# vdBerg93/cl-rrt

Hardware: AMD Instinct MI355X
Metric: nodes expanded/sec (200-obstacle scene) (higher is better)
Workload: dtype f64

## Files before the change

cl-rrt_amd/csrc/clrrt_capi.hip:

```cpp
#include <hip/hip_runtime.h>
#include <math.h>

#include <algorithm>
#include <climits>
#include <array>
#include <chrono>
#include <cmath>
#include <cstdio>
#include <cstdlib>
#include <cstring>
#include <deque>
#include <functional>
#include <optional>
#include <string>
#include <vector>

#include "../../include/clrrt.h"
#include "clrrt_dev.hpp"
#include "clrrt_internal.hpp"

static const int kWalkMaxOver = 2048, kWalkMaxChunks = 64;

using namespace clrrt;

#define CAND_K 10
#define NN_K 11

struct DevBuf {
  void* p = nullptr;
  size_t bytes = 0;
};

struct clrrt_ctx {
  int device = 0;
  int rank = 0;
  hipStream_t stream = nullptr;
  bool own_stream = false;
  clrrt_params params;
  DevParams dp;
  clrrt_capacity cap;
  std::string err;
  clrrt_node* tree = nullptr;
  NnRec* nn = nullptr;
  double* arena = nullptr;
  int64_t n_nodes = 0, n_rows = 0;
  BakedObs* obs = nullptr;
  int n_obs = 0;
  ObsGrid grid{};
  void* grid_buf = nullptr;
  size_t grid_bytes = 0;
  clrrt_sample* d_samples = nullptr;
  float* pk = nullptr;
  int* pi = nullptr;
  int64_t partial_cap = 0;
  int* cand = nullptr;
  float* ckey = nullptr;
  int* ncand = nullptr;
  int* ctie = nullptr;
  KeyId* sort_scratch = nullptr;
  int64_t sort_cap = 0;
  RollRes* res_spec = nullptr;
  clrrt_node* regnodes = nullptr;
  RollRes* res_gb = nullptr;
  double* slots = nullptr;
  int slot_rows = 0;
  int rows_deferred = 1;
  void* rep_buf = nullptr;
  int rep_n = 0;
  bool eval_deferred = false;
  clrrt_node* gbnodes = nullptr;
  SampleOut* so = nullptr;
  int* first_conflict = nullptr;
  clrrt_node* out_nodes = nullptr;
  Job* jobs = nullptr;
  int64_t* totals = nullptr;
  bool totals_zeroed = false;
  unsigned long long* work_ctr = nullptr;
  float* nn_seed = nullptr;
  double bbox[4] = {HUGE_VAL, HUGE_VAL, -HUGE_VAL, -HUGE_VAL};
  double* d_bbox = nullptr;
  double* h_bbox = nullptr;
  int64_t nnw_min_nodes = 8192;
  bool nnw_stateless = false;
  int nnw_bud_tiles = 3072, nnw_bud_ex = 4096, nnw_chunks = 16, nnw_max_over = 1024;
  bool nnw_max_over_set = false;
  bool nnw_bud_tiles_set = false;
  int nnw_half_max = 4096;
  int nnw_hscale = 50;
  int nnw_lpt = 0;
  int nnw_index = 5;
  int nnw_lds_floor = 0;
  int nnw_waves = -1;
  int nnw_double = 1;
  WalkBufs nnw{};
  WalkBufs nnw_alt{};
  struct { int64_t n = -1; double ox, oy, x0, y0, x1, y1; float delta; } nnw_built;
  CompactBufs cmp{};
  int roll_persistent = 1;
  int nn_debug = 0;
  int roll_blocks = 0;
  int n_cu = 256;
  int* roll_q = nullptr;
  int* roll_best = nullptr;
  int roll_priority = 1;
  int roll_coop = 1;
  int roll_spread = 1;
  int roll_lanes = 0;
  int nn_exact_fused = 1;
  int exact_min_width = 8;
  int exact_fixup = 1;
  int exact_fix_cap = 0;
  int* fix_n = nullptr;
  int* fix_ids = nullptr;
  int* fix_adj = nullptr;
  NnRec* fix_xrec = nullptr;
  int* fix_xi = nullptr;
  int* fix_xcand = nullptr;
  float* fix_xkey = nullptr;
  int* fix_xn = nullptr;
  std::vector<int> h_fix_cand;
  std::vector<RollRes> h_fix_spec;
  Job* fix_jobs = nullptr;
  RollRes* fix_res = nullptr;
  std::vector<int> h_fix;
  std::vector<clrrt_sample> h_fix_smp;
  std::vector<Job> h_fix_jobs;
  std::vector<int> h_fix_owner;
  std::vector<RollRes> h_fix_res;
  std::vector<SampleOut> h_fix_so;
  int64_t ex_stats[10] = {0, 0, 0, 0, 0, 0, 0, 0, 0, 0};
  int* roll_perm = nullptr;
  int* roll_pflag = nullptr;
  GoalRec* goal_recs = nullptr;
  int* bp_path = nullptr;
  clrrt_node* path_nodes = nullptr;
  double* path_rows = nullptr;
  int path_cap = 0;
  int64_t path_rows_cap = 0;
  int path_n = 0;
  int64_t path_nrows = 0;
  int* ri_int = nullptr;
  int64_t* ri_off = nullptr;
  float* ri_cost = nullptr;
  double* ri_terms = nullptr;
  double reg_x0 = 0, reg_y0 = 0, reg_x1 = 0, reg_y1 = 0;
  int nn_pipeline = 1;
  hipStream_t side = nullptr;
  int cu_split = 0;
  hipStream_t roll_st = nullptr;
  hipEvent_t ev_rs0 = nullptr, ev_rs1 = nullptr;
  hipEvent_t ev_tree = nullptr, ev_walk = nullptr, ev_commit = nullptr;
  clrrt_sample* d_samples2 = nullptr;
  clrrt_sample* h_samples2 = nullptr;
  int* cand2 = nullptr;
  float* ckey2 = nullptr;
  int* ncand2 = nullptr;
  int* ctie2 = nullptr;
  int nn_lag = 0;
  clrrt_sample* d_samples3 = nullptr;
  clrrt_sample* h_samples3 = nullptr;
  int* cand3 = nullptr;
  float* ckey3 = nullptr;
  int* ncand3 = nullptr;
  int* ctie3 = nullptr;
  WalkBufs nnw3{};
  hipStream_t side2 = nullptr;
  hipStream_t mst = nullptr;
  int nn_split_delta = 0;
  int nn_delta_early = 1;
  int nn_lane_order = 1;
  int* nn_order = nullptr;
  float* wseed[3] = {nullptr, nullptr, nullptr};
  hipEvent_t ev_wm[3] = {nullptr, nullptr, nullptr};
  float* nn_seed2 = nullptr;
  float* d1pk[3] = {nullptr, nullptr, nullptr};
  int* d1pi[3] = {nullptr, nullptr, nullptr};
  hipEvent_t ev_d1[3] = {nullptr, nullptr, nullptr};
  hipEvent_t ev_s[3] = {nullptr, nullptr, nullptr};
  hipEvent_t ev_lagw[3] = {nullptr, nullptr, nullptr};
  int stream_prio = 1;
  int walk_cu_reserve = 0;
  hipEvent_t ev_lag[3] = {nullptr, nullptr, nullptr};
  int stream_prio_applied = 0;
  bool side_prio_set = false;
  std::vector<clrrt_sample> pf_next, pf_samples;
  int pf_state = 0;
  struct {
    int T = 0;
    bool active = false;
    int R = 0;
    int T_alloc = 0, n_steps_alloc = 0;
    int64_t vcap = 0;
    RollRes* res = nullptr;
    RollRes* res_gb = nullptr;
    int* cand = nullptr;
    int* ncand = nullptr;
    clrrt_sample* samp = nullptr;
    int* best = nullptr;
    int* dlist[2] = {nullptr, nullptr};
    int cur_dl = 0, nd = 0;
    int nd_eval = -1;
    int* gv = nullptr;
    uint8_t* pend = nullptr;
    void* sel_tmp = nullptr;
    size_t sel_bytes = 0;
    int* d_cnt = nullptr;
    void* carry[2] = {nullptr, nullptr};
    int cur_c = 0, ncarry = 0, carry_cap = 0;
    int64_t round = 0;
    int slot = 0;
    int64_t deferred_total = 0;
  } def;
  struct {
    int rank = 0, world = 1;
    void* dev_local = nullptr;
    int cap_local = 0;
    clrrt_exchange_fn fn = nullptr;
    void* user = nullptr;
    double max_ms = 0;
    int64_t nd_global = 0;
    int64_t rows_stop = 0;
    int last_nb = 0;
    clrrt_node* xbuf = nullptr;
    uint32_t* xkey = nullptr;
    void* xtmp = nullptr;
    size_t xtmp_bytes = 0;
    int64_t xcap = 0;
    unsigned long long* d_goal = nullptr;
    bool poison_seen = false;
    bool fn_failed = false;
  } sh;
  int fail_at_round = 0;
  int fail_after_exchange = 0;
  bool debug_sync = false;
  unsigned long long* dbg_host = nullptr;
  bool iter_log = false;
  std::vector<int64_t> round_sizes;
  std::vector<clrrt_iteration> iters;
  std::vector<SampleOut> iter_tmp;
  clrrt_sample* h_samples = nullptr;
  int64_t* h_totals = nullptr;
  int* h_int = nullptr;
  int64_t last_eval_rows = 0;
  int64_t last_goal_nodes = 0;
  clrrt_counters counters{};
  int64_t nn_bf_keys = 0, nn_samples = 0;
  int64_t nn_super_bounds = 0;
  bool timing = false;
  static constexpr int kKtClasses = 6;
  double kt_ms[kKtClasses] = {};
  int64_t kt_n[kKtClasses] = {};
  std::vector<hipEvent_t> ev_pool;
  std::vector<std::pair<int, std::pair<hipEvent_t, hipEvent_t>>> ev_pending;
};
// ... 130 lines not shown
extern "C" {

int clrrt_abi_version(void) { return CLRRT_ABI_VERSION; }
static_assert(sizeof(clrrt_exchange_io) == 128, "clrrt_exchange_io layout (clrrt/abi.py ExchangeIO)");

int clrrt_params_default(clrrt_params* p, double v0, const double goal[4], double vmax) {
  if (!p) return CLRRT_EINVAL;
  memset(p, 0, sizeof(*p));
  p->veh.dmax = 0.52; p->veh.ddmax = 0.3294; p->veh.Td = 0.3; p->veh.Ta = 0.3;
  p->veh.amin = -6; p->veh.amax = 2; p->veh.L = 2.7;
  double lf = 1.0868, lr = 1.6132, Cf = 22201, Cr = 22201, m = 950 + 640;
  p->veh.Kus = (m / p->veh.L) * (lr / Cf - lf / Cr);
  p->veh.Vch = 20;
  p->ctrl_tla = 1.4; p->ctrl_mindla = 3.2; p->ctrl_dlavmin = 3; p->ref_int = 0.02; p->ref_mindist = 0.2;
  p->sim_dt = 0.04; p->ctrl_Kp = 8; p->ctrl_Ki = 0.05;
  p->Wcost[0] = 10; p->Wcost[1] = 5; p->Wcost[2] = 0; p->Wcost[3] = 4; p->Wcost[4] = 1;
  p->ref_res = std::max(std::abs(v0) * p->ref_int, p->ref_mindist);
  p->vmax = vmax;
  p->ay_road_max = 0;
  for (int i = 0; i < 4; i++) p->goal[i] = goal ? goal[i] : 0.0;
  p->bend = 0;
  p->obs_use_pred = 1;
  p->sort_limit = 10;
  p->collision_mode = CLRRT_COLLISION_STUB;
  return CLRRT_OK;
}

void clrrt_rng_seed(clrrt_rng* g, uint32_t seed) {
  int32_t* s = g->r;
  int32_t word = (int32_t)(seed == 0 ? 1 : seed);
  s[0] = word;
  for (int i = 1; i < 31; i++) {
    int32_t hi = word / 127773, lo = word % 127773;
    word = 16807 * lo - 2836 * hi;
    if (word < 0) word += 2147483647;
    s[i] = word;
  }
  s[31] = 3;
  s[32] = 0;
  s[33] = 0;
  g->pos = 0;
  for (int i = 0; i < 310; i++) clrrt_rng_next(g);
}

int32_t clrrt_rng_next(clrrt_rng* g) {
  int32_t* s = g->r;
  int f = s[31], r = s[32];
  uint32_t v = (uint32_t)s[f] + (uint32_t)s[r];
  s[f] = (int32_t)v;
  int32_t out = (int32_t)(v >> 1);
  f = f + 1 == 31 ? 0 : f + 1;
  r = r + 1 == 31 ? 0 : r + 1;
  s[31] = f;
  s[32] = r;
  return out;
}

int clrrt_draw_samples(const clrrt_params* p, clrrt_rng* rng, int32_t n, clrrt_sample* out) {
  if (!p || !rng || (n > 0 && !out)) return CLRRT_EINVAL;
  const double* g = p->goal;
  const double RM = 2147483647.0;
  double dGoal = sqrt(g[0] * g[0] + g[1] * g[1]);
  double hd = atan2(g[1], g[0]);
  double latMin = -7, latMax = 7;
  float fl = (float)(RM / (dGoal + 10));
  float fw = (float)(RM / (latMax - latMin));
  double ch, sh, cq, sq;
  ::sincos(hd, &sh, &ch);
  ::sincos(hd + M_PI / 2, &sq, &cq);
  for (int j = 0; j < n; j++) {
    double rLong = (float)clrrt_rng_next(rng) / fl;
    double rLat = latMin + (float)clrrt_rng_next(rng) / fw;
    out[j].x = rLong * ch + rLat * cq;
    out[j].y = rLong * sh + rLat * sq;
    double r = (double)clrrt_rng_next(rng) / (double)(2147483647 / 1);
    out[j].explore = r <= ((0 * 0.3) + (1 * 0.7));
    out[j].pad = 0;
  }
  return CLRRT_OK;
}

const char* clrrt_last_error(const clrrt_ctx* c) { return c ? c->err.c_str() : "null context"; }

static void free_all(clrrt_ctx* c) {
  if (c->side) hipStreamSynchronize(c->side);
  void* ptrs[] = {c->tree, c->nn, c->arena, c->obs, c->d_samples, c->pk, c->pi, c->cand, c->ckey, c->ncand,
                  c->ctie, c->sort_scratch, c->res_spec, c->regnodes, c->res_gb, c->gbnodes, c->so, c->first_conflict,
                  c->out_nodes, c->jobs, c->slots, c->rep_buf, c->totals, c->work_ctr, c->grid_buf,
                  c->nn_seed, c->d_bbox, c->roll_q, c->roll_best, c->roll_perm, c->roll_pflag,
                  c->goal_recs, c->bp_path, c->path_nodes, c->path_rows, c->ri_int, c->ri_off, c->ri_cost,
                  c->ri_terms, c->nnw.keys, c->nnw.keys2, c->nnw.vals, c->nnw.vals2, c->nnw.tmp, c->nnw.P, c->nnw.Q,
                  c->nnw.CE, c->nnw.ID, c->nnw.tiles, c->nnw.supers, c->nnw.sorder, c->nnw.HEAD, c->nnw.ovf_n, c->nnw.ovf, c->nnw.pk, c->nnw.pi, c->nnw_alt.keys, c->nnw_alt.keys2, c->nnw_alt.vals, c->nnw_alt.vals2, c->nnw_alt.tmp, c->nnw_alt.P, c->nnw_alt.Q, c->nnw_alt.CE, c->nnw_alt.ID, c->nnw_alt.tiles, c->nnw_alt.supers, c->nnw_alt.sorder, c->nnw_alt.HEAD, c->nnw_alt.ovf_n, c->nnw_alt.ovf, c->nnw_alt.pk, c->nnw_alt.pi, c->nnw.skeys, c->nnw.sids, c->nnw_alt.skeys, c->nnw_alt.sids, c->cmp.packed, c->cmp.scanned,
                  c->cmp.tmp, c->d_samples2, c->cand2, c->ckey2, c->ncand2, c->ctie2, c->d_samples3, c->cand3, c->ckey3,
                  c->ncand3, c->ctie3, c->nnw3.keys, c->nnw3.keys2, c->nnw3.vals, c->nnw3.vals2, c->nnw3.tmp, c->nnw3.P,
                  c->nnw3.Q, c->nnw3.CE, c->nnw3.ID, c->nnw3.tiles, c->nnw3.supers, c->nnw3.sorder, c->nnw3.HEAD,
                  c->nnw3.ovf_n, c->nnw3.ovf, c->nnw3.pk, c->nnw3.pi, c->nnw3.skeys, c->nnw3.sids,
                  c->nnw.trun, c->nnw_alt.trun, c->nnw3.trun, c->nnw.wctr, c->nnw_alt.wctr, c->nnw3.wctr};
  for (void* p : ptrs)
    if (p) hipFree(p);
  void* sptrs[] = {c->sh.xbuf, c->sh.xkey, c->sh.xtmp, c->sh.d_goal, c->fix_n, c->fix_ids, c->fix_jobs, c->fix_res, c->fix_adj,
                   c->fix_xrec, c->fix_xi, c->fix_xcand, c->fix_xkey, c->fix_xn};
  for (void* p : sptrs)
    if (p) hipFree(p);
  void* dptrs[] = {c->def.res, c->def.res_gb, c->def.cand, c->def.ncand, c->def.samp, c->def.best, c->def.dlist[0],
                   c->def.dlist[1], c->def.gv, c->def.pend, c->def.sel_tmp, c->def.d_cnt, c->def.carry[0],
                   c->def.carry[1]};
  for (void* p : dptrs)
    if (p) hipFree(p);
  if (c->h_samples) hipHostFree(c->h_samples);
  if (c->h_samples2) hipHostFree(c->h_samples2);
  if (c->h_samples3) hipHostFree(c->h_samples3);
  if (c->side2) hipStreamSynchronize(c->side2);
  if (c->side2) hipStreamDestroy(c->side2);
  for (auto e : c->ev_lag)
    if (e) hipEventDestroy(e);
  for (auto e : c->ev_lagw)
    if (e) hipEventDestroy(e);
  if (c->mst) hipStreamSynchronize(c->mst);
  if (c->mst) hipStreamDestroy(c->mst);
  for (int q = 0; q < 3; q++) {
    if (c->ev_d1[q]) hipEventDestroy(c->ev_d1[q]);
    if (c->ev_s[q]) hipEventDestroy(c->ev_s[q]);
    if (c->d1pk[q]) hipFree(c->d1pk[q]);
    if (c->wseed[q]) hipFree(c->wseed[q]);
    if (q == 0 && c->nn_order) hipFree(c->nn_order);
    if (c->ev_wm[q]) hipEventDestroy(c->ev_wm[q]);
    if (c->d1pi[q]) hipFree(c->d1pi[q]);
  }
  if (c->nn_seed2) hipFree(c->nn_seed2);
  if (c->side) hipStreamSynchronize(c->side);
  if (c->ev_tree) hipEventDestroy(c->ev_tree);
  if (c->ev_walk) hipEventDestroy(c->ev_walk);
  if (c->ev_commit) hipEventDestroy(c->ev_commit);
  if (c->side) hipStreamDestroy(c->side);
  if (c->roll_st) hipStreamDestroy(c->roll_st);
  if (c->ev_rs0) hipEventDestroy(c->ev_rs0);
  if (c->ev_rs1) hipEventDestroy(c->ev_rs1);
  if (c->h_totals) hipHostFree(c->h_totals);
  if (c->h_int) hipHostFree(c->h_int);
  if (c->h_bbox) hipHostFree(c->h_bbox);
  if (c->dbg_host) hipHostFree(c->dbg_host);
  for (auto& pe : c->ev_pending) { hipEventDestroy(pe.second.first); hipEventDestroy(pe.second.second); }
  for (auto e : c->ev_pool) hipEventDestroy(e);
  if (c->own_stream && c->stream) hipStreamDestroy(c->stream);
}

int clrrt_create(const clrrt_params* p, const clrrt_capacity* cap, int device, clrrt_ctx** out) {
  if (!p || !out) return CLRRT_EINVAL;
  *out = nullptr;
  int ndev = 0;
  if (hipGetDeviceCount(&ndev) != hipSuccess || ndev <= 0) return CLRRT_EHIP;
  if (device < 0 || device >= ndev) return CLRRT_EINVAL;
  clrrt_ctx* c = new clrrt_ctx();
  c->device = device;
  c->params = *p;
  c->debug_sync = getenv("CLRRT_DEBUG_SYNC") != nullptr;
  clrrt_capacity dc;
  dc.max_nodes = 1 << 20;
  dc.max_rows = 1 << 24;
  dc.max_batch = 4096;
  dc.max_obstacles = 4096;
  c->cap = cap ? *cap : dc;
  if (c->cap.max_nodes < 2 || c->cap.max_rows < 2 || c->cap.max_batch < 1 || c->cap.max_obstacles < 0) {
    delete c;
    return CLRRT_EINVAL;
  }
  derive(c->params, c->dp, 0);
  int rc = CLRRT_OK;
  auto chk = [&](hipError_t e) {
    if (e != hipSuccess && rc == CLRRT_OK) { rc = CLRRT_EHIP; c->err = hipGetErrorString(e); }
  };
  chk(hipSetDevice(device));
  chk(hipStreamCreateWithFlags(&c->stream, hipStreamNonBlocking));
  c->own_stream = true;
  const int64_t B = c->cap.max_batch;
  chk(dalloc(&c->tree, c->cap.max_nodes));
  chk(dalloc(&c->nn, c->cap.max_nodes));
  chk(dalloc(&c->arena, (size_t)c->cap.max_rows * 10));
  chk(dalloc(&c->obs, std::max<int64_t>(1, c->cap.max_obstacles)));
  chk(dalloc(&c->d_samples, B));
  c->partial_cap = std::max<int64_t>(B * 16, 4096) * NN_K;
  chk(dalloc(&c->pk, c->partial_cap));
  chk(dalloc(&c->pi, c->partial_cap));
  chk(dalloc(&c->cand, B * CAND_K));
  chk(dalloc(&c->ckey, B * CAND_K));
  chk(dalloc(&c->ncand, B));
  chk(dalloc(&c->ctie, B));
  chk(dalloc(&c->d_samples2, B));
  chk(dalloc(&c->cand2, B * CAND_K));
  chk(dalloc(&c->ckey2, B * CAND_K));
  chk(dalloc(&c->ncand2, B));
  chk(dalloc(&c->ctie2, B));
  chk(hipStreamCreateWithFlags(&c->side, hipStreamNonBlocking));
  chk(hipEventCreateWithFlags(&c->ev_tree, hipEventDisableTiming));
  chk(hipEventCreateWithFlags(&c->ev_walk, hipEventDisableTiming));
  chk(hipEventCreateWithFlags(&c->ev_commit, hipEventDisableTiming));
  chk(dalloc(&c->res_spec, B * CAND_K));
  chk(dalloc(&c->regnodes, B));
  chk(dalloc(&c->res_gb, B * CAND_K));
  c->slot_rows = 0;
  chk(hipMalloc(&c->rep_buf, replay_bytes() * (size_t)2 * B));
  chk(dalloc(&c->gbnodes, B));
  chk(dalloc(&c->so, B));
  chk(dalloc(&c->first_conflict, 1));
  chk(dalloc(&c->out_nodes, 2 * B));
  chk(dalloc(&c->jobs, 2 * B));
  chk(dalloc(&c->totals, 8));
  chk(dalloc(&c->cmp.packed, B));
  chk(dalloc(&c->cmp.scanned, B));
  c->cmp.tmp_bytes = compact_scan_bytes((int)B);
  chk(hipMalloc(&c->cmp.tmp, std::max<size_t>(c->cmp.tmp_bytes, 256)));
  chk(dalloc(&c->nn_seed, B));
  chk(dalloc(&c->roll_q, 1));
  chk(dalloc(&c->roll_best, B));
  chk(dalloc(&c->roll_perm, (int64_t)B * CAND_K));
  chk(dalloc(&c->roll_pflag, 2 * (int64_t)B * CAND_K + (int64_t)(roll_order_scratch_bytes(B * CAND_K) / 4 + 64)));
  {
    int ncu = 0;
    if (hipDeviceGetAttribute(&ncu, hipDeviceAttributeMultiprocessorCount, device) == hipSuccess && ncu > 0)
      c->n_cu = ncu;
  }
  chk(dalloc(&c->d_bbox, 4));
  chk(hipHostMalloc((void**)&c->h_bbox, sizeof(double) * 4, hipHostMallocDefault));
  chk(dalloc(&c->work_ctr, 64));
  if (rc == CLRRT_OK) chk(hipMemset(c->work_ctr, 0, 64 * sizeof(unsigned long long)));
  chk(hipHostMalloc((void**)&c->h_samples, sizeof(clrrt_sample) * B, hipHostMallocDefault));
  chk(hipHostMalloc((void**)&c->h_samples2, sizeof(clrrt_sample) * B, hipHostMallocDefault));
  chk(hipHostMalloc((void**)&c->h_totals, sizeof(int64_t) * 8, hipHostMallocDefault));
  chk(hipHostMalloc((void**)&c->h_int, sizeof(int) * 4, hipHostMallocDefault));
  if (rc != CLRRT_OK) {
    fprintf(stderr, "clrrt_create: %s\n", c->err.c_str());
    free_all(c);
    delete c;
    return rc;
  }
  *out = c;
  return CLRRT_OK;
}

void clrrt_destroy(clrrt_ctx* c) {
  if (!c) return;
  hipSetDevice(c->device);
  if (c->stream) hipStreamSynchronize(c->stream);
  free_all(c);
  delete c;
}

int clrrt_set_stream(clrrt_ctx* c, void* s) {
  if (!c) return CLRRT_EINVAL;
  HIPC(c, hipStreamSynchronize(c->stream));
  if (c->own_stream) hipStreamDestroy(c->stream);
  if (s) {
    c->stream = (hipStream_t)s;
    c->own_stream = false;
  } else {
    HIPC(c, hipStreamCreateWithFlags(&c->stream, hipStreamNonBlocking));
    c->own_stream = true;
  }
  return CLRRT_OK;
}

int clrrt_set_rank(clrrt_ctx* c, int32_t rank) {
  if (!c || rank < 0) return CLRRT_EINVAL;
  c->rank = rank;
  return CLRRT_OK;
}

int clrrt_set_params(clrrt_ctx* c, const clrrt_params* p) {
  if (!c || !p) return CLRRT_EINVAL;
  pf_reset(c);
  DevParams d;
  derive(*p, d, c->n_obs);
  int rc = flush_replays(c);
  if (rc != CLRRT_OK) return rc;
  if (c->slots && d.n_steps_max + 1 > c->slot_rows) {
    HIPC(c, hipSetDevice(c->device));
    HIPC(c, hipStreamSynchronize(c->stream));
    HIPC(c, hipFree(c->slots));
    c->slots = nullptr;
    c->slot_rows = 0;
    HIPC(c, dalloc(&c->slots, (size_t)2 * (d.n_steps_max + 1) * 10 * c->cap.max_batch * CAND_K));
    c->slot_rows = d.n_steps_max + 1;
  }
  c->params = *p;
  c->dp = d;
  return CLRRT_OK;
}

}

static const float kVehRad = 2.6220219f, kCullMargin = 0.05f;
static int build_grid(clrrt_ctx* c, const std::vector<BakedObs>& b) {
  std::vector<int> stat, mov;
  for (int i = 0; i < (int)b.size(); i++) (b[i].moving ? mov : stat).push_back(i);
// ... 1029 lines not shown
    const RollRes* sres = c->h_fix_spec.data() + (size_t)j * K;
    const int acc = o.k >= 0 ? spec[o.k] : -1;
    for (int q = 0; q < K; q++) {
      if (spec[q] < 0 || (o.k >= 0 && q >= o.k)) break;
      add_res(d, sres[q], -1);
    }
    bool found = false;
    for (int t = 0; t < ln; t++) {
      const int e = lst[t];
      if (e == acc) { found = true; break; }
      int q = -1;
      if (e < N)
        for (int r = 0; r < K && spec[r] >= 0; r++)
          if (spec[r] == e) { q = r; break; }
      if (q >= 0 && (o.k < 0 || q < o.k) && is_fail(sres[q].outcome)) {
        add_res(d, sres[q], +1);
      } else if (e < N) {
        job(j, 0, e);
      } else {
        const int pw = xpos[e - N];
        job(j, 1 + (pw & 1), pw >> 1);
      }
    }
    if (o.k >= 0 && !found) {
      stop = j;
      c->ex_stats[8]++;
      while (!c->h_fix_owner.empty() && c->h_fix_owner.back() == j) {
        c->h_fix_owner.pop_back();
        c->h_fix_jobs.pop_back();
      }
      break;
    }
  }
  const int nj = (int)c->h_fix_jobs.size();
  c->h_fix_res.resize(nj);
  if (nj > 0) {
    HIPC(c, hipMemcpyAsync(c->fix_jobs, c->h_fix_jobs.data(), sizeof(Job) * nj, hipMemcpyHostToDevice, st));
    RollArgs a = roll_args(c, nj);
    a.jobs = c->fix_jobs;
    a.res = c->fix_res;
    a.res_gb = c->fix_res;
    a.xreg = c->regnodes;
    a.xgb = c->gbnodes;
    a.job_stride = 64;
    if (c->exact_fix_cap > 0 && c->exact_fix_cap < a.p.n_steps_max) a.p.n_steps_max = c->exact_fix_cap;
    {
      KTimer kt(c, 1);
      HIPC(c, launch_rollout(st, SRC_LIST, a));
    }
    HIPC(c, hipMemcpyAsync(c->h_fix_res.data(), c->fix_res, sizeof(RollRes) * nj, hipMemcpyDeviceToHost, st));
    HIPC(c, hipStreamSynchronize(st));
  }
  int Lr = stop, resolved = 0;
  bool patched = false;
  const int cap = c->exact_fix_cap > 0 && c->exact_fix_cap < c->dp.n_steps_max ? c->exact_fix_cap : 0;
  for (int j = 0, q = 0; j < stop; j++) {
    SampleOut add = delta[j];
    bool ok = true, any = fn[j] != 0;
    for (; q < nj && c->h_fix_owner[q] == j; q++) {
      const RollRes& r = c->h_fix_res[q];
      if (!is_fail(r.outcome) || (cap && r.outcome == CLRRT_ROLL_ITERLIMIT)) ok = false;
      add_res(add, r, +1);
    }
    if (!ok) {
      Lr = j;
      c->ex_stats[4]++;
      break;
    }
    if (!any) continue;
    SampleOut& o = c->h_fix_so[j];
    o.rollouts += add.rollouts; o.steps += add.steps; o.f_col += add.f_col; o.f_acc += add.f_acc; o.f_it += add.f_it;
    patched = true;
    resolved++;
  }
  if (patched) HIPC(c, hipMemcpyAsync(c->so, c->h_fix_so.data(), sizeof(SampleOut) * Lr, hipMemcpyHostToDevice, st));
  c->ex_stats[0]++;
  c->ex_stats[1] += resolved;
  c->ex_stats[2] += nj;
  c->ex_stats[3] += Lr < n;
  *L = std::max(1, Lr);
  return CLRRT_OK;
}

static int eval_samples(clrrt_ctx* c, int n, bool exact, int* L_out, bool have_lists = false,
                        const std::function<int()>& during_roll = nullptr,
                        const std::function<int()>& pre_roll = nullptr) {
  hipStream_t st = c->stream;
  KeyId* scratch = nullptr;
  if (exact) {
    int rc = ensure_sort_scratch(c, (int64_t)n * c->n_nodes);
    if (rc != CLRRT_OK) return rc;
    scratch = c->sort_scratch;
  }
  if (!have_lists) {
    int rc = run_nn(c, n, scratch);
    if (rc != CLRRT_OK) return rc;
  }
  if (pre_roll) {
    int rc = pre_roll();
    if (rc != CLRRT_OK) return rc;
  }
  if (during_roll) HIPC(c, hipEventRecord(c->ev_tree, st));
  hipStream_t rst = st;
  if (c->roll_st) {
    rst = c->roll_st;
    HIPC(c, hipEventRecord(c->ev_rs0, st));
    HIPC(c, hipStreamWaitEvent(rst, c->ev_rs0, 0));
  }
  const bool persistent = c->roll_persistent && c->dp.n_steps_max > 0;
  const bool deferred = persistent && c->rows_deferred;
  if (!deferred) {
    int rc = flush_replays(c);
    if (rc == CLRRT_OK) rc = ensure_slots(c);
    if (rc != CLRRT_OK) return rc;
  }
  const bool defer = c->def.active && !exact && persistent && deferred;
  if (defer) {
    auto& d = c->def;
    d.slot = (int)(d.round % d.R);
    const int64_t B = c->cap.max_batch;
    HIPC(c, hipMemcpyAsync(d.cand + (int64_t)d.slot * B * CAND_K, c->cand, sizeof(int) * n * CAND_K,
                           hipMemcpyDeviceToDevice, st));
    HIPC(c, hipMemcpyAsync(d.ncand + (int64_t)d.slot * B, c->ncand, sizeof(int) * n, hipMemcpyDeviceToDevice, st));
    HIPC(c, hipMemcpyAsync(d.samp + (int64_t)d.slot * B, c->d_samples, sizeof(clrrt_sample) * n,
                           hipMemcpyDeviceToDevice, st));
    if (d.nd + (int64_t)n > d.vcap) return fail(c, CLRRT_ECAPACITY, "deferred samples exceed the commit buffers");
    if (rst != st) {
      HIPC(c, hipEventRecord(c->ev_rs0, st));
      HIPC(c, hipStreamWaitEvent(rst, c->ev_rs0, 0));
    }
  }
  {
    KTimer kt(c, 1, rst);
    RollArgs a = roll_args(c, n * CAND_K);
    a.res = c->res_spec;
    a.res_gb = c->res_gb;
    if (defer) defer_roll_args(c, a, true);
    a.slots = deferred ? nullptr : c->slots;
    a.slot_rows = c->slot_rows;
    a.slot_jobs = (int)(c->cap.max_batch * CAND_K);
    if (deferred) {
      a.rep = c->rep_buf;
      a.nrep = c->rep_n;
    }
    const int64_t nt = c->n_nodes;
    const int eighths = nt < 300000 ? 7 : nt < 700000 ? 5 : nt < 1100000 ? 4 : 3;
    const int blocks = c->roll_blocks > 0 ? std::min(c->roll_blocks, 4 * c->n_cu)
                       : c->cu_split > 0  ? std::max(1, (c->cu_split * c->n_cu) / 8)
                                          : std::max(1, (eighths * c->n_cu) / 8);
    a.coop_enable = c->roll_coop;
    a.lanes_per_wave = c->roll_lanes > 0 ? c->roll_lanes : c->roll_spread ? 0 : 64;
    if (c->roll_priority) {
      a.perm = c->roll_perm;
      a.pflag = c->roll_pflag;
    }
    unsigned long long*& dbg_host = c->dbg_host;
    if (c->debug_sync) {
      if (!dbg_host) HIPC(c, hipHostMalloc((void**)&dbg_host, sizeof(unsigned long long) * 8 * 4096, hipHostMallocMapped));
      memset(dbg_host, 0, sizeof(unsigned long long) * 8 * 4096);
      HIPC(c, hipHostGetDevicePointer((void**)&a.dbg, dbg_host, 0));
      HIPC(c, hipStreamSynchronize(rst));
      fprintf(stderr, "[dbg] pre-rollout work done (n %d, nrep %d, ncarry %d)\n", n, a.nrep, a.ncarry);
    }
    if (persistent && defer) {
      FillInts f;
      f.add(a.ncarry_out, 1, 0);
      f.add(c->roll_q, 1, 0);
      f.add(c->def.best + a.sbase, n, 0x7f7f7f7f);
      f.add(c->def.d_cnt + 2, 1, 0);
      f.add((int*)c->totals, 16, 0);
      HIPC(c, launch_fill_ints(rst, f));
      c->totals_zeroed = true;
      HIPC(c, launch_rollout_persistent(rst, a, n, c->roll_q, c->def.best, blocks, true));
    } else if (persistent)
      HIPC(c, launch_rollout_persistent(rst, a, n, c->roll_q, defer ? c->def.best : c->roll_best, blocks));
    else
      HIPC(c, launch_rollout(rst, SRC_SPEC, a));
    if (c->debug_sync) {
      const auto t0 = std::chrono::steady_clock::now();
      while (hipStreamQuery(rst) == hipErrorNotReady) {
        if (std::chrono::duration<double>(std::chrono::steady_clock::now() - t0).count() > 10.0) {
          fprintf(stderr, "[dbg] rollout kernel not done after 10 s; waves (iterations, busy, parked, qdone|first "
                          "busy lane, j|pass, steps|chain, wp|N, t):\n");
          unsigned long long tmax = 0;
          for (int w = 0; w < 4096; w++) tmax = std::max(tmax, dbg_host[w * 8 + 7]);
          int shown = 0;
          for (int w = 0; w < 4096 && shown < 40; w++) {
            const unsigned long long* d = dbg_host + w * 8;
            if (d[7] == 0 || tmax - d[7] < 100000000ull) continue;
            if (d[1] == 0 && d[2] == 0 && (d[3] >> 32)) continue;
            fprintf(stderr, "  wave %d: it %llu busy %016llx parked %016llx qdone %llu lane %d j %d pass %d steps %d "
                            "chain %d wp %d N %d age %.3f s\n", w, d[0], d[1], d[2], d[3] >> 32, (int)(uint32_t)d[3],
                    (int)(d[4] >> 32), (int)(uint32_t)d[4], (int)(d[5] >> 32), (int)(uint32_t)d[5], (int)(d[6] >> 32),
                    (int)(uint32_t)d[6], (double)(tmax - d[7]) * 1e-8);
            shown++;
          }
          int alive = 0;
          for (int w = 0; w < 4096; w++) alive += dbg_host[w * 8 + 7] != 0 && tmax - dbg_host[w * 8 + 7] < 100000000ull;
          fprintf(stderr, "  waves still beating: %d\n", alive);
          abort();
        }
      }
      fprintf(stderr, "[dbg] rollout kernel done: %s\n", hipGetErrorString(hipStreamQuery(rst)));
    }
    if (deferred) c->rep_n = 0;
    c->eval_deferred = deferred;
  }
  if (c->roll_st) {
    HIPC(c, hipEventRecord(c->ev_rs1, rst));
    HIPC(c, hipStreamWaitEvent(st, c->ev_rs1, 0));
  }
  if (during_roll) {
    int rc = during_roll();
    if (rc != CLRRT_OK) return rc;
  }
  SelArgs s;
  memset(&s, 0, sizeof(s));
  s.p = c->dp; s.tree = c->tree; s.cand = c->cand; s.ckey = c->ckey; s.ncand = c->ncand; s.res = c->res_spec;
  s.res_gb = c->res_gb; s.regnodes = c->regnodes; s.gbnodes = c->gbnodes; s.so = c->so; s.B = n;
  if (defer) {
    auto& d = c->def;
    s.cand = d.cand; s.ncand = d.ncand; s.res = d.res; s.res_gb = d.res_gb;
    s.ckey = nullptr;
    s.view = d.dlist[d.cur_dl];
    s.nd = d.nd;
    s.sbase = d.slot * (int)c->cap.max_batch;
    s.gv = d.gv;
    s.pend = d.pend;
    s.new_pend = d.d_cnt + 2;
    s.B = d.nd + n;
  }
  c->def.nd_eval = defer ? c->def.nd : -1;
  {
    KTimer kt(c, 2);
    HIPC(c, launch_select(st, s));
  }
  int L = n;
  if (exact && n > 1 && c->exact_fixup) {
    int rc = exact_fixups(c, n, &L);
    if (rc != CLRRT_OK) return rc;
  } else if (exact && n > 1) {
    c->h_int[0] = n;
    HIPC(c, hipMemcpyAsync(c->first_conflict, c->h_int, sizeof(int), hipMemcpyHostToDevice, st));
    {
      KTimer kt(c, 2);
      HIPC(c, launch_conflict(st, c->dp, n, c->d_samples, c->regnodes, c->gbnodes, c->so, c->ctie,
                              c->first_conflict));
    }
    HIPC(c, hipMemcpyAsync(c->h_int + 1, c->first_conflict, sizeof(int), hipMemcpyDeviceToHost, st));
    HIPC(c, hipStreamSynchronize(st));
    L = std::max(1, std::min(n, c->h_int[1]));
  }
  *L_out = L;
  return CLRRT_OK;
}

static int compact_and_copy(clrrt_ctx* c, int L, int* n_out, bool merge_bbox) {
  hipStream_t st = c->stream;
  auto& d = c->def;
  const bool defer = d.nd_eval >= 0;
  const int V = defer ? d.nd_eval + L : L;
  {
    KTimer kt(c, 2);
    const bool tag = defer && c->sh.world > 1;
    HIPC(c, launch_compact(st, V, c->d_samples, c->cand, c->regnodes, c->gbnodes, c->so, c->n_rows, c->rank,
                           c->out_nodes, c->jobs, c->totals, c->cmp, tag ? d.slot : 0, tag ? d.R : 0,
                           (int)c->cap.max_batch, c->totals_zeroed));
    c->totals_zeroed = false;
    if (merge_bbox) HIPC(c, launch_bbox(st, c->out_nodes, c->totals, 0, c->d_bbox));
    if (defer) HIPC(c, launch_defer_select(st, d.gv, d.pend, V, d.dlist[1 - d.cur_dl], d.d_cnt, d.sel_tmp, d.sel_bytes));
  }
  HIPC(c, hipMemcpyAsync(c->h_totals, c->totals, sizeof(int64_t) * 8, hipMemcpyDeviceToHost, st));
  if (merge_bbox) HIPC(c, hipMemcpyAsync(c->h_bbox, c->d_bbox, sizeof(double) * 4, hipMemcpyDeviceToHost, st));
  if (defer) {
    HIPC(c, hipMemcpyAsync(c->h_int, d.d_cnt, sizeof(int) * 2, hipMemcpyDeviceToHost, st));
    HIPC(c, hipMemcpyAsync(c->h_int + 3, d.d_cnt + 2, sizeof(int), hipMemcpyDeviceToHost, st));
    HIPC(c, hipMemcpyAsync(c->h_int + 2, (const char*)(c->work_ctr + 62), sizeof(int), hipMemcpyDeviceToHost, st));
  }
  HIPC(c, hipStreamSynchronize(st));
  {
    const int rw = watchdog_check(c);
    if (rw != CLRRT_OK) return rw;
  }
  if (c->iter_log && !defer && L > 0) {
    c->iter_tmp.resize(L);
    HIPC(c, hipMemcpy(c->iter_tmp.data(), c->so, sizeof(SampleOut) * L, hipMemcpyDeviceToHost));
    for (int j = 0; j < L; j++) {
      const SampleOut& o = c->iter_tmp[j];
      clrrt_iteration r;
      r.nodes = (o.k >= 0) + (o.k >= 0 && o.gb_ok);
      r.sim_count = o.steps; r.fail_collision = o.f_col; r.fail_acclimit = o.f_acc; r.fail_iterlimit = o.f_it;
      r.rollouts = o.rollouts;
      c->iters.push_back(r);
    }
  }
  if (merge_bbox) bbox_add(c, c->h_bbox[0], c->h_bbox[1], c->h_bbox[2], c->h_bbox[3]);
  if (defer) {
    if (c->h_int[2] != 0 || c->h_int[1] > d.carry_cap)
      return fail(c, CLRRT_ECAPACITY, "suspended rollouts exceed the carry buffer (raise defer_steps)");
    if (L > 0) d.deferred_total += c->h_int[3];
    d.cur_dl ^= 1;
    d.nd = c->h_int[0];
    d.cur_c ^= 1;
    d.ncarry = c->h_int[1];
    d.round++;
    d.nd_eval = -1;
  }
  int64_t nn = c->h_totals[0], nr = c->h_totals[1];
  if (c->n_rows + nr > c->cap.max_rows) return fail(c, CLRRT_ECAPACITY, "trajectory arena full");
  if (c->fail_at_round > 0 && --c->fail_at_round == 0)
    return fail(c, CLRRT_ECAPACITY, "injected failure (option fail_at_round)");
  c->counters.sim_count += c->h_totals[2];
  c->counters.fail_collision += c->h_totals[3];
  c->counters.fail_acclimit += c->h_totals[4];
  c->counters.fail_iterlimit += c->h_totals[5];
  c->counters.rollouts += c->h_totals[6];
  c->last_goal_nodes = c->h_totals[7];
  if (c->eval_deferred) {
    if (c->rep_n > 0) {
      int rc = flush_replays(c);
      if (rc != CLRRT_OK) return rc;
    }
    KTimer kt(c, 2);
    if (defer)
      HIPC(c, launch_replay_gather(st, c->jobs, c->out_nodes, (int)nn, c->tree, d.cand, d.samp, d.res, c->rep_buf));
    else
      HIPC(c, launch_replay_gather(st, c->jobs, c->out_nodes, (int)nn, c->tree, c->cand, c->d_samples, c->res_spec,
                                   c->rep_buf));
    c->rep_n = (int)nn;
  } else {
    KTimer kt(c, 2);
    HIPC(c, launch_copy_rows(st, c->jobs, c->out_nodes, (int)nn, c->slots, c->slot_rows,
                             (int)(c->cap.max_batch * CAND_K), c->arena));
  }
  c->n_rows += nr;
  c->last_eval_rows = nr;
  *n_out = (int)nn;
  return CLRRT_OK;
}

static int ensure_defer(clrrt_ctx* c) {
  auto& d = c->def;
  const int64_t B = c->cap.max_batch;
  const int n = std::max(1, c->dp.n_steps_max);
  const int R = (int)((2LL * n + d.T - 1) / d.T) + 2;
  if (c->sh.world > 1 && R > 256)
    return fail(c, CLRRT_EINVAL, "defer_steps too small for sharded rounds (more than 256 rounds in flight)");
  if (!d.res || d.R < R) {
    HIPC(c, hipStreamSynchronize(c->stream));
    for (void* p : {(void*)d.res, (void*)d.res_gb, (void*)d.cand, (void*)d.ncand, (void*)d.samp, (void*)d.best})
      if (p) HIPC(c, hipFree(p));
    d.res = nullptr; d.res_gb = nullptr; d.cand = nullptr; d.ncand = nullptr; d.samp = nullptr; d.best = nullptr;
    d.R = 0;
    HIPC(c, dalloc(&d.res, (size_t)R * B * CAND_K));
    HIPC(c, dalloc(&d.res_gb, (size_t)R * B * CAND_K));
    HIPC(c, dalloc(&d.cand, (size_t)R * B * CAND_K));
    HIPC(c, dalloc(&d.ncand, (size_t)R * B));
    HIPC(c, dalloc(&d.samp, (size_t)R * B));
    HIPC(c, dalloc(&d.best, (size_t)R * B));
    d.R = R;
  }
  if (!d.gv || d.vcap < (int64_t)d.R * B) {
    const int64_t V = (int64_t)d.R * B;
    int rc = flush_replays(c);
    if (rc != CLRRT_OK) return rc;
    HIPC(c, hipStreamSynchronize(c->stream));
    for (void* p : {(void*)c->regnodes, (void*)c->gbnodes, (void*)c->so, (void*)c->out_nodes, (void*)c->jobs,
                    c->rep_buf, (void*)c->cmp.packed, (void*)c->cmp.scanned, c->cmp.tmp})
      if (p) HIPC(c, hipFree(p));
    c->regnodes = nullptr; c->gbnodes = nullptr; c->so = nullptr; c->out_nodes = nullptr; c->jobs = nullptr;
    c->rep_buf = nullptr; c->cmp.packed = nullptr; c->cmp.scanned = nullptr; c->cmp.tmp = nullptr;
    for (void* p : {(void*)d.dlist[0], (void*)d.dlist[1], (void*)d.gv, (void*)d.pend, d.sel_tmp, (void*)d.d_cnt,
                    d.carry[0], d.carry[1]})
      if (p) HIPC(c, hipFree(p));
    d.dlist[0] = d.dlist[1] = nullptr; d.gv = nullptr; d.pend = nullptr; d.sel_tmp = nullptr; d.d_cnt = nullptr;
    d.carry[0] = d.carry[1] = nullptr;
    HIPC(c, dalloc(&c->regnodes, V));
    HIPC(c, dalloc(&c->gbnodes, V));
    HIPC(c, dalloc(&c->so, V));
    HIPC(c, dalloc(&c->out_nodes, 2 * V));
    HIPC(c, dalloc(&c->jobs, 2 * V));
    HIPC(c, hipMalloc(&c->rep_buf, replay_bytes() * (size_t)2 * V));
    HIPC(c, dalloc(&c->cmp.packed, V));
    HIPC(c, dalloc(&c->cmp.scanned, V));
    c->cmp.tmp_bytes = compact_scan_bytes((int)V);
    HIPC(c, hipMalloc(&c->cmp.tmp, std::max<size_t>(c->cmp.tmp_bytes, 256)));
    HIPC(c, dalloc(&d.dlist[0], V));
    HIPC(c, dalloc(&d.dlist[1], V));
    HIPC(c, dalloc(&d.gv, V));
    HIPC(c, dalloc(&d.pend, V));
    d.sel_bytes = defer_select_bytes((int)V);
    HIPC(c, hipMalloc(&d.sel_tmp, std::max<size_t>(d.sel_bytes, 256)));
    HIPC(c, dalloc(&d.d_cnt, 3));
    d.carry_cap = (int)std::min<int64_t>(V * CAND_K, 1 << 21);
    HIPC(c, hipMalloc(&d.carry[0], carry_bytes() * (size_t)d.carry_cap));
    HIPC(c, hipMalloc(&d.carry[1], carry_bytes() * (size_t)d.carry_cap));
    d.vcap = V;
  }
  return CLRRT_OK;
}

static int defer_begin(clrrt_ctx* c, bool batch) {
  auto& d = c->def;
  d.active = batch && d.T > 0 && c->roll_persistent && c->rows_deferred && c->dp.n_steps_max > 0;
  d.nd = 0; d.ncarry = 0; d.round = 0; d.slot = 0; d.nd_eval = -1; d.deferred_total = 0;
  return d.active ? ensure_defer(c) : CLRRT_OK;
}

static void defer_roll_args(clrrt_ctx* c, RollArgs& a, bool capped) {
  auto& d = c->def;
  a.res = d.res;
  a.res_gb = d.res_gb;
  a.jbase = d.slot * (int)c->cap.max_batch * CAND_K;
  a.sbase = d.slot * (int)c->cap.max_batch;
  a.cap = capped ? d.T : 0;
  a.carry_in = d.carry[d.cur_c];
  a.ncarry = d.ncarry;
  a.carry_out = d.carry[1 - d.cur_c];
  a.ncarry_out = d.d_cnt + 1;
  a.carry_cap = d.carry_cap;
}

static int ensure_slots(clrrt_ctx* c) {
  const int need = c->dp.n_steps_max + 1;
  if (c->slots && c->slot_rows >= need) return CLRRT_OK;
  HIPC(c, hipSetDevice(c->device));
  HIPC(c, hipStreamSynchronize(c->stream));
  if (c->slots) HIPC(c, hipFree(c->slots));
  c->slots = nullptr;
  c->slot_rows = 0;
  HIPC(c, dalloc(&c->slots, (size_t)2 * need * 10 * c->cap.max_batch * CAND_K));
  c->slot_rows = need;
  return CLRRT_OK;
}

static int watchdog_check(clrrt_ctx* c) {
  unsigned long long h[4];
  HIPC(c, hipMemcpy(h, c->work_ctr + 56, sizeof(h), hipMemcpyDeviceToHost));
  if (h[0] == 0) return CLRRT_OK;
  char msg[256];
  snprintf(msg, sizeof(msg), "rollout kernel watchdog: %llu waves; j %d fin %d steps %d chain %d qdone %d busy %d",
           h[0], (int)(h[1] >> 32), (int)(uint32_t)h[1], (int)(h[2] >> 32), (int)(uint32_t)h[2], (int)(h[3] >> 32),
           (int)(uint32_t)h[3]);
  return fail(c, CLRRT_EHIP, msg);
}

static int replay_check(clrrt_ctx* c) {
  HIPC(c, hipMemcpyAsync(c->h_int + 2, (const char*)(c->work_ctr + 61), sizeof(int), hipMemcpyDeviceToHost,
                         c->stream));
  HIPC(c, hipStreamSynchronize(c->stream));
  if (c->h_int[2] != 0) return fail(c, CLRRT_EHIP, "a deferred-row replay diverged from its committed rollout");
  return watchdog_check(c);
}

static int flush_replays(clrrt_ctx* c) {
  auto& d = c->def;
  if (c->rep_n <= 0 && d.ncarry <= 0) return CLRRT_OK;
  HIPC(c, hipSetDevice(c->device));
  KTimer kt(c, 1);
  RollArgs a = roll_args(c, 0);
  a.res = c->res_spec;
  a.res_gb = c->res_gb;
  a.rep = c->rep_buf;
  a.nrep = c->rep_n;
  a.coop_enable = c->roll_coop;
  a.lanes_per_wave = c->roll_spread ? 0 : 64;
  int* best = c->roll_best;
  if (d.ncarry > 0) {
    defer_roll_args(c, a, false);
    best = d.best;
    d.ncarry = 0;
  }
  HIPC(c, launch_rollout_persistent(c->stream, a, 0, c->roll_q, best, c->n_cu));
  c->rep_n = 0;
  return replay_check(c);
}

static int defer_drain(clrrt_ctx* c, int64_t* goal_nodes) {
  auto& d = c->def;
  if (!d.active) return CLRRT_OK;
  const bool sharded = c->sh.world > 1;
  if (d.nd > 0 || d.ncarry > 0 || sharded) {
    hipStream_t st = c->stream;
    {
      KTimer kt(c, 1);
      RollArgs a = roll_args(c, 0);
      a.rep = c->rep_buf;
      a.nrep = c->rep_n;
      a.coop_enable = c->roll_coop;
      a.lanes_per_wave = c->roll_spread ? 0 : 64;
      defer_roll_args(c, a, false);
      HIPC(c, launch_rollout_persistent(st, a, 0, c->roll_q, d.best, c->n_cu));
      c->rep_n = 0;
      d.ncarry = 0;
    }
    if (d.nd > 0 || sharded) {
      SelArgs s;
      memset(&s, 0, sizeof(s));
      s.p = c->dp; s.tree = c->tree; s.cand = d.cand; s.ckey = nullptr; s.ncand = d.ncand; s.res = d.res;
      s.res_gb = d.res_gb; s.regnodes = c->regnodes; s.gbnodes = c->gbnodes; s.so = c->so;
      s.view = d.dlist[d.cur_dl]; s.nd = d.nd; s.sbase = 0; s.gv = d.gv; s.pend = d.pend; s.B = d.nd;
      if (d.nd > 0) {
        KTimer kt(c, 2);
        HIPC(c, launch_select(st, s));
      }
      d.nd_eval = d.nd;
      int nn = 0, n_app = 0;
      int rc = compact_and_copy(c, 0, &nn, true);
      if (rc == CLRRT_OK) rc = commit_round(c, nn, c->sh.max_ms, &n_app);
      if (rc != CLRRT_OK) return rc;
      if (goal_nodes) *goal_nodes += c->last_goal_nodes;
      if (d.nd != 0 || d.ncarry != 0) return fail(c, CLRRT_EHIP, "deferred samples left after the drain");
    }
  }
  d.active = false;
  return flush_replays(c);
}

static int append_nodes(clrrt_ctx* c, const clrrt_node* dev_nodes, int n) {
  if (c->n_nodes + n > c->cap.max_nodes) return fail(c, CLRRT_ECAPACITY, "tree full");
  {
    KTimer kt(c, 2);
    HIPC(c, launch_append(c->stream, dev_nodes, n, c->n_nodes, c->tree, c->nn));
  }
  c->n_nodes += n;
  return CLRRT_OK;
}

extern "C" {

int clrrt_round_eval(clrrt_ctx* c, const clrrt_sample* samples, int32_t n, void* dev_out, int32_t* n_out) {
  if (!c || n < 0 || (n > 0 && !samples) || !n_out) return CLRRT_EINVAL;
  if (n > c->cap.max_batch) return fail(c, CLRRT_ECAPACITY, "batch larger than max_batch");
  if (c->n_nodes <= 0) return fail(c, CLRRT_ESTATE, "tree not initialised");
  HIPC(c, hipSetDevice(c->device));
  *n_out = 0;
  if (n == 0) return CLRRT_OK;
  const bool have = c->pf_state == 2 && (int)c->pf_samples.size() == n &&
                    memcmp(c->pf_samples.data(), samples, sizeof(clrrt_sample) * n) == 0;
  if (!have) {
    if (c->pf_state != 0 && c->side) HIPC(c, hipStreamSynchronize(c->side));
    memcpy(c->h_samples, samples, sizeof(clrrt_sample) * n);
    HIPC(c, hipMemcpyAsync(c->d_samples, c->h_samples, sizeof(clrrt_sample) * n, hipMemcpyHostToDevice, c->stream));
  }
  c->pf_state = 0;
  const int n2 = (int)std::min<size_t>(c->pf_next.size(), (size_t)c->cap.max_batch);
  NnSetup su{};
  bool side = false;
  if (n2 > 0 && c->nn_pipeline) {
    su = nn_setup(c);
    side = walk_serves(c, su);
  }
  auto during = [&]() -> int {
    memcpy(c->h_samples2, c->pf_next.data(), sizeof(clrrt_sample) * n2);
    c->pf_samples.assign(c->pf_next.begin(), c->pf_next.begin() + n2);
    c->pf_state = 1;
    return launch_side_walk(c, n2, su);
  };
  c->pf_next.clear();
  int L = n, rc;
  auto build = [&]() -> int { return pre_roll_build(c, su); };
  if ((rc = eval_samples(c, n, false, &L, have, side ? std::function<int()>(during) : nullptr,
                         side ? std::function<int()>(build) : nullptr)) != CLRRT_OK)
    return rc;
  int nn = 0;
  if ((rc = compact_and_copy(c, L, &nn, false)) != CLRRT_OK) return rc;
  if (dev_out && nn > 0)
    HIPC(c, hipMemcpyAsync(dev_out, c->out_nodes, sizeof(clrrt_node) * nn, hipMemcpyDeviceToDevice, c->stream));
  HIPC(c, hipStreamSynchronize(c->stream));
  *n_out = nn;
  return CLRRT_OK;
}

int clrrt_round_commit(clrrt_ctx* c, const void* dev_nodes, int32_t n, int32_t local_first, int32_t local_count) {
  (void)local_first;
  (void)local_count;
  if (!c || n < 0 || (n > 0 && !dev_nodes)) return CLRRT_EINVAL;
  HIPC(c, hipSetDevice(c->device));
  const int64_t first_new = c->n_nodes;
  int rc = append_nodes(c, (const clrrt_node*)dev_nodes, n);
  if (rc != CLRRT_OK) return rc;
  if (n > 0) {
    HIPC(c, launch_bbox(c->stream, (const clrrt_node*)dev_nodes, nullptr, n, c->d_bbox));
    HIPC(c, hipMemcpyAsync(c->h_bbox, c->d_bbox, sizeof(double) * 4, hipMemcpyDeviceToHost, c->stream));
  }
  HIPC(c, hipStreamSynchronize(c->stream));
  if (n > 0) bbox_add(c, c->h_bbox[0], c->h_bbox[1], c->h_bbox[2], c->h_bbox[3]);
  if (c->pf_state == 1) {
    if ((rc = side_delta_launch(c, (int)c->pf_samples.size(), first_new, n)) != CLRRT_OK) return rc;
    if (c->nnw_double && (rc = next_round_build(c)) != CLRRT_OK) return rc;
    if ((rc = side_lists_join(c)) != CLRRT_OK) return rc;
    c->pf_state = 2;
  }
  return CLRRT_OK;
}

int clrrt_rows_flush(clrrt_ctx* c) {
  if (!c) return CLRRT_EINVAL;
  HIPC(c, hipSetDevice(c->device));
  return flush_replays(c);
}

int clrrt_round_prefetch(clrrt_ctx* c, const clrrt_sample* next, int32_t n) {
  if (!c || n < 0 || (n > 0 && !next)) return CLRRT_EINVAL;
  if (n > c->cap.max_batch) return fail(c, CLRRT_ECAPACITY, "batch larger than max_batch");
  c->pf_next.assign(next, next + n);
  return CLRRT_OK;
}

static int shard_goal_reset(clrrt_ctx* c) {
  HIPC(c, hipMemsetAsync(c->sh.d_goal, 0, sizeof(unsigned long long), c->stream));
  return CLRRT_OK;
}
static int shard_goal_count(clrrt_ctx* c, int64_t* out) {
  unsigned long long v = 0;
  HIPC(c, hipMemcpyAsync(c->h_totals, c->sh.d_goal, sizeof(v), hipMemcpyDeviceToHost, c->stream));
  HIPC(c, hipStreamSynchronize(c->stream));
  memcpy(&v, c->h_totals, sizeof(v));
  *out = (int64_t)v;
  return CLRRT_OK;
}

static inline void shard_slice(const clrrt_ctx* c, int64_t g, int64_t* f, int* n) {
  const int64_t W = c->sh.world, r = c->sh.rank;
  *f = g * r / W;
  *n = (int)(g * (r + 1) / W - *f);
}

static int shard_expansion_end(clrrt_ctx* c, int rc) {
  auto& h = c->sh;
  if (h.world > 1 && !h.poison_seen && !h.fn_failed) {
    clrrt_exchange_io io;
    memset(&io, 0, sizeof(io));
    io.flags = 1;
    io.elapsed_ms = h.max_ms;
    io.aux_local = rc != CLRRT_OK ? (1ll << 48) : 0;
    io.bbox_local[0] = io.bbox_local[1] = HUGE_VAL;
    io.bbox_local[2] = io.bbox_local[3] = -HUGE_VAL;
    io.stream = (void*)c->stream;
    io.aux_sum = io.aux_local;
    const int r = h.fn(h.user, &io);
    if (rc == CLRRT_OK) {
      if (r != 0) rc = fail(c, CLRRT_EHIP, "the closing exchange of the sharded expansion failed");
      else if (io.aux_sum >> 48)
        rc = fail(c, CLRRT_EHIP, "sharded expansion: " + std::to_string(io.aux_sum >> 48) + " rank(s) failed");
    }
  }
  if (rc != CLRRT_OK) {
    c->def.ncarry = 0;
    c->def.nd = 0;
  }
  return rc;
}
static void shard_expansion_begin(clrrt_ctx* c) {
  c->sh.poison_seen = c->sh.fn_failed = false;
}

static int commit_round(clrrt_ctx* c, int nn, double elapsed_ms, int* n_app) {
  auto& h = c->sh;
  *n_app = 0;
  if (h.world <= 1) {
    *n_app = nn;
    const int rc = append_nodes(c, c->out_nodes, nn);
    if (rc == CLRRT_OK) c->round_sizes.push_back(c->n_nodes);
    return rc;
  }
  if (nn > h.cap_local) return fail(c, CLRRT_ECAPACITY, "the round's records exceed the exchange buffer");
  std::optional<KTimer> kt;
  kt.emplace(c, 5);
  if (nn > 0)
    HIPC(c, hipMemcpyAsync(h.dev_local, c->out_nodes, sizeof(clrrt_node) * nn, hipMemcpyDeviceToDevice, c->stream));
  clrrt_exchange_io io;
  memset(&io, 0, sizeof(io));
  io.n_local = nn;
  io.elapsed_ms = elapsed_ms;
  const int64_t nd_loc = c->def.active ? c->def.nd : 0;
  const bool rows_full =
      c->n_rows + nn + 2 * ((int64_t)h.last_nb + nd_loc) * (c->dp.n_steps_max + 1) > c->cap.max_rows;
  io.aux_local = nd_loc + (rows_full ? (1ll << 32) : 0);
  for (int q = 0; q < 4; q++) io.bbox_local[q] = nn > 0 ? c->h_bbox[q] : (q < 2 ? HUGE_VAL : -HUGE_VAL);
  io.stream = (void*)c->stream;
  io.max_elapsed_ms = elapsed_ms;
  io.aux_sum = io.aux_local;
  if (h.fn(h.user, &io) != 0 || io.n_all < 0 || (io.n_all > 0 && !io.dev_all)) {
    h.fn_failed = true;
    return fail(c, CLRRT_EHIP, "the exchange of the round's records failed");
  }
  kt.reset();
  const int64_t aux_sum = io.aux_sum;
  if (aux_sum >> 48) {
    h.poison_seen = true;
    return fail(c, CLRRT_EHIP, "sharded expansion: " + std::to_string(aux_sum >> 48) + " rank(s) failed this round");
  }
  if (c->fail_after_exchange > 0 && --c->fail_after_exchange == 0)
    return fail(c, CLRRT_ECAPACITY, "injected failure (option fail_after_exchange)");
  h.max_ms = io.max_elapsed_ms;
  h.nd_global = aux_sum & 0xffffffffll;
  h.rows_stop = (aux_sum >> 32) & 0xffff;
  const int32_t n_all = io.n_all;
  void* all = io.dev_all;
  if (n_all > 0) {
    if (n_all > h.xcap) {
      HIPC(c, hipStreamSynchronize(c->stream));
      for (void* p : {(void*)h.xbuf, (void*)h.xkey, h.xtmp})
        if (p) HIPC(c, hipFree(p));
      h.xbuf = nullptr; h.xkey = nullptr; h.xtmp = nullptr;
      const int64_t cap = std::max<int64_t>(2 * (int64_t)n_all, 4096);
      HIPC(c, dalloc(&h.xbuf, cap));
      HIPC(c, dalloc(&h.xkey, 4 * cap));
      h.xtmp_bytes = xorder_sort_bytes((int)cap);
      HIPC(c, hipMalloc(&h.xtmp, std::max<size_t>(h.xtmp_bytes, 256)));
      h.xcap = cap;
    }
    HIPC(c, launch_xorder(c->stream, (const clrrt_node*)all, n_all, c->def.active, h.xkey, h.xtmp, h.xtmp_bytes,
                          h.xbuf, h.d_goal));
    int rc = append_nodes(c, h.xbuf, n_all);
    if (rc != CLRRT_OK) return rc;
    bbox_add(c, io.bbox_all[0], io.bbox_all[1], io.bbox_all[2], io.bbox_all[3]);
  }
  *n_app = n_all;
  c->round_sizes.push_back(c->n_nodes);
  return CLRRT_OK;
}

struct LagSlot {
  clrrt_sample* d = nullptr;
  clrrt_sample* h = nullptr;
  int* cand = nullptr;
  float* ckey = nullptr;
  int* ncand = nullptr;
  int* ctie = nullptr;
  hipEvent_t ev = nullptr;
  hipEvent_t evw = nullptr;
  int n = 0;
  int64_t g = 0;
  int64_t tree_n = 0;
  int stream = 0;
  float* d1pk = nullptr;
  int* d1pi = nullptr;
  int d1_chunks = 0;
  int64_t d1_count = 0;
  hipEvent_t evd1 = nullptr;
  hipEvent_t evs = nullptr;
  float* wseed = nullptr;
  hipEvent_t evm = nullptr;
};

static int lag_alloc(clrrt_ctx* c) {
  if (c->side2) return CLRRT_OK;
  const int64_t B = c->cap.max_batch;
  HIPC(c, dalloc(&c->d_samples3, B));
  HIPC(c, dalloc(&c->cand3, B * CAND_K));
  HIPC(c, dalloc(&c->ckey3, B * CAND_K));
  HIPC(c, dalloc(&c->ncand3, B));
  HIPC(c, dalloc(&c->ctie3, B));
  HIPC(c, hipHostMalloc((void**)&c->h_samples3, sizeof(clrrt_sample) * B, hipHostMallocDefault));
  for (auto& e : c->ev_lag) HIPC(c, hipEventCreateWithFlags(&e, hipEventDisableTiming));
  for (auto& e : c->ev_lagw) HIPC(c, hipEventCreateWithFlags(&e, hipEventDisableTiming));
  if (c->cu_split > 0) {
    const int nw = (c->n_cu + 31) / 32;
    std::vector<uint32_t> ms(nw, 0u);
    for (int i = 0; i < c->n_cu; i++)
      if ((i % 8) >= c->cu_split) ms[i / 32] |= 1u << (i % 32);
    HIPC(c, hipExtStreamCreateWithCUMask(&c->side2, (uint32_t)nw, ms.data()));
  } else {
    HIPC(c, hipStreamCreateWithFlags(&c->side2, hipStreamNonBlocking));
  }
  HIPC(c, hipStreamCreateWithFlags(&c->mst, hipStreamNonBlocking));
  HIPC(c, dalloc(&c->nn_seed2, B));
  for (int q = 0; q < 3; q++) {
    HIPC(c, dalloc(&c->d1pk[q], c->partial_cap));
    HIPC(c, dalloc(&c->wseed[q], B));
    if (q == 0) HIPC(c, dalloc(&c->nn_order, B));
    HIPC(c, hipEventCreateWithFlags(&c->ev_wm[q], hipEventDisableTiming));
    HIPC(c, dalloc(&c->d1pi[q], c->partial_cap));
    HIPC(c, hipEventCreateWithFlags(&c->ev_d1[q], hipEventDisableTiming));
    HIPC(c, hipEventCreateWithFlags(&c->ev_s[q], hipEventDisableTiming));
  }
  return CLRRT_OK;
}

static int apply_stream_prio(clrrt_ctx* c) {
  const int want = (c->stream_prio ? 1 : 2) + 4 * c->walk_cu_reserve;
  if (c->stream_prio_applied == want || c->cu_split > 0) return CLRRT_OK;
  int lo = 0, hi = 0;
  HIPC(c, hipDeviceGetStreamPriorityRange(&lo, &hi));
  const int p_hi = c->stream_prio ? hi : 0, p_lo = c->stream_prio ? lo : 0;
  HIPC(c, hipDeviceSynchronize());
  auto remake = [&](hipStream_t& st, int pr) -> int {
    if (st) HIPC(c, hipStreamDestroy(st));
    HIPC(c, hipStreamCreateWithPriority(&st, hipStreamNonBlocking, pr));
    return CLRRT_OK;
  };
  int rc;
  if (c->walk_cu_reserve > 0) {
    const int nw = (c->n_cu + 31) / 32;
    std::vector<uint32_t> ms(nw, 0u);
    for (int i = 0; i < c->n_cu; i++)
      if ((i % 8) >= c->walk_cu_reserve) ms[i / 32] |= 1u << (i % 32);
    for (hipStream_t* st : {&c->side, &c->side2}) {
      if (*st) HIPC(c, hipStreamDestroy(*st));
      HIPC(c, hipExtStreamCreateWithCUMask(st, (uint32_t)nw, ms.data()));
    }
    if ((rc = remake(c->mst, p_hi)) != CLRRT_OK) return rc;
  } else if ((!c->side_prio_set && (rc = remake(c->side, p_lo)) != CLRRT_OK) ||
             (rc = remake(c->side2, p_lo)) != CLRRT_OK || (rc = remake(c->mst, p_hi)) != CLRRT_OK) {
    return rc;
  }
  if (c->own_stream && (rc = remake(c->stream, p_hi)) != CLRRT_OK) return rc;
  c->stream_prio_applied = want;
  return CLRRT_OK;
}

static int expand_lag2(clrrt_ctx* c, clrrt_rng* rng, int64_t n_iters, double budget_ms, int32_t batch,
                       clrrt_stats* out) {
  int rc = lag_alloc(c);
  if (rc == CLRRT_OK) rc = apply_stream_prio(c);
  if (rc == CLRRT_OK) rc = defer_begin(c, true);
  if (rc != CLRRT_OK) return rc;
  clrrt_stats st{};
  const auto t0 = std::chrono::steady_clock::now();
  clrrt_rng work = *rng, committed = *rng;
  std::deque<clrrt_sample> pending;
  const int cur = batch;
  const bool sharded = c->sh.world > 1;
  c->sh.max_ms = 0;
  c->sh.nd_global = 0;
  c->sh.rows_stop = 0;
  shard_expansion_begin(c);
  if (sharded && (rc = shard_goal_reset(c)) != CLRRT_OK) return rc;
  const int64_t nodes_before = c->n_nodes;
  hipStream_t sides[2] = {c->side, c->side2};
  WalkBufs* W[3] = {&c->nnw, &c->nnw_alt, &c->nnw3};
  int64_t built_n[3] = {-1, -1, -1};
  double built_f[3][7] = {};
  LagSlot A, B;
  A.d = c->d_samples2; A.h = c->h_samples2; A.cand = c->cand2; A.ckey = c->ckey2; A.ncand = c->ncand2;
  A.ctie = c->ctie2; A.ev = c->ev_lag[0]; A.evw = c->ev_lagw[0];
  B.d = c->d_samples3; B.h = c->h_samples3; B.cand = c->cand3; B.ckey = c->ckey3; B.ncand = c->ncand3;
  B.ctie = c->ctie3; B.ev = c->ev_lag[1]; B.evw = c->ev_lagw[1];
  A.d1pk = c->d1pk[0]; A.d1pi = c->d1pi[0]; A.evd1 = c->ev_d1[0]; A.evs = c->ev_s[0];
  B.d1pk = c->d1pk[1]; B.d1pi = c->d1pi[1]; B.evd1 = c->ev_d1[1]; B.evs = c->ev_s[1];
  A.wseed = c->wseed[0]; A.evm = c->ev_wm[0];
  B.wseed = c->wseed[1]; B.evm = c->ev_wm[1];
  float* cur_wseed = c->wseed[2];
  hipEvent_t cur_evm = c->ev_wm[2];
  const bool early = c->nn_delta_early != 0;
  hipEvent_t cur_ev = c->ev_lag[2];
  hipEvent_t cur_evw = c->ev_lagw[2];
  float* cur_d1pk = c->d1pk[2];
  int* cur_d1pi = c->d1pi[2];
  hipEvent_t cur_evd1 = c->ev_d1[2], cur_evs = c->ev_s[2];
  const bool split_delta = c->nn_split_delta != 0;
  struct RoleGuard {
    std::function<void()> f;
    ~RoleGuard() { f(); }
  } role_guard{[&]() {
    c->d_samples2 = A.d; c->h_samples2 = A.h; c->cand2 = A.cand; c->ckey2 = A.ckey; c->ncand2 = A.ncand; c->ctie2 = A.ctie;
    c->d_samples3 = B.d; c->h_samples3 = B.h; c->cand3 = B.cand; c->ckey3 = B.ckey; c->ncand3 = B.ncand; c->ctie3 = B.ctie;
    c->ev_lag[0] = A.ev; c->ev_lag[1] = B.ev; c->ev_lag[2] = cur_ev;
    c->ev_lagw[0] = A.evw; c->ev_lagw[1] = B.evw; c->ev_lagw[2] = cur_evw;
    c->nnw_built.n = -1;
    c->nnw.sorted_n = -1;
    c->nnw_alt.sorted_n = -1;
    c->nnw3.sorted_n = -1;
  }};
  bool have_cur = false;
  int cur_stream = 0;
  double last_round_ms = 0;
  auto frame_of = [](const NnSetup& su, double* f) {
    f[0] = su.fr.ox; f[1] = su.fr.oy; f[2] = su.fr.delta; f[3] = su.x0; f[4] = su.y0; f[5] = su.x1; f[6] = su.y1;
  };
  auto build = [&](int k, const NnSetup& su) -> int {
    double f[7];
    frame_of(su, f);
    if (built_n[k] == c->n_nodes && std::equal(f, f + 7, built_f[k])) return CLRRT_OK;
    int r2 = ensure_walk_set(c, *W[k]);
    if (r2 != CLRRT_OK) return r2;
    const WalkBufs* prev = nullptr;
    for (int q = 1; q <= 2 && !prev; q++) {
      const WalkBufs* w = W[(k + 3 - q) % 3];
      if (w->P && w->sorted_n > 0) prev = w;
    }
    KTimer kt(c, 0, c->stream);
    HIPC(c, launch_nn_walk_build(c->stream, c->nn, (int)c->n_nodes, su.fr, su.x0, su.y0, su.x1, su.y1, *W[k], prev));
    built_n[k] = c->n_nodes;
    std::copy(f, f + 7, built_f[k]);
    return CLRRT_OK;
  };
  auto walk = [&](LagSlot& sl, int n, int k, const NnSetup& su, int si) -> int {
    hipStream_t s = sides[si];
    int r2 = ensure_walk_set(c, *W[k]);
    if (r2 != CLRRT_OK) return r2;
    c->nn_bf_keys += (int64_t)n * c->n_nodes;
    c->nn_samples += n;
    HIPC(c, hipStreamWaitEvent(s, c->ev_tree, 0));
    HIPC(c, hipMemcpyAsync(sl.d, sl.h, sizeof(clrrt_sample) * n, hipMemcpyHostToDevice, s));
    HIPC(c, hipEventRecord(sl.evs, s));
    sl.d1_count = 0;
    sl.d1_chunks = 0;
    c->nn_super_bounds += (int64_t)n * walk_super_count(c->n_nodes);
    {
      KTimer kt(c, 0, s), kt3(c, 3, s);
      W[k]->seed_out = early ? sl.wseed : nullptr;
      W[k]->ev_main = early ? sl.evm : nullptr;
      const hipError_t ew = launch_nn_walk_search(s, sl.d, n, c->nn, (int)c->n_nodes, c->dp, su.fr, su.x0, su.y0, su.x1,
                                                  su.y1, *W[k], sl.cand, sl.ckey, sl.ncand, sl.ctie, c->work_ctr + 18,
                                                  c->nnw_stateless);
      W[k]->seed_out = nullptr;
      W[k]->ev_main = nullptr;
      HIPC(c, ew);
    }
    HIPC(c, hipEventRecord(sl.evw, s));
    sl.n = n;
    sl.tree_n = c->n_nodes;
    sl.stream = si;
    return CLRRT_OK;
  };
  auto draw_to = [&](int64_t want) {
    while ((int64_t)pending.size() < want) {
      clrrt_sample smp;
      clrrt_draw_samples(&c->params, &work, 1, &smp);
      pending.push_back(smp);
    }
  };
  for (int64_t k = 0; rc == CLRRT_OK; k++) {
    const auto tr0 = std::chrono::steady_clock::now();
    if (n_iters > 0 && st.iterations >= n_iters) break;
    const double ms0 = std::chrono::duration<double, std::milli>(tr0 - t0).count();
    if (n_iters == 0 && !((sharded ? c->sh.max_ms : ms0) < budget_ms)) break;
    const int64_t left = n_iters > 0 ? n_iters - st.iterations : INT64_MAX;
    const int64_t gb = std::min<int64_t>(cur, left);
    int64_t f0 = 0;
    int nb = (int)gb;
    if (sharded) shard_slice(c, gb, &f0, &nb);
    c->sh.last_nb = nb;
    const int64_t nc = gb + (sharded ? c->sh.nd_global : (int64_t)c->def.nd);
    if (c->n_nodes + 2 * nc > c->cap.max_nodes ||
        (sharded ? c->sh.rows_stop > 0 : c->n_rows + 2 * nc * (c->dp.n_steps_max + 1) > c->cap.max_rows)) {
      if (n_iters > 0) { rc = fail(c, CLRRT_ECAPACITY, "tree capacity exhausted"); break; }
      st.capacity_stop = 1;
      break;
    }
    const int wk = (int)(k % 3);
    const NnSetup su = nn_setup(c);
    const bool serve = c->n_nodes >= c->nnw_min_nodes && su.region_ok;
    int64_t gA = 0, gB = 0, fA = 0, fB = 0;
    int nA = 0, nB = 0;
    if (serve) {
      const bool more = n_iters > 0 || ms0 + 2.0 * last_round_ms < budget_ms;
      if (A.n == 0 && (n_iters > 0 || ms0 + last_round_ms < budget_ms)) gA = std::max<int64_t>(0, std::min<int64_t>(cur, left - gb));
      const int64_t gA_eff = A.n > 0 ? A.g : gA;
      if (more && gA_eff > 0) gB = std::max<int64_t>(0, std::min<int64_t>(cur, left - gb - gA_eff));
      nA = (int)gA;
      nB = (int)gB;
      if (sharded) {
        shard_slice(c, gA, &fA, &nA);
        shard_slice(c, gB, &fB, &nB);
      }
    }
    const int64_t gA_all = A.n > 0 ? A.g : gA;
    draw_to(gb + gA_all + gB);
    if (have_cur) {
      KTimer kt(c, 4);
      HIPC(c, hipStreamWaitEvent(c->stream, cur_ev, 0));
    } else {
      for (int j = 0; j < nb; j++) c->h_samples[j] = pending[f0 + j];
      HIPC(c, hipMemcpyAsync(c->d_samples, c->h_samples, sizeof(clrrt_sample) * nb, hipMemcpyHostToDevice, c->stream));
      if (serve) {
        HIPC(c, hipStreamSynchronize(c->side));
        HIPC(c, hipStreamSynchronize(c->side2));
        HIPC(c, hipStreamSynchronize(c->mst));
        if ((rc = build(wk, su)) != CLRRT_OK) break;
        c->nn_bf_keys += (int64_t)nb * c->n_nodes;
        c->nn_samples += nb;
        c->nn_super_bounds += (int64_t)nb * walk_super_count(c->n_nodes);
        KTimer kt(c, 0), kt3(c, 3);
        HIPC(c, launch_nn_walk_search(c->stream, c->d_samples, nb, c->nn, (int)c->n_nodes, c->dp, su.fr, su.x0, su.y0,
                                      su.x1, su.y1, *W[wk], c->cand, c->ckey, c->ncand, c->ctie, c->work_ctr + 18,
                                      c->nnw_stateless));
      } else if ((rc = run_nn(c, nb, nullptr)) != CLRRT_OK) {
        break;
      }
    }
    if (serve && (nA > 0 || nB > 0) && (rc = build(wk, su)) != CLRRT_OK) break;
    auto ahead = [&]() -> int {
      if (nA > 0) {
        for (int j = 0; j < nA; j++) A.h[j] = pending[gb + fA + j];
        const int r2 = walk(A, nA, wk, su, cur_stream);
        if (r2 != CLRRT_OK) return r2;
        A.g = gA;
      }
      if (nB > 0) {
        for (int j = 0; j < nB; j++) B.h[j] = pending[gb + gA_all + fB + j];
        const int r2 = walk(B, nB, wk, su, nA > 0 ? A.stream : 1 - A.stream);
        if (r2 != CLRRT_OK) return r2;
        B.g = gB;
      }
      return CLRRT_OK;
    };
    int L = nb, nn = 0, n_app = 0;
    if ((rc = eval_samples(c, nb, false, &L, true, (nA > 0 || nB > 0) ? std::function<int()>(ahead) : nullptr,
                           nullptr)) != CLRRT_OK)
      break;
    if ((rc = compact_and_copy(c, L, &nn, true)) != CLRRT_OK) break;
    const double ms_commit = std::chrono::duration<double, std::milli>(std::chrono::steady_clock::now() - t0).count();
    if ((rc = commit_round(c, nn, ms_commit, &n_app)) != CLRRT_OK) break;
    if ((A.n > 0 || (split_delta && B.n > 0)))
      HIPC(c, hipEventRecord(c->ev_commit, c->stream));
    if (A.n > 0 && split_delta) {
      hipStream_t s = c->mst;
      HIPC(c, hipStreamWaitEvent(s, c->ev_commit, 0));
      HIPC(c, hipStreamWaitEvent(s, early ? A.evm : A.evw, 0));
      const int64_t first2 = A.tree_n + A.d1_count, cnt2 = c->n_nodes - first2;
      int nch2 = 0;
      if (cnt2 > 0) {
        KTimer kt(c, 0, s);
        c->nn_bf_keys += (int64_t)A.n * cnt2;
        const NnSetup su2 = nn_setup(c);
        const int max_chunks = (int)std::max<int64_t>(1, c->partial_cap / ((int64_t)A.n * NN_K));
        HIPC(c, launch_nn_delta_partial(s, A.d, A.n, c->nn, (int)first2, (int)cnt2, c->dp, su2.fr, c->pk, c->pi,
                                        max_chunks, A.ckey, A.ncand, early ? A.wseed : c->nn_seed, early,
                                        c->nn_lane_order ? c->nn_order : nullptr, &nch2));
      }
      if (early) HIPC(c, hipStreamWaitEvent(s, A.evw, 0));
      if (A.d1_count > 0) HIPC(c, hipStreamWaitEvent(s, A.evd1, 0));
      {
        KTimer kt(c, 0, s);
        if (A.d1_count > 0)
          HIPC(c, launch_nn_delta_merge(s, A.n, A.d1_chunks, c->dp, A.d1pk, A.d1pi, (int)A.tree_n, A.cand, A.ckey,
                                        A.ncand, A.ctie));
        HIPC(c, launch_nn_delta_merge(s, A.n, nch2, c->dp, c->pk, c->pi, (int)first2, A.cand, A.ckey, A.ncand, A.ctie));
      }
      HIPC(c, hipEventRecord(A.ev, s));
    } else if (A.n > 0 && early) {
      hipStream_t s = c->mst;
      HIPC(c, hipStreamWaitEvent(s, c->ev_commit, 0));
      HIPC(c, hipStreamWaitEvent(s, A.evm, 0));
      const int64_t first = A.tree_n, cnt = c->n_nodes - A.tree_n;
      int nch = 0;
      if (cnt > 0) {
        KTimer kt(c, 0, s);
        c->nn_bf_keys += (int64_t)A.n * cnt;
        const NnSetup su2 = nn_setup(c);
        const int max_chunks = (int)std::max<int64_t>(1, c->partial_cap / ((int64_t)A.n * NN_K));
        HIPC(c, launch_nn_delta_partial(s, A.d, A.n, c->nn, (int)first, (int)cnt, c->dp, su2.fr, c->pk, c->pi,
                                        max_chunks, nullptr, nullptr, A.wseed, true,
                                        c->nn_lane_order ? c->nn_order : nullptr, &nch));
      }
      HIPC(c, hipStreamWaitEvent(s, A.evw, 0));
      {
        KTimer kt(c, 0, s);
        HIPC(c, launch_nn_delta_merge(s, A.n, nch, c->dp, c->pk, c->pi, (int)first, A.cand, A.ckey, A.ncand, A.ctie));
      }
      HIPC(c, hipEventRecord(A.ev, s));
    } else if (A.n > 0) {
      hipStream_t s = c->mst;
      HIPC(c, hipStreamWaitEvent(s, c->ev_commit, 0));
      HIPC(c, hipStreamWaitEvent(s, A.evw, 0));
      const int64_t first = A.tree_n, cnt = c->n_nodes - A.tree_n;
      if (cnt > 0) {
        KTimer kt(c, 0, s);
        c->nn_bf_keys += (int64_t)A.n * cnt;
        const NnSetup su2 = nn_setup(c);
        const int max_chunks = (int)std::max<int64_t>(1, c->partial_cap / ((int64_t)A.n * NN_K));
        HIPC(c, launch_nn_delta(s, A.d, A.n, c->nn, (int)first, (int)cnt, c->dp, su2.fr, c->pk, c->pi, max_chunks,
                                A.cand, A.ckey, A.ncand, A.ctie, c->nn_seed));
      }
      HIPC(c, hipEventRecord(A.ev, s));
    }
    if (split_delta && B.n > 0) {
      hipStream_t s2 = c->mst;
      HIPC(c, hipStreamWaitEvent(s2, c->ev_commit, 0));
      HIPC(c, hipStreamWaitEvent(s2, B.evs, 0));
      HIPC(c, hipStreamWaitEvent(s2, early ? B.evm : B.evw, 0));
      const int64_t cnt1 = c->n_nodes - B.tree_n;
      B.d1_count = cnt1;
      B.d1_chunks = 0;
      if (cnt1 > 0) {
        KTimer kt(c, 0, s2);
        c->nn_bf_keys += (int64_t)B.n * cnt1;
        const NnSetup su1 = nn_setup(c);
        const int max_chunks = (int)std::max<int64_t>(1, c->partial_cap / ((int64_t)B.n * NN_K));
        HIPC(c, launch_nn_delta_partial(s2, B.d, B.n, c->nn, (int)B.tree_n, (int)cnt1, c->dp, su1.fr, B.d1pk, B.d1pi,
                                        max_chunks, B.ckey, B.ncand, early ? B.wseed : c->nn_seed2, early,
                                        c->nn_lane_order ? c->nn_order : nullptr, &B.d1_chunks));
      }
      HIPC(c, hipEventRecord(B.evd1, s2));
    }
    {
      const NnSetup sn = nn_setup(c);
      if (B.n > 0 && c->n_nodes >= c->nnw_min_nodes && sn.region_ok && (rc = build((int)((k + 1) % 3), sn)) != CLRRT_OK)
        break;
    }
    for (int64_t j = 0; j < gb; j++) {
      pending.pop_front();
      for (int q = 0; q < 3; q++) clrrt_rng_next(&committed);
    }
    st.iterations += gb;
    st.goal_nodes_added += c->last_goal_nodes;
    st.speculated += gb;
    st.rounds++;
    {
      LagSlot old;
      old.d = c->d_samples; old.h = c->h_samples; old.cand = c->cand; old.ckey = c->ckey; old.ncand = c->ncand;
      old.ctie = c->ctie; old.ev = cur_ev; old.evw = cur_evw; old.stream = cur_stream;
      old.d1pk = cur_d1pk; old.d1pi = cur_d1pi; old.evd1 = cur_evd1; old.evs = cur_evs;
      old.wseed = cur_wseed; old.evm = cur_evm;
      have_cur = A.n > 0;
      c->d_samples = A.d; c->h_samples = A.h; c->cand = A.cand; c->ckey = A.ckey; c->ncand = A.ncand; c->ctie = A.ctie;
      cur_ev = A.ev;
      cur_evw = A.evw;
      cur_stream = A.stream;
      cur_d1pk = A.d1pk; cur_d1pi = A.d1pi; cur_evd1 = A.evd1; cur_evs = A.evs;
      cur_wseed = A.wseed; cur_evm = A.evm;
      A = B;
      B = old;
      B.n = 0;
      B.stream = 1 - A.stream;
    }
    last_round_ms = std::chrono::duration<double, std::milli>(std::chrono::steady_clock::now() - tr0).count();
  }
  if (rc == CLRRT_OK) rc = defer_drain(c, &st.goal_nodes_added);
  st.deferred = c->def.deferred_total;
  if (rc == CLRRT_OK) rc = flush_replays(c);
  if (rc == CLRRT_OK && sharded) rc = shard_goal_count(c, &st.goal_nodes_added);
  rc = shard_expansion_end(c, rc);
  c->def.active = false;
  for (hipStream_t s : {c->side, c->side2, c->mst, c->stream}) {
    const hipError_t e = hipStreamSynchronize(s);
    if (e != hipSuccess && rc == CLRRT_OK) rc = fail(c, CLRRT_EHIP, std::string("hipStreamSynchronize: ") + hipGetErrorString(e));
  }
  st.nodes_added = c->n_nodes - nodes_before;
  st.elapsed_ms = std::chrono::duration<double, std::milli>(std::chrono::steady_clock::now() - t0).count();
  *rng = committed;
  if (out) *out = st;
  return rc;
}

int clrrt_expand(clrrt_ctx* c, clrrt_rng* rng, int64_t n_iters, double budget_ms, int32_t mode, int32_t batch,
                 clrrt_stats* out) {
  if (!c || !rng || n_iters < 0 || (mode != CLRRT_MODE_EXACT && mode != CLRRT_MODE_BATCH)) return CLRRT_EINVAL;
  pf_reset(c);
  if (n_iters == 0 && !(budget_ms > 0)) return CLRRT_EINVAL;
  if (c->n_nodes <= 0) return fail(c, CLRRT_ESTATE, "tree not initialised");
  c->round_sizes.clear();
  const bool sharded = c->sh.world > 1;
  if (sharded && mode != CLRRT_MODE_BATCH) return fail(c, CLRRT_EINVAL, "sharded expansion runs BATCH rounds only");
  HIPC(c, hipSetDevice(c->device));
  const int64_t bmax = (int64_t)c->cap.max_batch * c->sh.world;
  batch = (int32_t)std::max<int64_t>(1, std::min<int64_t>(batch > 0 ? batch : bmax, bmax));
  if (sharded && batch < c->sh.world) return fail(c, CLRRT_EINVAL, "fewer samples per round than ranks");
  const int lag = c->nn_lag ? c->nn_lag
                  : (n_iters == 0 ? budget_ms >= 1000.0 : n_iters >= 64 * (int64_t)batch) ? 2 : 1;
  if (mode == CLRRT_MODE_BATCH && c->nn_pipeline && lag == 2) return expand_lag2(c, rng, n_iters, budget_ms, batch, out);
  clrrt_stats st{};
  auto t0 = std::chrono::steady_clock::now();
  clrrt_rng work = *rng;
  clrrt_rng committed = *rng;
  std::deque<clrrt_sample> pending;
  const bool exact = mode == CLRRT_MODE_EXACT;
  int cur = exact ? std::min(batch, std::max(16, c->exact_min_width)) : batch;
  int64_t nodes_before = c->n_nodes;
  int rc = defer_begin(c, !exact);
  c->sh.max_ms = 0;
  c->sh.nd_global = 0;
  c->sh.rows_stop = 0;
  shard_expansion_begin(c);
  if (rc == CLRRT_OK && sharded) rc = shard_goal_reset(c);
  bool have_next = false;
  double last_round_ms = 0;
  auto draw_to = [&](int64_t want) {
    while ((int64_t)pending.size() < want) {
      clrrt_sample smp;
      clrrt_draw_samples(&c->params, &work, 1, &smp);
      pending.push_back(smp);
    }
  };
  for (; rc == CLRRT_OK;) {
    const auto tr0 = std::chrono::steady_clock::now();
    if (n_iters > 0 && st.iterations >= n_iters) break;
    if (n_iters == 0) {
      double ms = std::chrono::duration<double, std::milli>(std::chrono::steady_clock::now() - t0).count();
      if (!((sharded ? c->sh.max_ms : ms) < budget_ms)) break;
    }
    int64_t gb = cur;
    if (n_iters > 0) gb = std::min<int64_t>(gb, n_iters - st.iterations);
    int64_t f0 = 0;
    int nb = (int)gb;
    if (sharded) shard_slice(c, gb, &f0, &nb);
    c->sh.last_nb = nb;
    const int64_t nc = gb + (sharded ? c->sh.nd_global : (int64_t)c->def.nd);
    if (c->n_nodes + 2 * nc > c->cap.max_nodes ||
        (sharded ? c->sh.rows_stop > 0 : c->n_rows + 2 * nc * (c->dp.n_steps_max + 1) > c->cap.max_rows)) {
      if (n_iters > 0) { rc = fail(c, CLRRT_ECAPACITY, "tree capacity exhausted"); break; }
      st.capacity_stop = 1;
      break;
    }
    draw_to(gb);
    if (!have_next) {
      for (int j = 0; j < nb; j++) c->h_samples[j] = pending[f0 + j];
      HIPC(c, hipMemcpyAsync(c->d_samples, c->h_samples, sizeof(clrrt_sample) * nb, hipMemcpyHostToDevice, c->stream));
    }
    int64_t gb2 = 0, f2 = 0;
    int nb2 = 0;
    NnSetup su{};
    if (!exact && c->nn_pipeline) {
      gb2 = cur;
      if (n_iters > 0) gb2 = std::max<int64_t>(0, std::min<int64_t>(gb2, n_iters - st.iterations - gb));
      if (n_iters == 0) {
        double ms = std::chrono::duration<double, std::milli>(std::chrono::steady_clock::now() - t0).count();
        if (!(ms + last_round_ms < budget_ms)) gb2 = 0;
      }
      nb2 = (int)gb2;
      if (sharded) shard_slice(c, gb2, &f2, &nb2);
      if (nb2 > 0) {
        su = nn_setup(c);
        if (!walk_serves(c, su)) nb2 = 0;
      }
    }
    auto prefetch = [&]() -> int {
      draw_to(gb + gb2);
      for (int j = 0; j < nb2; j++) c->h_samples2[j] = pending[gb + f2 + j];
      return launch_side_walk(c, nb2, su);
    };
    int L = nb, nn = 0, n_app = 0;
    auto build = [&]() -> int { return pre_roll_build(c, su); };
    if ((rc = eval_samples(c, nb, exact, &L, have_next, nb2 > 0 ? std::function<int()>(prefetch) : nullptr,
                           nb2 > 0 ? std::function<int()>(build) : nullptr)) != CLRRT_OK)
      break;
    if (!exact) {
      int64_t want = gb + (int64_t)cur;
      if (n_iters > 0) want = std::min<int64_t>(want, n_iters - st.iterations);
      draw_to(want);
    }
    if ((rc = compact_and_copy(c, L, &nn, true)) != CLRRT_OK) break;
    const int64_t first_new = c->n_nodes;
    const double ms_commit = std::chrono::duration<double, std::milli>(std::chrono::steady_clock::now() - t0).count();
    if ((rc = commit_round(c, nn, ms_commit, &n_app)) != CLRRT_OK) break;
    have_next = false;
    if (nb2 > 0) {
      if ((rc = side_delta_launch(c, nb2, first_new, n_app)) != CLRRT_OK) break;
      if (c->nnw_double && (rc = next_round_build(c)) != CLRRT_OK) break;
      if ((rc = side_lists_join(c)) != CLRRT_OK) break;
      have_next = true;
    }
    const int64_t used = exact ? L : gb;
    for (int64_t j = 0; j < used; j++) {
      pending.pop_front();
      for (int k = 0; k < 3; k++) clrrt_rng_next(&committed);
    }
    st.iterations += used;
    st.goal_nodes_added += c->last_goal_nodes;
    st.speculated += exact ? nb : gb;
    st.rounds++;
    if (exact) cur = std::max(c->exact_min_width, std::min(batch, L == nb ? 2 * nb : 2 * L));
    last_round_ms = std::chrono::duration<double, std::milli>(std::chrono::steady_clock::now() - tr0).count();
  }
  if (rc == CLRRT_OK) rc = defer_drain(c, &st.goal_nodes_added);
  st.deferred = c->def.deferred_total;
  if (rc == CLRRT_OK) rc = flush_replays(c);
  if (rc == CLRRT_OK && sharded) rc = shard_goal_count(c, &st.goal_nodes_added);
  rc = shard_expansion_end(c, rc);
  c->def.active = false;
  HIPC(c, hipStreamSynchronize(c->side));
  HIPC(c, hipStreamSynchronize(c->stream));
  st.nodes_added = c->n_nodes - nodes_before;
  st.elapsed_ms = std::chrono::duration<double, std::milli>(std::chrono::steady_clock::now() - t0).count();
  *rng = committed;
  if (out) *out = st;
  return rc;
}

int clrrt_set_shards(clrrt_ctx* c, int32_t rank, int32_t world, void* dev_local, int32_t cap_local,
                     clrrt_exchange_fn exchange, void* user) {
  if (!c || world < 1 || rank < 0 || rank >= world) return CLRRT_EINVAL;
  if (world > 1 && (!dev_local || cap_local <= 0 || !exchange)) return CLRRT_EINVAL;
  HIPC(c, hipSetDevice(c->device));
  auto& h = c->sh;
  h.rank = rank;
  h.world = world;
  h.dev_local = world > 1 ? dev_local : nullptr;
  h.cap_local = world > 1 ? cap_local : 0;
  h.fn = world > 1 ? exchange : nullptr;
  h.user = world > 1 ? user : nullptr;
  c->rank = rank;
  if (world > 1 && !h.d_goal) HIPC(c, dalloc(&h.d_goal, 1));
  return CLRRT_OK;
}

int clrrt_rollout_batch(clrrt_ctx* c, const clrrt_rollout_job* jobs, int32_t n, clrrt_rollout_result* out,
                        double* rows_out, int32_t rows_cap) {
  if (!c || n < 0 || (n > 0 && (!jobs || !out))) return CLRRT_EINVAL;
  pf_reset(c);
  if (rows_out && rows_cap < c->dp.n_steps_max + 1) return fail(c, CLRRT_EINVAL, "rows_cap < max steps + 1");
  HIPC(c, hipSetDevice(c->device));
  if (n == 0) return CLRRT_OK;
  for (int j = 0; j < n; j++)
    if (jobs[j].parent < 0 || jobs[j].parent >= c->n_nodes) return fail(c, CLRRT_EINVAL, "job parent out of range");
  std::vector<Job> hj(n);
  for (int j = 0; j < n; j++) {
    hj[j].parent = jobs[j].parent; hj[j].from_reg = 0; hj[j].gb = jobs[j].gb; hj[j].pad = 0;
    hj[j].sx = jobs[j].sample[0]; hj[j].sy = jobs[j].sample[1];
    hj[j].row_off = rows_out ? (int64_t)j * rows_cap : -1;
  }
  Job* dj = nullptr;
  RollRes* dr = nullptr;
  double* drows = nullptr;
  hipError_t e = hipMalloc((void**)&dj, sizeof(Job) * n);
  if (e == hipSuccess) e = hipMalloc((void**)&dr, sizeof(RollRes) * n);
  if (e == hipSuccess && rows_out) e = hipMalloc((void**)&drows, sizeof(double) * 10 * (size_t)rows_cap * n);
  if (e == hipSuccess) e = hipMemcpyAsync(dj, hj.data(), sizeof(Job) * n, hipMemcpyHostToDevice, c->stream);
  if (e == hipSuccess) {
    RollArgs a = roll_args(c, n);
    a.jobs = dj;
    a.arena = drows;
    a.res = dr;
    KTimer kt(c, 1);
    e = launch_rollout(c->stream, SRC_LIST, a);
// ... 235 lines not shown
```

cl-rrt_amd/csrc/clrrt_internal.hpp:

```cpp
#pragma once
#include <hip/hip_runtime.h>
#include <stdint.h>

#include "../../include/clrrt.h"
#include "clrrt_dev.hpp"
#include "clrrt_stdsort.hpp"

namespace clrrt {

#define CLRRT_ROLL_PENDING (-2)

struct RollRes {
  double st[10];
  double costE, costS;
  double bx, by;
  double fx, fy;
  double vback;
  int32_t outcome;
  int32_t nrows;
  int32_t refN;
  int32_t pad;
};

struct WorkCtr {
  uint32_t steps, scan, box;
};

struct St10 {
  double v[10];
};

struct Job {
  int32_t parent;
  int32_t from_reg;
  int32_t gb;
  int32_t pad;
  double sx, sy;
  int64_t row_off;
};

struct SampleOut {
  float thr;
  int32_t k;
  int32_t gb_ok;
  int32_t nrows_reg, nrows_gb;
  int32_t rollouts, steps, f_col, f_acc, f_it;
  int32_t g;
  int32_t pend;
};

enum { SRC_SPEC = 0, SRC_LIST = 2, SRC_EXPL = 3 };

struct SimJob {
  double st[10];
  double ax, ay, hx, hy, vstart;
  int32_t n, gb;
  int64_t row_off;
  int64_t ref_off;
};

struct ObsGrid {
  const uint32_t* start;
  const uint16_t* items;
  const uint16_t* mov;
  int gw, gh, nitems, nmov;
  float x0, y0, inv;
};

struct RollArgs {
  DevParams p;
  ObsGrid grid;
  const clrrt_node* __restrict__ tree;
  const clrrt_sample* __restrict__ samples;
  const int* __restrict__ cand;
  const Job* __restrict__ jobs;
  const SimJob* __restrict__ sims;
  double* __restrict__ refv;
  int ref_cap;
  const BakedObs* __restrict__ obs;
  double* __restrict__ arena;
  double* __restrict__ slots;
  int slot_rows, slot_jobs;
  RollRes* __restrict__ res;
  RollRes* __restrict__ res_gb;
  unsigned long long* ctr;
  int njobs;
  int* perm;
  int* pflag;
  int B;
  int coop_off;
  int coop_enable;
  const void* rep;
  int nrep;
  int lanes_per_wave;
  int cap;
  const void* carry_in;
  int ncarry;
  void* carry_out;
  int* ncarry_out;
  int carry_cap;
  int jbase, sbase;
  unsigned long long* dbg;
  const clrrt_node* __restrict__ xreg;
  const clrrt_node* __restrict__ xgb;
  int job_stride;
};

struct SelArgs {
  DevParams p;
  const clrrt_node* __restrict__ tree;
  const int* __restrict__ cand;
  const float* __restrict__ ckey;
  const int* __restrict__ ncand;
  const RollRes* __restrict__ res;
  const RollRes* __restrict__ res_gb;
  clrrt_node* regnodes;
  clrrt_node* gbnodes;
  SampleOut* so;
  int B;
  const int* view;
  int nd, sbase;
  int* gv;
  uint8_t* pend;
  int* new_pend;
};

struct NnFrame {
  double ox, oy;
  float delta;
  int debug;
};
struct WalkTile {
  float pcx, pcy, pr;
  float rcx, rcy, rr;
  float thx, thy, thh;
  float apx, apy, aph;
  float cemin;
  float aopt;
  int32_t nonfinite;
  float eroot;
};
static_assert(sizeof(WalkTile) == 64, "WalkTile layout");
struct WalkBufs {
  uint32_t *keys, *keys2;
  int *vals, *vals2;
  int* sorder;
  void* tmp;
  size_t tmp_bytes;
  float4 *P, *Q;
  float* CE;
  int* ID;
  int* HEAD;
  int2* trun;
  WalkTile *tiles, *supers;
  int bud_tiles, bud_ex, max_over, nch;
  int half_max = 4096;
  int lds_floor = 0;
  int waves = 0;
  int waves_min_batch = 0;
  int index_kind = 0;
  int hscale_pct = 100;
  int* wctr = nullptr;
  int lpt = 0;
  float* seed_out = nullptr;
  hipEvent_t ev_main = nullptr;
  int* ovf_n;
  int4* ovf;
  float* pk;
  int* pi;
  uint64_t* skeys;
  int* sids;
  int64_t sorted_n;
  double sorted_x0, sorted_y0, sorted_scale;
  int sorted_kind;
  int64_t cap_nodes;
  int cap_batch;
};
size_t walk_sort_bytes(int n);
int64_t walk_tile_count(int64_t n);
int64_t walk_super_count(int64_t n);
hipError_t launch_nn_walk(hipStream_t st, const clrrt_sample* S, int B, const NnRec* nodes, int N, const DevParams& p,
                          const NnFrame& fr, double x0, double y0, double x1, double y1, WalkBufs& w, int* cand,
                          float* ckey, int* ncand, int* ctie, unsigned long long* stats, bool stateless);
hipError_t launch_nn_walk_build(hipStream_t st, const NnRec* nodes, int N, const NnFrame& fr, double x0, double y0,
                                double x1, double y1, WalkBufs& w, const WalkBufs* prev = nullptr);
hipError_t launch_nn_walk_search(hipStream_t st, const clrrt_sample* S, int B, const NnRec* nodes, int N,
                                 const DevParams& p, const NnFrame& fr, double x0, double y0, double x1, double y1,
                                 WalkBufs& w, int* cand, float* ckey, int* ncand, int* ctie, unsigned long long* stats,
                                 bool stateless);
hipError_t launch_walk_audit(hipStream_t st, const clrrt_sample* S, int B, const NnRec* nodes, int N, const DevParams& p,
                             const NnFrame& fr, const WalkBufs& w, int* out);
hipError_t launch_nn_delta(hipStream_t st, const clrrt_sample* S, int B, const NnRec* nodes, int first, int count,
                           const DevParams& p, const NnFrame& fr, float* pk, int* pi, int max_chunks, int* cand,
                           float* ckey, int* ncand, int* ctie, float* seed);
hipError_t launch_nn_delta_partial(hipStream_t st, const clrrt_sample* S, int B, const NnRec* nodes, int first,
                                   int count, const DevParams& p, const NnFrame& fr, float* pk, int* pi, int max_chunks,
                                   const float* ckey, const int* ncand, float* gcap, bool seeded, int* order,
                                   int* nchunks_out);
hipError_t launch_nn_delta_merge(hipStream_t st, int B, int nchunks, const DevParams& p, const float* pk, const int* pi,
                                 int id0, int* cand, float* ckey, int* ncand, int* ctie);
hipError_t launch_nn(hipStream_t st, const clrrt_sample* S, int B, const NnRec* nodes, int N,
                     const DevParams& p, float* pk, int* pi, int* cand, float* ckey, int* ncand, int* ctie,
                     int max_chunks, KeyId* exact_scratch, float* seed, unsigned long long* stats, const NnFrame& fr);
hipError_t launch_nn_exact_only(hipStream_t st, const clrrt_sample* S, int B, const NnRec* nodes, int N,
                                const DevParams& p, const int* ctie, KeyId* scratch, int* cand, float* ckey,
                                int* ncand);
hipError_t launch_rollout(hipStream_t st, int src, const RollArgs& a);
hipError_t launch_nn_exact_small(hipStream_t st, const clrrt_sample* S, int B, const NnRec* nodes, int N,
                                 const DevParams& p, int* cand, float* ckey, int* ncand, int* ctie);
int nn_exact_small_max();
hipError_t launch_rollout_persistent(hipStream_t st, const RollArgs& a, int B, int* qnext, int* best, int blocks,
                                     bool prefilled = false);
struct FillInts {
  int* p[8];
  int n[8];
  int v[8];
  int nj = 0;
  void add(int* ptr, int count, int value) {
    if (ptr && count > 0) { p[nj] = ptr; n[nj] = count; v[nj] = value; nj++; }
  }
};
hipError_t launch_fill_ints(hipStream_t st, const FillInts& f);
size_t roll_order_scratch_bytes(int n);
size_t replay_bytes();
size_t carry_bytes();
hipError_t launch_replay_gather(hipStream_t st, const Job* jobs, const clrrt_node* recs, int n, const clrrt_node* tree,
                                const int* cand, const clrrt_sample* S, const RollRes* res, void* out);
hipError_t launch_select(hipStream_t st, const SelArgs& a);
hipError_t launch_copy_rows(hipStream_t st, const Job* jobs, const clrrt_node* recs, int n, const double* slots,
                            int slot_rows, int slot_jobs, double* arena);
#define FIX_MAX 4
hipError_t launch_nn_exact_x(hipStream_t st, const clrrt_sample* S, const NnRec* nodes, int N, const DevParams& p,
                             const clrrt_node* reg, const clrrt_node* gbn, const SampleOut* so, int n, NnRec* xrec,
                             const int* slist, const int* xcnt, int nlist, int xmax, int* cand, float* ckey,
                             int* ncand, int* ctie);
hipError_t launch_conflict_fix(hipStream_t st, const DevParams& p, int B, const clrrt_sample* S,
                               const clrrt_node* reg, const clrrt_node* gbn, const SampleOut* so, const int* ctie,
                               const int* ncand, const float* ckey, const RollRes* res, int* fix_n, int* fix_ids,
                               int* fix_adj);
hipError_t launch_conflict(hipStream_t st, const DevParams& p, int B, const clrrt_sample* S,
                           const clrrt_node* reg, const clrrt_node* gbn, const SampleOut* so, const int* ctie,
                           int* first);
struct CompactBufs {
  uint64_t* packed;
  uint64_t* scanned;
  void* tmp;
  size_t tmp_bytes;
};
size_t compact_scan_bytes(int n);
size_t defer_select_bytes(int n);
hipError_t launch_defer_select(hipStream_t st, const int* gv, const uint8_t* pend, int n, int* out, int* n_out,
                               void* tmp, size_t tmp_bytes);
hipError_t launch_compact(hipStream_t st, int L, const clrrt_sample* S, const int* cand, const clrrt_node* reg,
                          const clrrt_node* gbn, const SampleOut* so, int64_t row_base, int rank,
                          clrrt_node* out, Job* jobs, int64_t* totals, CompactBufs& cb, int tag_slot = 0,
                          int tag_R = 0, int tag_B = 1, bool totals_zeroed = false);
size_t xorder_sort_bytes(int n);
hipError_t launch_xorder(hipStream_t st, const clrrt_node* recs, int n, bool sort, uint32_t* keys, void* tmp,
                         size_t tmp_bytes, clrrt_node* out, unsigned long long* goal);
hipError_t launch_bbox(hipStream_t st, const clrrt_node* recs, const int64_t* n_dev, int n_host, double* out4);
hipError_t launch_append(hipStream_t st, const clrrt_node* in, int n, int64_t base, clrrt_node* tree, NnRec* nn);
hipError_t launch_selftest_math(hipStream_t st, int fn, const double* a, const double* b, int n, double* out);
hipError_t launch_obs_distance(hipStream_t st, const DevParams& p, const BakedObs* obs, const double* states, int n,
                               double* out);
hipError_t launch_selftest_units(hipStream_t st, int unit, const double* in, const BakedObs* obs, int n,
                                 const DevParams& p, const DevParams* cp, double* out);
struct GoalRec { int32_t id; float cost; };
hipError_t launch_goal_gather(hipStream_t st, const clrrt_node* tree, int64_t n, GoalRec* out, int* cnt);
hipError_t launch_backtrack(hipStream_t st, const clrrt_node* tree, int64_t n, int start, int cap, int* path,
                            int* len);
struct ReinitArgs {
  DevParams p;
  const BakedObs* obs;
  const clrrt_node* pn;
  int n;
  const double* prow;
  double car[10];
  clrrt_node* tree;
  NnRec* nn;
  double* arena;
  int* kidx;
  int64_t* koff;
  double* terms;
  float* costs;
  int64_t* out;
  int rank;
  int64_t max_nodes, max_rows;
};
hipError_t launch_gather_nodes(hipStream_t st, const clrrt_node* tree, const int* ids, int n, clrrt_node* out);
hipError_t launch_path_transform(hipStream_t st, clrrt_node* nodes, int n, double* rows, int64_t nrows, int to_world,
                                 const double pose[3]);
hipError_t launch_tree_reinit(hipStream_t st, const ReinitArgs& a);
hipError_t launch_init_root(hipStream_t st, const double* state, clrrt_node* tree, NnRec* nn, double* arena);

}
```

cl-rrt_amd/csrc/clrrt_kernels.hip:

```cpp
#include <hip/hip_runtime.h>
#include <hipcub/hipcub.hpp>
#include <stddef.h>
#include <stdint.h>

#include "clrrt_dev.hpp"
#include "clrrt_internal.hpp"
#include "clrrt_stdsort.hpp"

namespace clrrt {

#define CAND_K 10
#define NN_K (CAND_K + 1)
static_assert(CAND_K == 10, "sortLimit");

__device__ __forceinline__ bool lex_less(float ka, int ia, float kb, int ib) {
  return (ka < kb) || (ka == kb && ia < ib);
}

__device__ __forceinline__ void topk_insert(float (&keys)[NN_K], int (&ids)[NN_K], float k, int i) {
#pragma unroll
  for (int j = 0; j < NN_K; j++) {
    bool sw = lex_less(k, i, keys[j], ids[j]);
    float tk = keys[j];
    int ti = ids[j];
// ... 1138 lines not shown
  PhaseClk pclk{};
  pclk.last = __builtin_amdgcn_s_memtime();
  PhaseClk* pc = &pclk;
#else
  PhaseClk* pc = nullptr;
#endif
  if (act) {
    for (int pass = 0; pass < 2; pass++) {
      RollRes out;
      const RefD R = gb ? make_goal_ref(pbx, pby, P) : make_ref(pbx, pby, sx, sy, P);
      run_rollout_ref<NEED_GAP>(ps, R, pvb, gb, P, ov, rows, es, out, w, nullptr, pc);
      if (pass == 1) {
        a.res_gb[j] = out;
        break;
      }
      a.res[j] = out;
      if (SRC != SRC_SPEC) break;
      const bool ok = (out.outcome == CLRRT_ROLL_END || out.outcome == CLRRT_ROLL_GOAL) &&
                      feasible_goal_bias(P, out.st, out.bx, out.by);
      if (!ok) {
        a.res_gb[j].outcome = -1;
        break;
      }
#pragma unroll
      for (int k = 0; k < 10; k++) ps.v[k] = out.st[k];
      pbx = out.bx; pby = out.by; pvb = out.vback;
      gb = 1;
      if (a.slots) rows = a.slots + pass_stride + j * slot;
    }
  }
  if (a.ctr) {
    __shared__ __attribute__((aligned(16))) unsigned long long s_ctr[4];
    if (threadIdx.x < 3) s_ctr[threadIdx.x] = 0;
    __syncthreads();
    if (w.steps) {
      atomicAdd(&s_ctr[0], (unsigned long long)w.steps);
      atomicAdd(&s_ctr[1], (unsigned long long)w.scan);
      atomicAdd(&s_ctr[2], (unsigned long long)w.box);
    }
    __syncthreads();
    if (threadIdx.x < 3 && s_ctr[threadIdx.x]) atomicAdd(&a.ctr[threadIdx.x], s_ctr[threadIdx.x]);
  }
#ifdef CLRRT_ROLL_PROFILE
  if (a.ctr && j < a.njobs && gt % js == 0)
    for (int q = 0; q < 8; q++) atomicAdd(&a.ctr[40 + q], (unsigned long long)pclk.t[q]);
#endif
}


struct RollSrc {
  double st[10];
  double bx, by, vb;
  double sx, sy;
  int32_t gb, pad;
};

struct Replay {
  RollSrc src;
  int64_t row_off;
  int32_t nrows;
  int32_t pad;
};

struct Carry {
  Roll r;
  double c7, c8, c9;
  int64_t row_off;
  int32_t j;
  int32_t bs;
  int32_t k, pass, steps, chain, rp, nrows_rp;
};

size_t carry_bytes() { return sizeof(Carry); }

__device__ __forceinline__ int roll_likely_long(const double* st, double sx, double sy) {
  const float dx = (float)(sx - st[0]), dy = (float)(sy - st[1]);
  const float d2 = dx * dx + dy * dy;
  if (!(d2 >= 64.f && d2 < 400.f)) return 0;
  const float c = cosf((float)st[2]), s = sinf((float)st[2]);
  const float along = dx * c + dy * s, across = fabsf(dy * c - dx * s);
  return (along > 0.f && across >= 0.57735f * along) ? 1 : 0;
}

__global__ void __launch_bounds__(256) k_roll_order(const int* __restrict__ pflag, const int* __restrict__ ppos,
                                                    int n, int* __restrict__ perm) {
  const int q = blockIdx.x * blockDim.x + threadIdx.x;
  if (q >= n) return;
  const int nf = ppos[n - 1] + pflag[n - 1];
  const int pos = pflag[q] ? ppos[q] : nf + (q - ppos[q]);
  perm[pos] = q;
}

__global__ void __launch_bounds__(256) k_roll_flag(RollArgs a) {
  const int j = blockIdx.x * blockDim.x + threadIdx.x;
  if (j >= a.njobs) return;
  const int id = a.cand[j];
  a.pflag[(j % CAND_K) * a.B + j / CAND_K] =
      id < 0 ? 0 : roll_likely_long(a.tree[id].state, a.samples[j / CAND_K].x, a.samples[j / CAND_K].y);
}

#ifndef REFILL_MIN
#define REFILL_MIN 16
#endif

#ifndef CLRRT_ABANDON_EVERY
#define CLRRT_ABANDON_EVERY 16
#endif

#ifndef CLRRT_ROLL_WAVES
#define CLRRT_ROLL_WAVES 1
#endif
constexpr int kFinSuspend = 1000;
template <bool NEED_GAP, bool COOP, bool CARRY>
__global__ void __launch_bounds__(256) __attribute__((amdgpu_waves_per_eu(CLRRT_ROLL_WAVES))) k_roll_run(RollArgs a,
                                                  int* __restrict__ qnext, int* __restrict__ best, int B) {
  extern __shared__ float4 lds[];
  glibc::stage_tables();
  const ObsView ov = stage_obstacles<NEED_GAP>(a, lds);
  CLRRT_PARAMS_DECL(P);
  const int lane = threadIdx.x & 63;
  CoopLds cl{};
  if constexpr (COOP) {
    char* base = (char*)lds + a.coop_off + (size_t)(threadIdx.x >> 6) * kCoopLdsPerWave;
    cl.veh = (Box4*)base;
    cl.t = (double*)(base + 64 * sizeof(Box4));
    cl.hit = (int*)(base + 64 * sizeof(Box4) + 64 * sizeof(double));
    cl.q = (uint32_t*)(base + 64 * sizeof(Box4) + 64 * sizeof(double) + 64 * sizeof(int));
    cl.cap = COOP_QCAP;
  }
  const int64_t slot = (int64_t)a.slot_rows * 10;
  const int64_t pass_stride = slot * a.slot_jobs;
  WorkCtr w{0, 0, 0};
  Roll r;
  double c7 = 0, c8 = 0, c9 = 0;
  int j = -1, k = 0, bs = 0, pass = 0, steps = 0, chain = 0, cap_at = 0x7fffffff;
  bool exhausted = false;
  const Replay* __restrict__ reps = (const Replay*)a.rep;
  const Carry* __restrict__ cin = (const Carry*)a.carry_in;
  Carry* __restrict__ cout = (Carry*)a.carry_out;
  const int ncarry = CARRY ? a.ncarry : 0;
  const int nq = ncarry + a.nrep + a.njobs;
  double* rows = nullptr;
  bool rp = false;
  int nrows_rp = 0;
  unsigned long long n_rep = 0, n_rep_bad = 0;
  bool iq = false;
  RollSrc src;
  PhaseClk pclk{};
#ifdef CLRRT_ROLL_PROFILE
  __shared__ uint64_t s_phase[4][9];
  PhaseClk* pc = &pclk;
  pclk.wq = s_phase[threadIdx.x >> 6];
  if ((threadIdx.x & 63) == 0) {
    pclk.wq[0] = __builtin_amdgcn_s_memtime();
    for (int q = 1; q < 9; q++) pclk.wq[q] = 0;
  }
  __builtin_amdgcn_wave_barrier();
#else
  PhaseClk* pc = nullptr;
#endif
  int fin = -1;
#ifdef CLRRT_ROLL_PROFILE
  unsigned long long chain_steps = 0, job_steps = 0, tail_steps = 0;
  uint64_t t_qdone = 0;
  const uint64_t t_start = __builtin_amdgcn_s_memtime();
#endif
  bool qdone = false;
#ifdef CLRRT_LANE_STATS
  unsigned long long ls_w[2] = {0, 0}, ls_l[2] = {0, 0}, ls_sparse[2] = {0, 0};
#endif
  const bool lane_on = lane < a.lanes_per_wave;
  const int refill_min = min(REFILL_MIN, max(1, a.lanes_per_wave / 4));

  auto finish_parked = [&]() {
    if (CARRY && fin == kFinSuspend) {
      const int slot_c = atomicAdd(a.ncarry_out, 1);
      if (slot_c < a.carry_cap) {
        Carry& co = cout[slot_c];
        co.r = r;
        co.c7 = c7; co.c8 = c8; co.c9 = c9;
        co.row_off = rows ? (int64_t)((rows - a.arena) / 10) : -1;
// ... 216 lines not shown
#endif
    w.steps++;
    if (rows && (!rp || steps < nrows_rp)) store_row(rows + (int64_t)steps * 10, 1, r, c7, c8, c9);
    if (pc) pc->mark(5);
    if (o < 0 && steps >= P.n_steps_max) o = CLRRT_ROLL_ITERLIMIT;
    if (o >= 0) {
      fin = o;
    } else if (best_s < k) {
      if (pass == 0) a.res[j].outcome = -1;
      a.res_gb[j].outcome = -1;
      j = -1;
    }
  }
  if (a.ctr) {
    unsigned long long v0 = w.steps, v1 = w.scan, v2 = w.box;
#pragma unroll
    for (int q = 32; q > 0; q >>= 1) {
      v0 += (unsigned long long)__shfl_xor((long long)v0, q, 64);
      v1 += (unsigned long long)__shfl_xor((long long)v1, q, 64);
      v2 += (unsigned long long)__shfl_xor((long long)v2, q, 64);
    }
    if (lane == 0 && v0) {
      atomicAdd(&a.ctr[0], v0);
      atomicAdd(&a.ctr[1], v1);
      atomicAdd(&a.ctr[2], v2);
    }
    if (n_rep) {
      atomicAdd(&a.ctr[60], n_rep);
      if (n_rep_bad) atomicAdd(&a.ctr[61], n_rep_bad);
    }
  }
#ifdef CLRRT_LANE_STATS
  if (a.ctr && lane == 0)
    for (int q = 0; q < 2; q++) {
      atomicAdd(&a.ctr[33 + 3 * q], ls_w[q]);
      atomicAdd(&a.ctr[34 + 3 * q], ls_l[q]);
      atomicAdd(&a.ctr[35 + 3 * q], ls_sparse[q]);
    }
#endif
#ifdef CLRRT_ROLL_PROFILE
  if (a.ctr && lane == 0)
    for (int q = 0; q < 8; q++) atomicAdd(&a.ctr[40 + q], (unsigned long long)pclk.wq[1 + q]);
  if (a.ctr) {
    unsigned long long cmax = chain_steps, tail = tail_steps;
#pragma unroll
    for (int q = 32; q > 0; q >>= 1) {
      cmax = max(cmax, (unsigned long long)__shfl_xor((long long)cmax, q, 64));
      tail = max(tail, (unsigned long long)__shfl_xor((long long)tail, q, 64));
    }
    if (lane == 0) {
      const unsigned long long life = __builtin_amdgcn_s_memtime() - t_start;
      atomicAdd(&a.ctr[48], life);
      atomicMax(&a.ctr[49], life);
      atomicMax(&a.ctr[50], cmax);
      atomicAdd(&a.ctr[51], 1ull);
      if (t_qdone) {
        atomicAdd(&a.ctr[52], t_qdone - t_start);
        atomicMax(&a.ctr[53], t_qdone - t_start);
      }
      atomicMax(&a.ctr[54], tail);
      atomicAdd(&a.ctr[55], tail);
    }
  }
#endif
}

__device__ __forceinline__ void fill_node(clrrt_node& n, const RollRes& r, int parent, float pcE,
                                          float pcS) {
  for (int k = 0; k < 10; k++) n.state[k] = r.st[k];
  n.ref_front[0] = r.fx; n.ref_front[1] = r.fy;
  n.ref_back[0] = r.bx; n.ref_back[1] = r.by;
  n.ref_vback = r.vback;
  n.ang_par = node_ang_par(r.bx, r.by, r.fx, r.fy);
  n.parent = parent;
  n.costE = (float)(r.costE + (double)pcE);
  n.costS = (float)(r.costS + (double)pcS);
  n.goal = r.outcome == CLRRT_ROLL_GOAL;
  n.nrows = r.nrows;
  n.owner = 0;
  n.row_offset = -1;
}


__global__ void k_select(SelArgs a) {
  const int v = blockIdx.x * blockDim.x + threadIdx.x;
  if (v >= a.B) return;
  const int g = v < a.nd ? a.view[v] : a.sbase + (v - a.nd);
  const int64_t g0 = (int64_t)g * CAND_K;
  const int nc = a.ncand[g];
  SampleOut o = {};
  o.k = -1;
  o.g = g;
  static_assert(offsetof(RollRes, nrows) == offsetof(RollRes, outcome) + 4 && offsetof(RollRes, outcome) % 8 == 0,
                "outcome and nrows load as one int2");
  int2 on[CAND_K];
#pragma unroll
  for (int k = 0; k < CAND_K; k++)
    on[k] = k < nc ? *(const int2*)&a.res[g0 + k].outcome : make_int2(-1, 1);
  bool pend = false;
#pragma unroll
  for (int k = 0; k < CAND_K; k++) {
    if (k >= nc || o.k >= 0 || pend) break;
    if (on[k].x == CLRRT_ROLL_PENDING) { pend = true; break; }
    o.rollouts++;
    o.steps += on[k].y - 1;
    o.f_col += on[k].x == CLRRT_ROLL_COLLISION;
    o.f_acc += on[k].x == CLRRT_ROLL_ACCLIMIT;
    o.f_it += on[k].x == CLRRT_ROLL_ITERLIMIT;
    if (on[k].x == CLRRT_ROLL_END || on[k].x == CLRRT_ROLL_GOAL) o.k = k;
  }
  if (!pend && o.k >= 0 && a.res_gb[g0 + o.k].outcome == CLRRT_ROLL_PENDING) pend = true;
  if (pend) {
    SampleOut z = {};
    z.k = -1;
    z.g = g;
    z.pend = 1;
    a.so[v] = z;
    if (a.gv) a.gv[v] = g;
    if (a.pend) a.pend[v] = 1;
    if (a.new_pend && v >= a.nd) atomicAdd(a.new_pend, 1);
    return;
  }
  if (a.gv) a.gv[v] = g;
  if (a.pend) a.pend[v] = 0;
  o.thr = !a.ckey ? __builtin_inff()
          : o.k >= 0 ? a.ckey[g0 + o.k] : (nc == a.p.sort_limit ? a.ckey[g0 + nc - 1] : __builtin_inff());
  o.gb_ok = 0;
  if (o.k >= 0) {
    const int pid = a.cand[g0 + o.k];
    const clrrt_node& par = a.tree[pid];
    clrrt_node n;
    fill_node(n, a.res[g0 + o.k], pid, par.costE, par.costS);
    a.regnodes[v] = n;
    o.nrows_reg = n.nrows;
    const RollRes& gr = a.res_gb[g0 + o.k];
    if (gr.outcome >= 0) {
      o.rollouts++;
      o.steps += gr.nrows - 1;
      o.f_col += gr.outcome == CLRRT_ROLL_COLLISION;
      o.f_acc += gr.outcome == CLRRT_ROLL_ACCLIMIT;
      o.f_it += gr.outcome == CLRRT_ROLL_ITERLIMIT;
      if (gr.outcome == CLRRT_ROLL_END || gr.outcome == CLRRT_ROLL_GOAL) {
        clrrt_node gn;
        fill_node(gn, gr, CLRRT_PARENT_PREV, n.costE, n.costS);
        a.gbnodes[v] = gn;
        o.gb_ok = 1;
        o.nrows_gb = gn.nrows;
      }
    }
  }
  a.so[v] = o;
}

__global__ void k_conflict(DevParams p, int B, const clrrt_sample* __restrict__ S,
                           const clrrt_node* __restrict__ regnodes, const clrrt_node* __restrict__ gbnodes,
                           const SampleOut* __restrict__ so, const int* __restrict__ ctie, int* first_conflict) {
  const int j = blockIdx.x * blockDim.x + threadIdx.x;
  if (j >= B) return;
  const double sx = S[j].x, sy = S[j].y;
  const int ex = S[j].explore;
  const float thr = so[j].thr;
  const bool tie = ctie[j] != 0;
  bool conflict = false;
  for (int k = 0; k < j && !conflict; k++) {
    if (so[k].k < 0) continue;
    if (tie) { conflict = true; break; }
    for (int w = 0; w < 2; w++) {
      if (w == 1 && !so[k].gb_ok) break;
      const clrrt_node& n = w == 0 ? regnodes[k] : gbnodes[k];
      float c, s;
      glibc::sincosf((float)(-n.state[2] - 0.0), s, c);
      float key = dubins_key(sx, sy, n.state[0], n.state[1], c, s);
      if (!ex) key = n.costE + key;
      if (!(key > thr) && feasible_node(n.ref_back[0], n.ref_back[1], n.ang_par, sx, sy, p.feas_len)) {
        conflict = true;
        break;
      }
    }
  }
  if (conflict) atomicMin(first_conflict, j);
}

__global__ void k_conflict_fix(DevParams p, int B, const clrrt_sample* __restrict__ S,
                               const clrrt_node* __restrict__ regnodes, const clrrt_node* __restrict__ gbnodes,
                               const SampleOut* __restrict__ so, const int* __restrict__ ctie,
                               const int* __restrict__ ncand, const float* __restrict__ ckey,
                               const RollRes* __restrict__ res, int* __restrict__ fix_n, int* __restrict__ fix_ids,
                               int* __restrict__ fix_adj) {
  const int j = blockIdx.x * blockDim.x + threadIdx.x;
  if (j >= B) return;
  const double sx = S[j].x, sy = S[j].y;
  const int ex = S[j].explore;
  const float thr = so[j].thr;
  const int kk = so[j].k, nc = ncand[j], lim = p.sort_limit;
  const int g0 = so[j].g * CAND_K;
  const bool tie = ctie[j] != 0 &&
                   !(kk >= 0 && kk < lim - 1 && (kk == 0 || ckey[g0 + kk - 1] != ckey[g0 + kk]) &&
                     (kk + 1 >= nc || ckey[g0 + kk + 1] != ckey[g0 + kk]));
  int m = 0;
  int ids[FIX_MAX];
  float nk[FIX_MAX];
  int bad = 0;
  for (int k = 0; k < j && !bad; k++) {
    if (so[k].k < 0) continue;
    if (tie) { bad = 1; break; }
    for (int w = 0; w < 2; w++) {
      if (w == 1 && !so[k].gb_ok) break;
      const clrrt_node& n = w == 0 ? regnodes[k] : gbnodes[k];
      float c, s;
      glibc::sincosf((float)(-n.state[2] - 0.0), s, c);
      float key = dubins_key(sx, sy, n.state[0], n.state[1], c, s);
      if (!ex) key = n.costE + key;
      if (!(key > thr) && feasible_node(n.ref_back[0], n.ref_back[1], n.ang_par, sx, sy, p.feas_len)) {
        if (key == thr || m == FIX_MAX) { bad = key == thr ? 2 : 3; break; }
        ids[m] = 2 * k + w;
        nk[m] = key;
        m++;
      }
    }
  }
  int adj[5] = {0, 0, 0, 0, 0};
  int mw = m;
  if (!bad && m > 0) {
    if (kk >= 0) {
      if (kk + m > lim - 1) bad = 4;
    } else {
      for (int a = 0; a < m && !bad; a++) {
        for (int b = a + 1; b < m; b++)
          if (nk[a] == nk[b]) bad = 1;
        for (int o = 0; o < nc; o++)
          if (nk[a] == ckey[g0 + o]) bad = 1;
      }
      if (!bad) {
        mw = 0;
// ... 20 lines not shown
    }
  }
  for (int a = 0; a < (bad ? 0 : mw); a++) fix_ids[j * FIX_MAX + a] = ids[a];
#pragma unroll
  for (int q = 0; q < 5; q++) fix_adj[j * 5 + q] = adj[q];
  fix_n[j] = bad ? -bad : mw;
}

__global__ void __launch_bounds__(256) k_compact_count(int L, const SampleOut* __restrict__ so,
                                                       const clrrt_node* __restrict__ regnodes,
                                                       const clrrt_node* __restrict__ gbnodes,
                                                       uint64_t* __restrict__ packed, int64_t* __restrict__ totals) {
  const int s = blockIdx.x * blockDim.x + threadIdx.x;
  unsigned long long cnt[6] = {0, 0, 0, 0, 0, 0};
  if (s < L) {
    const SampleOut& o = so[s];
    uint64_t nn = 0, nr = 0;
    if (o.k >= 0) { nn++; nr += (uint64_t)o.nrows_reg; cnt[5] += regnodes[s].goal; }
    if (o.gb_ok) { nn++; nr += (uint64_t)o.nrows_gb; cnt[5] += gbnodes[s].goal; }
    cnt[0] = o.steps; cnt[1] = o.f_col; cnt[2] = o.f_acc; cnt[3] = o.f_it; cnt[4] = o.rollouts;
    packed[s] = (nr << 24) | nn;
  }
  __shared__ unsigned long long s_cnt[6];
  if (threadIdx.x < 6) s_cnt[threadIdx.x] = 0;
  __syncthreads();
#pragma unroll
  for (int c = 0; c < 6; c++) {
    unsigned long long v = cnt[c];
#pragma unroll
    for (int o = 32; o > 0; o >>= 1) v += __shfl_xor(v, o, 64);
    if ((threadIdx.x & 63) == 0 && v) atomicAdd(&s_cnt[c], v);
  }
  __syncthreads();
  if (threadIdx.x < 6 && s_cnt[threadIdx.x]) atomicAdd((unsigned long long*)&totals[2 + threadIdx.x], s_cnt[threadIdx.x]);
}

__global__ void __launch_bounds__(256) k_compact_scatter(int L, const SampleOut* __restrict__ so,
                                                         const clrrt_node* __restrict__ regnodes,
                                                         const clrrt_node* __restrict__ gbnodes,
                                                         const uint64_t* __restrict__ packed,
                                                         const uint64_t* __restrict__ scanned, int64_t row_base,
                                                         int rank, clrrt_node* __restrict__ out, Job* __restrict__ jobs,
                                                         int64_t* __restrict__ totals, int tag_slot, int tag_R,
                                                         int tag_B) {
  const int s = blockIdx.x * blockDim.x + threadIdx.x;
  if (s >= L) return;
  const uint64_t off = scanned[s];
  int64_t node_off = (int64_t)(off & 0xffffffu), row_off = (int64_t)(off >> 24);
  if (s == L - 1) {
    const uint64_t tot = off + packed[s];
    totals[0] = (int64_t)(tot & 0xffffffu);
    totals[1] = (int64_t)(tot >> 24);
  }
  const SampleOut& o = so[s];
  const int tag = tag_R > 0 ? ((tag_slot - o.g / tag_B + tag_R) % tag_R) << 8 : 0;
  if (o.k >= 0) {
    clrrt_node n = regnodes[s];
    n.goal |= tag;
    n.owner = rank;
    n.row_offset = row_base + row_off;
    out[node_off] = n;
    Job jb;
    jb.parent = o.g * CAND_K + o.k; jb.from_reg = 0; jb.gb = 0; jb.pad = 0;
    jb.sx = 0; jb.sy = 0;
    jb.row_off = row_base + row_off;
    jobs[node_off] = jb;
    node_off++;
    row_off += o.nrows_reg;
  }
  if (o.gb_ok) {
    clrrt_node n = gbnodes[s];
    n.goal |= tag;
    n.owner = rank;
    n.row_offset = row_base + row_off;
    out[node_off] = n;
    Job jb;
    jb.parent = o.g * CAND_K + o.k; jb.from_reg = 0; jb.gb = 1; jb.pad = 0;
    jb.sx = 0; jb.sy = 0;
    jb.row_off = row_base + row_off;
    jobs[node_off] = jb;
  }
}

__global__ void __launch_bounds__(256) k_copy_rows(const Job* __restrict__ jobs, const clrrt_node* __restrict__ recs,
                                                   const double* __restrict__ slots, int slot_rows, int slot_jobs,
                                                   double* __restrict__ arena) {
  const int i = blockIdx.x;
  const Job jb = jobs[i];
  const int n = recs[i].nrows * 10;
  const double* src = slots + ((int64_t)jb.gb * slot_jobs + jb.parent) * slot_rows * 10;
  double* dst = arena + jb.row_off * 10;
  for (int t = threadIdx.x; t < n; t += blockDim.x) dst[t] = src[t];
}

__global__ void __launch_bounds__(256) k_replay_gather(const Job* __restrict__ jobs, const clrrt_node* __restrict__ recs,
                                                       int n, const clrrt_node* __restrict__ tree,
                                                       const int* __restrict__ cand, const clrrt_sample* __restrict__ S,
                                                       const RollRes* __restrict__ res, Replay* __restrict__ out) {
  const int i = blockIdx.x * blockDim.x + threadIdx.x;
  if (i >= n) return;
  const Job jb = jobs[i];
  Replay o;
  o.row_off = jb.row_off;
  o.nrows = recs[i].nrows;
  o.pad = 0;
  o.src.gb = jb.gb;
  o.src.pad = 0;
  if (jb.gb) {
    const RollRes& g = res[jb.parent];
#pragma unroll
    for (int q = 0; q < 10; q++) o.src.st[q] = g.st[q];
    o.src.bx = g.bx; o.src.by = g.by; o.src.vb = g.vback;
    o.src.sx = o.src.sy = 0.0;
  } else {
    const clrrt_node& p = tree[cand[jb.parent]];
#pragma unroll
    for (int q = 0; q < 10; q++) o.src.st[q] = p.state[q];
    o.src.bx = p.ref_back[0]; o.src.by = p.ref_back[1]; o.src.vb = p.ref_vback;
    o.src.sx = S[jb.parent / CAND_K].x; o.src.sy = S[jb.parent / CAND_K].y;
  }
  out[i] = o;
}

size_t replay_bytes() { return sizeof(Replay); }

hipError_t launch_replay_gather(hipStream_t st, const Job* jobs, const clrrt_node* recs, int n, const clrrt_node* tree,
                                const int* cand, const clrrt_sample* S, const RollRes* res, void* out) {
  if (n <= 0) return hipSuccess;
  hipLaunchKernelGGL(k_replay_gather, dim3((n + 255) / 256), dim3(256), 0, st, jobs, recs, n, tree, cand, S, res,
                     (Replay*)out);
  return hipGetLastError();
}

__global__ void __launch_bounds__(256) k_bbox(const clrrt_node* __restrict__ recs, const int64_t* n_dev, int n_host,
                                              double* __restrict__ out4) {
  __shared__ double s[4][256];
  const int n = n_dev ? (int)*n_dev : n_host;
  double v[4] = {HUGE_VAL, HUGE_VAL, -HUGE_VAL, -HUGE_VAL};
  for (int i = threadIdx.x; i < n; i += blockDim.x) {
    const double x = recs[i].state[0], y = recs[i].state[1];
    if (isfinite(x) && isfinite(y)) {
      v[0] = fmin(v[0], x); v[1] = fmin(v[1], y); v[2] = fmax(v[2], x); v[3] = fmax(v[3], y);
    }
  }
  for (int k = 0; k < 4; k++) s[k][threadIdx.x] = v[k];
  __syncthreads();
  for (int off = blockDim.x / 2; off > 0; off >>= 1) {
    if ((int)threadIdx.x < off) {
      s[0][threadIdx.x] = fmin(s[0][threadIdx.x], s[0][threadIdx.x + off]);
      s[1][threadIdx.x] = fmin(s[1][threadIdx.x], s[1][threadIdx.x + off]);
      s[2][threadIdx.x] = fmax(s[2][threadIdx.x], s[2][threadIdx.x + off]);
      s[3][threadIdx.x] = fmax(s[3][threadIdx.x], s[3][threadIdx.x + off]);
    }
    __syncthreads();
  }
  if (threadIdx.x < 4) out4[threadIdx.x] = s[threadIdx.x][0];
}

__global__ void k_append(const clrrt_node* __restrict__ in, int n, int64_t base, clrrt_node* __restrict__ tree,
                         NnRec* __restrict__ nn) {
  const int i = blockIdx.x * blockDim.x + threadIdx.x;
  if (i >= n) return;
  clrrt_node d = in[i];
  if (d.parent == CLRRT_PARENT_PREV) d.parent = (int32_t)(base + i - 1);
  tree[base + i] = d;
  NnRec r;
  r.x = d.state[0]; r.y = d.state[1];
  r.bx = d.ref_back[0]; r.by = d.ref_back[1];
  r.ang_par = d.ang_par;
  float ang = (float)(-d.state[2] - 0.0);
  glibc::sincosf(ang, r.s, r.c);
  r.costE = d.costE;
  r.id = (int32_t)(base + i);
  r.ca = cosf((float)d.ang_par); r.sa = sinf((float)d.ang_par);
  nn[base + i] = r;
}

__device__ __forceinline__ NnRec nn_record(const clrrt_node& d, int64_t id) {
  NnRec r;
  r.x = d.state[0]; r.y = d.state[1];
  r.bx = d.ref_back[0]; r.by = d.ref_back[1];
  r.ang_par = d.ang_par;
  float ang = (float)(-d.state[2] - 0.0);
  glibc::sincosf(ang, r.s, r.c);
  r.costE = d.costE;
  r.id = (int32_t)id;
  r.ca = cosf((float)d.ang_par); r.sa = sinf((float)d.ang_par);
  return r;
}

__device__ void init_root(const double* st, clrrt_node* tree, NnRec* nn, double* arena, int owner) {
  const int N = (int)floor(sqrt(1.0 * 1.0 + 0.0 * 0.0) / 0.1);
  double h = (1.0 - 0.0) / (double)(uint64_t)(N - 1);
  double x = 0.0;
  for (int i = 1; i < N; i++) x += h;
  clrrt_node n;
  for (int k = 0; k < 10; k++) { n.state[k] = st[k]; arena[k] = st[k]; }
  n.ref_front[0] = 0.0; n.ref_front[1] = 0.0;
  n.ref_back[0] = x; n.ref_back[1] = 0.0;
  n.ref_vback = st[4];
  n.ang_par = node_ang_par(x, 0.0, 0.0, 0.0);
  n.parent = -1;
  n.costE = 0.f; n.costS = 0.f;
  n.goal = 0;
  n.nrows = 1;
  n.owner = owner;
  n.row_offset = 0;
  tree[0] = n;
  nn[0] = nn_record(n, 0);
}

__global__ void k_init_root(const double* __restrict__ st, clrrt_node* tree, NnRec* nn, double* arena) {
  if (threadIdx.x != 0 || blockIdx.x != 0) return;
  init_root(st, tree, nn, arena, 0);
}

__global__ void __launch_bounds__(256) k_goal_gather(const clrrt_node* __restrict__ tree, int64_t n,
                                                     GoalRec* __restrict__ out, int* __restrict__ cnt) {
  for (int64_t i = (int64_t)blockIdx.x * blockDim.x + threadIdx.x; i - threadIdx.x < n;
       i += (int64_t)gridDim.x * blockDim.x) {
    const bool g = i < n && tree[i].goal != 0;
    const unsigned long long m = __ballot(g);
    if (m == 0) continue;
    const int lane = threadIdx.x & 63;
    int base = 0;
    if (lane == __ffsll((long long)m) - 1) base = atomicAdd(cnt, __popcll(m));
    base = __shfl(base, __ffsll((long long)m) - 1);
    if (g) {
      const int off = __popcll(m & ((1ull << lane) - 1ull));
      out[base + off] = GoalRec{(int32_t)i, tree[i].costS};
    }
  }
}

__global__ void k_backtrack(const clrrt_node* __restrict__ tree, int64_t n, int start, int cap,
                            int* __restrict__ path, int* __restrict__ len) {
  if (threadIdx.x != 0 || blockIdx.x != 0) return;
  int k = 0;
  int64_t p = start;
  while (p >= 0 && p < n && k <= n) {
    if (k < cap) path[k] = (int)p;
    k++;
    p = tree[p].parent;
  }
  *len = (p == -1) ? k : -1;
}

__global__ void k_gather_nodes(const clrrt_node* __restrict__ tree, const int* __restrict__ ids, int n,
                               clrrt_node* __restrict__ out) {
  const int i = blockIdx.x * blockDim.x + threadIdx.x;
  if (i < n) out[i] = tree[ids[i]];
}

__device__ __forceinline__ void point_world_to_car(double& Xw, double& Yw, double P0, double P1, double s,
                                                   double c) {
  double Xc = Xw * c - P0 * c - P1 * s + Yw * s;
  double Yc = Yw * c - P1 * c + P0 * s - Xw * s;
  Xw = Xc; Yw = Yc;
}
__device__ __forceinline__ void point_car_to_world(double& Xc, double& Yc, double P0, double P1, double s,
                                                   double c) {
  double Xw = c * Xc - s * Yc + P0;
  double Yw = s * Xc + c * Yc + P1;
  Xc = Xw; Yc = Yw;
}

__global__ void __launch_bounds__(256) k_path_transform(clrrt_node* __restrict__ nodes, int n,
                                                        double* __restrict__ rows, int64_t nrows, int to_world,
                                                        double P0, double P1, double P2) {
  glibc::stage_tables();
  double s, c;
// ... 370 lines not shown
    if (e != hipSuccess) return e;
    e = launch_nn_brute(st, S, B, nodes, N, p, fr, pk, pi, cand, ckey, ncand, ctie, max_chunks, seed,
                        stats ? stats + 5 : nullptr);
    if (e != hipSuccess) return e;
  }
  if (exact_scratch) return launch_nn_exact_any(st, S, B, nodes, N, p, ctie, exact_scratch, cand, ckey, ncand);
  return hipSuccess;
}

hipError_t launch_nn_exact_small(hipStream_t st, const clrrt_sample* S, int B, const NnRec* nodes, int N,
                                 const DevParams& p, int* cand, float* ckey, int* ncand, int* ctie) {
  if (N > NN_EXACT_LDS_MAX || B <= 0) return hipErrorInvalidValue;
  const size_t lds = sizeof(KeyId) * (size_t)N + sizeof(int2) * (size_t)(N / 2 + 64);
  if (lds > 64 * 1024) {
    const hipError_t e = hipFuncSetAttribute((const void*)&k_nn_exact_fused, hipFuncAttributeMaxDynamicSharedMemorySize,
                                             (int)lds);
    if (e != hipSuccess) return e;
  }
  hipLaunchKernelGGL(k_nn_exact_fused, dim3(B), dim3(64), lds, st, S, B, nodes, N, p, cand, ckey, ncand, ctie);
  return hipGetLastError();
}

int nn_exact_small_max() { return NN_EXACT_LDS_MAX; }

__global__ void k_build_xrec(const clrrt_node* __restrict__ reg, const clrrt_node* __restrict__ gbn,
                             const SampleOut* __restrict__ so, int n, int64_t base, NnRec* __restrict__ xrec) {
  if (blockIdx.x != 0 || threadIdx.x != 0) return;
  int64_t pos = 0;
  for (int k = 0; k < n; k++) {
    if (so[k].k < 0) continue;
    xrec[pos] = nn_record(reg[k], base + pos);
    pos++;
    if (so[k].gb_ok) {
      xrec[pos] = nn_record(gbn[k], base + pos);
      pos++;
    }
  }
}

hipError_t launch_nn_exact_x(hipStream_t st, const clrrt_sample* S, const NnRec* nodes, int N, const DevParams& p,
                             const clrrt_node* reg, const clrrt_node* gbn, const SampleOut* so, int n, NnRec* xrec,
                             const int* slist, const int* xcnt, int nlist, int xmax, int* cand, float* ckey,
                             int* ncand, int* ctie) {
  if (nlist <= 0) return hipSuccess;
  const int Nl = N + xmax;
  if (Nl > NN_EXACT_LDS_MAX) return hipErrorInvalidValue;
  hipLaunchKernelGGL(k_build_xrec, dim3(1), dim3(64), 0, st, reg, gbn, so, n, (int64_t)N, xrec);
  LAUNCH_CHECK();
  const size_t lds = sizeof(KeyId) * (size_t)Nl + sizeof(int2) * (size_t)(Nl / 2 + 64);
  if (lds > 64 * 1024) {
    const hipError_t e = hipFuncSetAttribute((const void*)&k_nn_exact_fused, hipFuncAttributeMaxDynamicSharedMemorySize,
                                             (int)lds);
    if (e != hipSuccess) return e;
  }
  hipLaunchKernelGGL(k_nn_exact_fused, dim3(nlist), dim3(64), lds, st, S, nlist, nodes, N, p, cand, ckey, ncand, ctie,
                     (const NnRec*)xrec, xcnt, slist, Nl);
  return hipGetLastError();
}

hipError_t launch_nn_delta(hipStream_t st, const clrrt_sample* S, int B, const NnRec* nodes, int first, int count,
                           const DevParams& p, const NnFrame& fr, float* pk, int* pi, int max_chunks, int* cand,
                           float* ckey, int* ncand, int* ctie, float* seed) {
  if (count <= 0 || B <= 0) return hipSuccess;
  const int groups = (B + CLRRT_PATH_BLK - 1) / CLRRT_PATH_BLK;
  int nchunks = (count + 255) / 256;
  const int want = max(1, 2048 / max(1, groups));
  nchunks = max(1, min(nchunks, min(want, max_chunks)));
  int chunk = (count + nchunks - 1) / nchunks;
  chunk = (chunk + 255) & ~255;
  nchunks = (count + chunk - 1) / chunk;
  hipLaunchKernelGGL(k_nn_delta_seed, dim3((B + 63) / 64), dim3(64), 0, st, B, p.sort_limit, ckey, ncand, seed);
  LAUNCH_CHECK();
  hipLaunchKernelGGL(k_nn_partial, dim3(groups, nchunks), dim3(CLRRT_PATH_BLK), 0, st, S, B, nodes + first, count, chunk,
                     nchunks, p, fr, pk, pi, seed, nullptr, nullptr);
  LAUNCH_CHECK();
  hipLaunchKernelGGL(k_nn_merge_delta, dim3((B + 63) / 64), dim3(64), 0, st, B, nchunks, p.sort_limit, pk, pi,
                     first, cand, ckey, ncand, ctie);
  LAUNCH_CHECK();
  return hipSuccess;
}

hipError_t launch_nn_delta_partial(hipStream_t st, const clrrt_sample* S, int B, const NnRec* nodes, int first,
                                   int count, const DevParams& p, const NnFrame& fr, float* pk, int* pi, int max_chunks,
                                   const float* ckey, const int* ncand, float* gcap, bool seeded, int* order,
                                   int* nchunks_out) {
  *nchunks_out = 0;
  if (count <= 0 || B <= 0) return hipSuccess;
  const int* sord = nullptr;
  if (order) {
    hipLaunchKernelGGL(k_nn_order, dim3(1), dim3(1024), 0, st, S, B, order);
    LAUNCH_CHECK();
    sord = order;
  }
  const int groups = (B + CLRRT_PATH_BLK - 1) / CLRRT_PATH_BLK;
  int nchunks = (count + 255) / 256;
  const int want = max(1, 2048 / max(1, groups));
  nchunks = max(1, min(nchunks, min(want, max_chunks)));
  int chunk = (count + nchunks - 1) / nchunks;
  chunk = (chunk + 255) & ~255;
  nchunks = (count + chunk - 1) / chunk;
  if (!seeded) {
    hipLaunchKernelGGL(k_nn_delta_seed, dim3((B + 63) / 64), dim3(64), 0, st, B, ckey ? p.sort_limit : 0, ckey, ncand,
                       gcap);
    LAUNCH_CHECK();
  }
  hipLaunchKernelGGL(k_nn_partial, dim3(groups, nchunks), dim3(CLRRT_PATH_BLK), 0, st, S, B, nodes + first, count, chunk,
                     nchunks, p, fr, pk, pi, gcap, nullptr, sord);
  LAUNCH_CHECK();
  *nchunks_out = nchunks;
  return hipSuccess;
}
hipError_t launch_nn_delta_merge(hipStream_t st, int B, int nchunks, const DevParams& p, const float* pk, const int* pi,
                                 int id0, int* cand, float* ckey, int* ncand, int* ctie) {
  if (nchunks <= 0 || B <= 0) return hipSuccess;
  hipLaunchKernelGGL(k_nn_merge_delta, dim3((B + 63) / 64), dim3(64), 0, st, B, nchunks, p.sort_limit, pk, pi, id0, cand,
                     ckey, ncand, ctie);
  LAUNCH_CHECK();
  return hipSuccess;
}

hipError_t launch_nn_exact_only(hipStream_t st, const clrrt_sample* S, int B, const NnRec* nodes, int N,
                                const DevParams& p, const int* ctie, KeyId* scratch, int* cand, float* ckey,
                                int* ncand) {
  return launch_nn_exact_any(st, S, B, nodes, N, p, ctie, scratch, cand, ckey, ncand);
}

static hipError_t launch_nn_brute(hipStream_t st, const clrrt_sample* S, int B, const NnRec* nodes, int N,
                                  const DevParams& p, const NnFrame& fr, float* pk, int* pi, int* cand,
                                  float* ckey, int* ncand, int* ctie, int max_chunks, const float* seed,
                                  unsigned long long* tstat) {
  int threads = 256;
  int groups = (B + 255) / 256;
  int nchunks = (N + 255) / 256;
  int want = max(1, 2048 / max(1, groups));
  nchunks = max(1, min(nchunks, min(want, max_chunks)));

  int chunk = (N + nchunks - 1) / nchunks;
  chunk = (chunk + 255) & ~255;
  nchunks = (N + chunk - 1) / chunk;
  hipLaunchKernelGGL(k_nn_partial, dim3(groups, nchunks), dim3(threads), 0, st, S, B, nodes, N, chunk, nchunks,
                     p, fr, pk, pi, seed, tstat, nullptr);
  LAUNCH_CHECK();
  hipLaunchKernelGGL(k_nn_merge, dim3((B + 255) / 256), dim3(256), 0, st, B, nchunks, p.sort_limit, pk, pi,
                     cand, ckey, ncand, ctie);
  LAUNCH_CHECK();
  return hipSuccess;
}

static size_t roll_lds_bytes(const RollArgs& a) {
  size_t lds = 0;
  if (a.p.coll_mode == CLRRT_COLLISION_OBB) {
    lds = (size_t)a.p.n_obs * (6 * sizeof(float4) + sizeof(float));
    if (a.grid.gw > 0)
      lds += sizeof(uint32_t) * ((size_t)a.grid.gw * a.grid.gh + 1) +
             sizeof(uint16_t) * ((size_t)a.grid.nitems + a.grid.nmov);
  }
  return lds;
}

template <int SRC>
static hipError_t launch_roll_t(hipStream_t st, const RollArgs& a) {
  if (a.njobs <= 0) return hipSuccess;
  const size_t lds = roll_lds_bytes(a);
  const int64_t threads = (int64_t)a.njobs * (a.job_stride > 1 ? a.job_stride : 1);
  dim3 grid((unsigned)((threads + 255) / 256)), block(256);
  if (a.p.need_gap)
    hipLaunchKernelGGL((k_rollout<SRC, true>), grid, block, 0, st, a);
  else
  {
    if (lds > 64 * 1024) {
      hipError_t e = hipFuncSetAttribute((const void*)&k_rollout<SRC, false>,
                                         hipFuncAttributeMaxDynamicSharedMemorySize, (int)lds);
      if (e != hipSuccess) return e;
    }
    hipLaunchKernelGGL((k_rollout<SRC, false>), grid, block, lds, st, a);
  }
  LAUNCH_CHECK();
  return hipSuccess;
}

size_t roll_order_scratch_bytes(int n) {
  size_t bytes = 0;
  hipcub::DeviceScan::ExclusiveSum(nullptr, bytes, (const int*)nullptr, (int*)nullptr, n);
  return bytes;
}
static hipError_t roll_order(hipStream_t st, const RollArgs& a) {
  if (!a.perm || !a.pflag) return hipSuccess;
  int* ppos = a.pflag + a.njobs;
  void* tmp = (void*)(((uintptr_t)(a.pflag + 2 * (size_t)a.njobs) + 255) & ~(uintptr_t)255);
  size_t bytes = roll_order_scratch_bytes(a.njobs);
  hipError_t e = hipcub::DeviceScan::ExclusiveSum(tmp, bytes, a.pflag, ppos, a.njobs, st);
  if (e != hipSuccess) return e;
  hipLaunchKernelGGL(k_roll_order, dim3((a.njobs + 63) / 64), dim3(64), 0, st, a.pflag, ppos, a.njobs, a.perm);
  return hipGetLastError();
}

__global__ void __launch_bounds__(256) k_fill_ints(FillInts f) {
  const int stride = gridDim.x * blockDim.x;
  for (int q = 0; q < f.nj; q++)
    for (int i = blockIdx.x * blockDim.x + threadIdx.x; i < f.n[q]; i += stride) f.p[q][i] = f.v[q];
}
hipError_t launch_fill_ints(hipStream_t st, const FillInts& f) {
  if (f.nj <= 0) return hipSuccess;
  int mx = 0;
  for (int q = 0; q < f.nj; q++) mx = f.n[q] > mx ? f.n[q] : mx;
  const int blocks = (mx + 255) / 256 < 64 ? (mx + 255) / 256 : 64;
  hipLaunchKernelGGL(k_fill_ints, dim3(blocks > 0 ? blocks : 1), dim3(256), 0, st, f);
  LAUNCH_CHECK();
  return hipSuccess;
}

hipError_t launch_rollout_persistent(hipStream_t st, const RollArgs& a0, int B, int* qnext, int* best, int blocks,
                                     bool prefilled) {
  hipError_t e;
  if (!prefilled && a0.ncarry_out && (e = hipMemsetAsync(a0.ncarry_out, 0, sizeof(int), st)) != hipSuccess) return e;
  if (a0.njobs <= 0 && a0.nrep <= 0 && a0.ncarry <= 0) return hipSuccess;
  if (!prefilled) {
    if ((e = hipMemsetAsync(qnext, 0, sizeof(int), st)) != hipSuccess) return e;
    if (B > 0 && (e = hipMemsetAsync(best + a0.sbase, 0x7f, sizeof(int) * B, st)) != hipSuccess) return e;
  }
  RollArgs a = a0;
  a.B = B;
  const size_t obs_lds = a.p.need_gap ? 0 : (roll_lds_bytes(a0) + 15) / 16 * 16;
  const bool coop = a.coop_enable && !a.p.need_gap && a.p.coll_mode == CLRRT_COLLISION_OBB && a.p.n_obs > 0 && a.grid.gw > 0 &&
                    obs_lds + 4 * kCoopLdsPerWave <= 148 * 1024;
  a.coop_off = (int)obs_lds;
  const size_t lds = obs_lds + (coop ? 4 * kCoopLdsPerWave : 0);
  const bool carry = a.cap > 0 || a.ncarry > 0;
  const void* fn = a.p.need_gap ? (carry ? (const void*)&k_roll_run<true, false, true> : (const void*)&k_roll_run<true, false, false>)
                   : coop       ? (carry ? (const void*)&k_roll_run<false, true, true> : (const void*)&k_roll_run<false, true, false>)
                                : (carry ? (const void*)&k_roll_run<false, false, true> : (const void*)&k_roll_run<false, false, false>);
  if (lds > 64 * 1024 && (e = hipFuncSetAttribute(fn, hipFuncAttributeMaxDynamicSharedMemorySize, (int)lds)) != hipSuccess)
    return e;
  const int nqueue = a0.njobs + a0.nrep + a0.ncarry;
  int lpw = a0.lanes_per_wave > 0 && a0.lanes_per_wave < 64 ? a0.lanes_per_wave : 64;
  if (a0.lanes_per_wave <= 0) {
    const int waves = 4 * blocks;
    lpw = (nqueue + waves - 1) / waves;
    lpw = lpw < 1 ? 1 : (lpw > 64 ? 64 : lpw);
  }
  a.lanes_per_wave = lpw;
  const int nb = blocks < (nqueue + 4 * lpw - 1) / (4 * lpw) ? blocks : (nqueue + 4 * lpw - 1) / (4 * lpw);
  if (a.njobs > 0 && a.perm && a.pflag) {
    hipLaunchKernelGGL(k_roll_flag, dim3((a.njobs + 63) / 64), dim3(64), 0, st, a);
    LAUNCH_CHECK();
    if ((e = roll_order(st, a)) != hipSuccess) return e;
  } else {
    a.perm = nullptr;
  }
  if (carry) {
    if (a.p.need_gap)
      hipLaunchKernelGGL((k_roll_run<true, false, true>), dim3(nb), dim3(256), lds, st, a, qnext, best, B);
    else if (coop)
      hipLaunchKernelGGL((k_roll_run<false, true, true>), dim3(nb), dim3(256), lds, st, a, qnext, best, B);
    else
      hipLaunchKernelGGL((k_roll_run<false, false, true>), dim3(nb), dim3(256), lds, st, a, qnext, best, B);
  } else if (a.p.need_gap) {
    hipLaunchKernelGGL((k_roll_run<true, false, false>), dim3(nb), dim3(256), lds, st, a, qnext, best, B);
  } else if (coop) {
    hipLaunchKernelGGL((k_roll_run<false, true, false>), dim3(nb), dim3(256), lds, st, a, qnext, best, B);
  } else {
    hipLaunchKernelGGL((k_roll_run<false, false, false>), dim3(nb), dim3(256), lds, st, a, qnext, best, B);
  }
  LAUNCH_CHECK();
  return hipSuccess;
}


hipError_t launch_rollout(hipStream_t st, int src, const RollArgs& a) {
  if (src == SRC_SPEC) return launch_roll_t<SRC_SPEC>(st, a);
  if (src == SRC_EXPL) return launch_roll_t<SRC_EXPL>(st, a);
  return launch_roll_t<SRC_LIST>(st, a);
}

hipError_t launch_select(hipStream_t st, const SelArgs& a) {
  hipLaunchKernelGGL(k_select, dim3((a.B + CLRRT_SEL_BLK - 1) / CLRRT_SEL_BLK), dim3(CLRRT_SEL_BLK), 0, st, a);
  LAUNCH_CHECK();
  return hipSuccess;
}

hipError_t launch_copy_rows(hipStream_t st, const Job* jobs, const clrrt_node* recs, int n, const double* slots,
                            int slot_rows, int slot_jobs, double* arena) {
  if (n <= 0) return hipSuccess;
  hipLaunchKernelGGL(k_copy_rows, dim3(n), dim3(256), 0, st, jobs, recs, slots, slot_rows, slot_jobs, arena);
  LAUNCH_CHECK();
  return hipSuccess;
}

hipError_t launch_conflict_fix(hipStream_t st, const DevParams& p, int B, const clrrt_sample* S,
                               const clrrt_node* reg, const clrrt_node* gbn, const SampleOut* so, const int* ctie,
                               const int* ncand, const float* ckey, const RollRes* res, int* fix_n, int* fix_ids,
                               int* fix_adj) {
  if (B <= 0) return hipSuccess;
  hipLaunchKernelGGL(k_conflict_fix, dim3((B + 63) / 64), dim3(64), 0, st, p, B, S, reg, gbn, so, ctie, ncand, ckey,
                     res, fix_n, fix_ids, fix_adj);
  LAUNCH_CHECK();
  return hipSuccess;
}

hipError_t launch_conflict(hipStream_t st, const DevParams& p, int B, const clrrt_sample* S,
                           const clrrt_node* reg, const clrrt_node* gbn, const SampleOut* so, const int* ctie,
                           int* first) {
  hipLaunchKernelGGL(k_conflict, dim3((B + 63) / 64), dim3(64), 0, st, p, B, S, reg, gbn, so, ctie, first);
  LAUNCH_CHECK();
  return hipSuccess;
}

size_t defer_select_bytes(int n) {
  size_t bytes = 0;
  hipcub::DeviceSelect::Flagged(nullptr, bytes, (const int*)nullptr, (const uint8_t*)nullptr, (int*)nullptr,
                                (int*)nullptr, n);
  return bytes;
}
hipError_t launch_defer_select(hipStream_t st, const int* gv, const uint8_t* pend, int n, int* out, int* n_out,
                               void* tmp, size_t tmp_bytes) {
  if (n <= 0) return hipMemsetAsync(n_out, 0, sizeof(int), st);
  size_t bytes = tmp_bytes;
  return hipcub::DeviceSelect::Flagged(tmp, bytes, gv, pend, out, n_out, n, st);
}

size_t compact_scan_bytes(int n) {
  size_t bytes = 0;
  hipcub::DeviceScan::ExclusiveSum(nullptr, bytes, (const uint64_t*)nullptr, (uint64_t*)nullptr, n);
  return bytes;
}

__global__ void k_xorder_keys(const clrrt_node* __restrict__ recs, int n, uint32_t* __restrict__ keys,
                              uint32_t* __restrict__ idx) {
  const int i = blockIdx.x * blockDim.x + threadIdx.x;
  if (i >= n) return;
  keys[i] = 255u - (((uint32_t)recs[i].goal >> 8) & 0xffu);
  idx[i] = (uint32_t)i;
}
__global__ void k_xgather(const clrrt_node* __restrict__ recs, const uint32_t* __restrict__ idx, int n,
                          clrrt_node* __restrict__ out) {
  const int i = blockIdx.x * blockDim.x + threadIdx.x;
  if (i >= n) return;
  clrrt_node r = recs[idx ? idx[i] : i];
  r.goal &= 0xff;
  out[i] = r;
}
__global__ void k_goal_count(const clrrt_node* __restrict__ recs, int n, unsigned long long* goal) {
  unsigned long long c = 0;
  for (int i = blockIdx.x * blockDim.x + threadIdx.x; i < n; i += gridDim.x * blockDim.x) c += recs[i].goal & 1;
#pragma unroll
  for (int o = 32; o > 0; o >>= 1) c += __shfl_xor(c, o, 64);
  if ((threadIdx.x & 63) == 0 && c) atomicAdd(goal, c);
}
size_t xorder_sort_bytes(int n) {
  size_t bytes = 0;
  hipcub::DeviceRadixSort::SortPairs(nullptr, bytes, (const uint32_t*)nullptr, (uint32_t*)nullptr,
                                     (const uint32_t*)nullptr, (uint32_t*)nullptr, n, 0, 8);
  return bytes;
}
hipError_t launch_xorder(hipStream_t st, const clrrt_node* recs, int n, bool sort, uint32_t* keys, void* tmp,
                         size_t tmp_bytes, clrrt_node* out, unsigned long long* goal) {
  if (n <= 0) return hipSuccess;
  const unsigned g = (unsigned)((n + 255) / 256);
  uint32_t* idx = nullptr;
// ... 112 lines not shown
```

Before: 1.335 million.

## Fuse commit compaction, bbox and counts into one scatter kernel with single readback

Folds the per-block counts into the select kernel and replaces the compact, bbox and defer-select launches with a single k_commit_scatter kernel. That kernel uses a last-block ticket to write one CommitRec, which is read back with a single memcpy. It also fuses replay-gather into tree append, moves the deferred ring copies into the rollout flag kernel, hoists the round prologue fill, and gives each NN lane its own order buffer so ordering is computed once per slot. The aim is to cut kernel launches, D2D copies and host-device round trips per round, at the cost of more complex cross-block ticket synchronisation.

Measured after the change: 1.344 million, median of 6. Within noise of the previous version (+0.7%).

```diff
diff --git a/cl-rrt_amd/csrc/clrrt_capi.hip b/cl-rrt_amd/csrc/clrrt_capi.hip
--- a/cl-rrt_amd/csrc/clrrt_capi.hip
+++ b/cl-rrt_amd/csrc/clrrt_capi.hip
@@ -74,6 +74,11 @@
   clrrt_node* out_nodes = nullptr;
   Job* jobs = nullptr;
   int64_t* totals = nullptr;
+  bool app_gather = false;
+  const int* app_cand = nullptr;
+  const clrrt_sample* app_samp = nullptr;
+  const RollRes* app_res = nullptr;
+  CommitRec* h_rec = nullptr;
   bool totals_zeroed = false;
   unsigned long long* work_ctr = nullptr;
   float* nn_seed = nullptr;
@@ -169,7 +174,7 @@
   int nn_split_delta = 0;
   int nn_delta_early = 1;
   int nn_lane_order = 1;
-  int* nn_order = nullptr;
+  int* nn_order[3] = {nullptr, nullptr, nullptr};
   float* wseed[3] = {nullptr, nullptr, nullptr};
   hipEvent_t ev_wm[3] = {nullptr, nullptr, nullptr};
   float* nn_seed2 = nullptr;
@@ -466,6 +471,21 @@
 
 const char* clrrt_last_error(const clrrt_ctx* c) { return c ? c->err.c_str() : "null context"; }
 
+static void free_commit_bufs(clrrt_ctx* c) {
+  for (void* p : {(void*)c->cmp.bsum, (void*)c->cmp.bpend, (void*)c->cmp.bbox_part, (void*)c->cmp.ticket, (void*)c->cmp.rec})
+    if (p) hipFree(p);
+  c->cmp.bsum = nullptr; c->cmp.bpend = nullptr; c->cmp.bbox_part = nullptr; c->cmp.ticket = nullptr; c->cmp.rec = nullptr;
+}
+static hipError_t alloc_commit_bufs(clrrt_ctx* c, int64_t V) {
+  const int nb = commit_blocks((int)V);
+  hipError_t e;
+  if ((e = dalloc(&c->cmp.bsum, nb)) != hipSuccess || (e = dalloc(&c->cmp.bpend, nb)) != hipSuccess ||
+      (e = dalloc(&c->cmp.bbox_part, 4 * (size_t)nb)) != hipSuccess || (e = dalloc(&c->cmp.ticket, 1)) != hipSuccess ||
+      (e = hipMalloc((void**)&c->cmp.rec, sizeof(CommitRec))) != hipSuccess)
+    return e;
+  return hipMemset(c->cmp.ticket, 0, sizeof(unsigned));
+}
+
 static void free_all(clrrt_ctx* c) {
   if (c->side) hipStreamSynchronize(c->side);
   void* ptrs[] = {c->tree, c->nn, c->arena, c->obs, c->d_samples, c->pk, c->pi, c->cand, c->ckey, c->ncand,
@@ -507,7 +527,7 @@
     if (c->ev_s[q]) hipEventDestroy(c->ev_s[q]);
     if (c->d1pk[q]) hipFree(c->d1pk[q]);
     if (c->wseed[q]) hipFree(c->wseed[q]);
-    if (q == 0 && c->nn_order) hipFree(c->nn_order);
+    if (c->nn_order[q]) hipFree(c->nn_order[q]);
     if (c->ev_wm[q]) hipEventDestroy(c->ev_wm[q]);
     if (c->d1pi[q]) hipFree(c->d1pi[q]);
   }
@@ -521,6 +541,8 @@
   if (c->ev_rs0) hipEventDestroy(c->ev_rs0);
   if (c->ev_rs1) hipEventDestroy(c->ev_rs1);
   if (c->h_totals) hipHostFree(c->h_totals);
+  if (c->h_rec) hipHostFree(c->h_rec);
+  free_commit_bufs(c);
   if (c->h_int) hipHostFree(c->h_int);
   if (c->h_bbox) hipHostFree(c->h_bbox);
   if (c->dbg_host) hipHostFree(c->dbg_host);
@@ -594,6 +616,8 @@
   chk(dalloc(&c->cmp.scanned, B));
   c->cmp.tmp_bytes = compact_scan_bytes((int)B);
   chk(hipMalloc(&c->cmp.tmp, std::max<size_t>(c->cmp.tmp_bytes, 256)));
+  chk(alloc_commit_bufs(c, B));
+  chk(hipHostMalloc((void**)&c->h_rec, sizeof(CommitRec), hipHostMallocDefault));
   chk(dalloc(&c->nn_seed, B));
   chk(dalloc(&c->roll_q, 1));
   chk(dalloc(&c->roll_best, B));
@@ -1789,10 +1813,34 @@
   return CLRRT_OK;
 }
 
+static int round_prologue(clrrt_ctx* c, int n, hipStream_t s) {
+  auto& d = c->def;
+  const int sbase = (int)(d.round % d.R) * (int)c->cap.max_batch;
+  FillInts f;
+  f.add(d.d_cnt + 1, 1, 0);
+  f.add(c->roll_q, 1, 0);
+  f.add(d.best + sbase, n, 0x7f7f7f7f);
+  f.add(d.d_cnt + 2, 1, 0);
+  f.add((int*)c->totals, 16, 0);
+  HIPC(c, launch_fill_ints(s, f));
+  c->totals_zeroed = true;
+  return CLRRT_OK;
+}
+
+static void select_counts(clrrt_ctx* c, SelArgs& s) {
+  s.packed = c->cmp.packed;
+  s.totals = c->totals;
+  s.bsum = c->cmp.bsum;
+  s.bpend = c->cmp.bpend;
+  s.ticket = c->cmp.ticket;
+}
+
 static int eval_samples(clrrt_ctx* c, int n, bool exact, int* L_out, bool have_lists = false,
                         const std::function<int()>& during_roll = nullptr,
-                        const std::function<int()>& pre_roll = nullptr) {
+                        const std::function<int()>& pre_roll = nullptr, bool prologue_done = false,
+                        bool count = false) {
   hipStream_t st = c->stream;
+  if (!prologue_done) c->totals_zeroed = false;
   KeyId* scratch = nullptr;
   if (exact) {
     int rc = ensure_sort_scratch(c, (int64_t)n * c->n_nodes);
@@ -1822,20 +1870,16 @@
     if (rc != CLRRT_OK) return rc;
   }
   const bool defer = c->def.active && !exact && persistent && deferred;
+  RingStore ring;
   if (defer) {
     auto& d = c->def;
     d.slot = (int)(d.round % d.R);
     const int64_t B = c->cap.max_batch;
-    HIPC(c, hipMemcpyAsync(d.cand + (int64_t)d.slot * B * CAND_K, c->cand, sizeof(int) * n * CAND_K,
-                           hipMemcpyDeviceToDevice, st));
-    HIPC(c, hipMemcpyAsync(d.ncand + (int64_t)d.slot * B, c->ncand, sizeof(int) * n, hipMemcpyDeviceToDevice, st));
-    HIPC(c, hipMemcpyAsync(d.samp + (int64_t)d.slot * B, c->d_samples, sizeof(clrrt_sample) * n,
-                           hipMemcpyDeviceToDevice, st));
     if (d.nd + (int64_t)n > d.vcap) return fail(c, CLRRT_ECAPACITY, "deferred samples exceed the commit buffers");
-    if (rst != st) {
-      HIPC(c, hipEventRecord(c->ev_rs0, st));
-      HIPC(c, hipStreamWaitEvent(rst, c->ev_rs0, 0));
-    }
+    ring.cand = d.cand + (int64_t)d.slot * B * CAND_K;
+    ring.ncand = d.ncand + (int64_t)d.slot * B;
+    ring.samp = d.samp + (int64_t)d.slot * B;
+    ring.ncand_src = c->ncand;
   }
   {
     KTimer kt(c, 1, rst);
@@ -1870,15 +1914,11 @@
       fprintf(stderr, "[dbg] pre-rollout work done (n %d, nrep %d, ncarry %d)\n", n, a.nrep, a.ncarry);
     }
     if (persistent && defer) {
-      FillInts f;
-      f.add(a.ncarry_out, 1, 0);
-      f.add(c->roll_q, 1, 0);
-      f.add(c->def.best + a.sbase, n, 0x7f7f7f7f);
-      f.add(c->def.d_cnt + 2, 1, 0);
-      f.add((int*)c->totals, 16, 0);
-      HIPC(c, launch_fill_ints(rst, f));
-      c->totals_zeroed = true;
-      HIPC(c, launch_rollout_persistent(rst, a, n, c->roll_q, c->def.best, blocks, true));
+      if (!prologue_done) {
+        const int rc = round_prologue(c, n, rst);
+        if (rc != CLRRT_OK) return rc;
+      }
+      HIPC(c, launch_rollout_persistent(rst, a, n, c->roll_q, c->def.best, blocks, true, &ring));
     } else if (persistent)
       HIPC(c, launch_rollout_persistent(rst, a, n, c->roll_q, defer ? c->def.best : c->roll_best, blocks));
     else
@@ -1940,6 +1980,11 @@
   c->def.nd_eval = defer ? c->def.nd : -1;
   {
     KTimer kt(c, 2);
+    if (count && !exact) {
+      if (!c->totals_zeroed) HIPC(c, hipMemsetAsync(c->totals, 0, sizeof(int64_t) * 8, st));
+      c->totals_zeroed = true;
+      select_counts(c, s);
+    }
     HIPC(c, launch_select(st, s));
   }
   int L = n;
@@ -1962,12 +2007,41 @@
   return CLRRT_OK;
 }
 
-static int compact_and_copy(clrrt_ctx* c, int L, int* n_out, bool merge_bbox) {
+static int compact_and_copy(clrrt_ctx* c, int L, int* n_out, bool merge_bbox, bool counted = false,
+                            bool fuse_append = false) {
   hipStream_t st = c->stream;
   auto& d = c->def;
   const bool defer = d.nd_eval >= 0;
   const int V = defer ? d.nd_eval + L : L;
-  {
+  c->app_gather = false;
+  if (counted) {
+    {
+      KTimer kt(c, 2);
+      const bool tag = defer && c->sh.world > 1;
+      if (!c->totals_zeroed) HIPC(c, hipMemsetAsync(c->totals, 0, sizeof(int64_t) * 8, st));
+      c->totals_zeroed = false;
+      CommitArgs a;
+      memset(&a, 0, sizeof(a));
+      a.V = V; a.so = c->so; a.reg = c->regnodes; a.gbn = c->gbnodes; a.row_base = c->n_rows; a.rank = c->rank;
+      a.out = c->out_nodes; a.jobs = c->jobs; a.totals = c->totals;
+      a.tag_slot = tag ? d.slot : 0; a.tag_R = tag ? d.R : 0; a.tag_B = (int)c->cap.max_batch;
+      if (defer) {
+        a.gv = d.gv; a.pend = d.pend; a.dl_out = d.dlist[1 - d.cur_dl]; a.d_cnt = d.d_cnt;
+        a.carry_ovf = c->work_ctr + 62;
+      }
+      a.watchdog = c->work_ctr + 56;
+      a.d_bbox = c->d_bbox;
+      HIPC(c, launch_commit_scatter(st, a, c->cmp));
+    }
+    HIPC(c, hipMemcpyAsync(c->h_rec, c->cmp.rec, sizeof(CommitRec), hipMemcpyDeviceToHost, st));
+    HIPC(c, hipStreamSynchronize(st));
+    memcpy(c->h_totals, c->h_rec->totals, sizeof(int64_t) * 8);
+    if (merge_bbox) memcpy(c->h_bbox, c->h_rec->bbox, sizeof(double) * 4);
+    if (defer) {
+      c->h_int[0] = c->h_rec->cnt[0]; c->h_int[1] = c->h_rec->cnt[1]; c->h_int[3] = c->h_rec->cnt[2];
+      c->h_int[2] = c->h_rec->carry_ovf;
+    }
+  } else {
     KTimer kt(c, 2);
     const bool tag = defer && c->sh.world > 1;
     HIPC(c, launch_compact(st, V, c->d_samples, c->cand, c->regnodes, c->gbnodes, c->so, c->n_rows, c->rank,
@@ -1977,15 +2051,17 @@
     if (merge_bbox) HIPC(c, launch_bbox(st, c->out_nodes, c->totals, 0, c->d_bbox));
     if (defer) HIPC(c, launch_defer_select(st, d.gv, d.pend, V, d.dlist[1 - d.cur_dl], d.d_cnt, d.sel_tmp, d.sel_bytes));
   }
-  HIPC(c, hipMemcpyAsync(c->h_totals, c->totals, sizeof(int64_t) * 8, hipMemcpyDeviceToHost, st));
-  if (merge_bbox) HIPC(c, hipMemcpyAsync(c->h_bbox, c->d_bbox, sizeof(double) * 4, hipMemcpyDeviceToHost, st));
-  if (defer) {
-    HIPC(c, hipMemcpyAsync(c->h_int, d.d_cnt, sizeof(int) * 2, hipMemcpyDeviceToHost, st));
-    HIPC(c, hipMemcpyAsync(c->h_int + 3, d.d_cnt + 2, sizeof(int), hipMemcpyDeviceToHost, st));
-    HIPC(c, hipMemcpyAsync(c->h_int + 2, (const char*)(c->work_ctr + 62), sizeof(int), hipMemcpyDeviceToHost, st));
-  }
-  HIPC(c, hipStreamSynchronize(st));
-  {
+  if (!counted) {
+    HIPC(c, hipMemcpyAsync(c->h_totals, c->totals, sizeof(int64_t) * 8, hipMemcpyDeviceToHost, st));
+    if (merge_bbox) HIPC(c, hipMemcpyAsync(c->h_bbox, c->d_bbox, sizeof(double) * 4, hipMemcpyDeviceToHost, st));
+    if (defer) {
+      HIPC(c, hipMemcpyAsync(c->h_int, d.d_cnt, sizeof(int) * 2, hipMemcpyDeviceToHost, st));
+      HIPC(c, hipMemcpyAsync(c->h_int + 3, d.d_cnt + 2, sizeof(int), hipMemcpyDeviceToHost, st));
+      HIPC(c, hipMemcpyAsync(c->h_int + 2, (const char*)(c->work_ctr + 62), sizeof(int), hipMemcpyDeviceToHost, st));
+    }
+    HIPC(c, hipStreamSynchronize(st));
+  }
+  if (!counted || c->h_rec->watchdog != 0) {
     const int rw = watchdog_check(c);
     if (rw != CLRRT_OK) return rw;
   }
@@ -2029,11 +2105,15 @@
       if (rc != CLRRT_OK) return rc;
     }
     KTimer kt(c, 2);
-    if (defer)
-      HIPC(c, launch_replay_gather(st, c->jobs, c->out_nodes, (int)nn, c->tree, d.cand, d.samp, d.res, c->rep_buf));
-    else
-      HIPC(c, launch_replay_gather(st, c->jobs, c->out_nodes, (int)nn, c->tree, c->cand, c->d_samples, c->res_spec,
-                                   c->rep_buf));
+    const int* g_cand = defer ? d.cand : c->cand;
+    const clrrt_sample* g_samp = defer ? d.samp : c->d_samples;
+    const RollRes* g_res = defer ? d.res : c->res_spec;
+    if (fuse_append && c->sh.world <= 1) {
+      c->app_gather = true;
+      c->app_cand = g_cand; c->app_samp = g_samp; c->app_res = g_res;
+    } else {
+      HIPC(c, launch_replay_gather(st, c->jobs, c->out_nodes, (int)nn, c->tree, g_cand, g_samp, g_res, c->rep_buf));
+    }
     c->rep_n = (int)nn;
   } else {
     KTimer kt(c, 2);
@@ -2092,6 +2172,8 @@
     HIPC(c, dalloc(&c->cmp.scanned, V));
     c->cmp.tmp_bytes = compact_scan_bytes((int)V);
     HIPC(c, hipMalloc(&c->cmp.tmp, std::max<size_t>(c->cmp.tmp_bytes, 256)));
+    free_commit_bufs(c);
+    HIPC(c, alloc_commit_bufs(c, V));
     HIPC(c, dalloc(&d.dlist[0], V));
     HIPC(c, dalloc(&d.dlist[1], V));
     HIPC(c, dalloc(&d.gv, V));
@@ -2207,13 +2289,16 @@
       s.p = c->dp; s.tree = c->tree; s.cand = d.cand; s.ckey = nullptr; s.ncand = d.ncand; s.res = d.res;
       s.res_gb = d.res_gb; s.regnodes = c->regnodes; s.gbnodes = c->gbnodes; s.so = c->so;
       s.view = d.dlist[d.cur_dl]; s.nd = d.nd; s.sbase = 0; s.gv = d.gv; s.pend = d.pend; s.B = d.nd;
+      HIPC(c, hipMemsetAsync(c->totals, 0, sizeof(int64_t) * 8, st));
+      c->totals_zeroed = true;
       if (d.nd > 0) {
         KTimer kt(c, 2);
+        select_counts(c, s);
         HIPC(c, launch_select(st, s));
       }
       d.nd_eval = d.nd;
       int nn = 0, n_app = 0;
-      int rc = compact_and_copy(c, 0, &nn, true);
+      int rc = compact_and_copy(c, 0, &nn, true, true, true);
       if (rc == CLRRT_OK) rc = commit_round(c, nn, c->sh.max_ms, &n_app);
       if (rc != CLRRT_OK) return rc;
       if (goal_nodes) *goal_nodes += c->last_goal_nodes;
@@ -2368,7 +2453,22 @@
   *n_app = 0;
   if (h.world <= 1) {
     *n_app = nn;
-    const int rc = append_nodes(c, c->out_nodes, nn);
+    int rc = CLRRT_OK;
+    if (c->app_gather) {
+      c->app_gather = false;
+      if (c->n_nodes + nn > c->cap.max_nodes) {
+        c->rep_n = 0;
+        return fail(c, CLRRT_ECAPACITY, "tree full");
+      }
+      {
+        KTimer kt(c, 2);
+        HIPC(c, launch_append_replay(c->stream, c->out_nodes, nn, c->n_nodes, c->tree, c->nn, c->jobs, c->app_cand,
+                                     c->app_samp, c->app_res, c->rep_buf));
+      }
+      c->n_nodes += nn;
+    } else {
+      rc = append_nodes(c, c->out_nodes, nn);
+    }
     if (rc == CLRRT_OK) c->round_sizes.push_back(c->n_nodes);
     return rc;
   }
@@ -2451,6 +2551,7 @@
   hipEvent_t evs = nullptr;
   float* wseed = nullptr;
   hipEvent_t evm = nullptr;
+  int* order = nullptr;
 };
 
 static int lag_alloc(clrrt_ctx* c) {
@@ -2478,7 +2579,7 @@
   for (int q = 0; q < 3; q++) {
     HIPC(c, dalloc(&c->d1pk[q], c->partial_cap));
     HIPC(c, dalloc(&c->wseed[q], B));
-    if (q == 0) HIPC(c, dalloc(&c->nn_order, B));
+    HIPC(c, dalloc(&c->nn_order[q], B));
     HIPC(c, hipEventCreateWithFlags(&c->ev_wm[q], hipEventDisableTiming));
     HIPC(c, dalloc(&c->d1pi[q], c->partial_cap));
     HIPC(c, hipEventCreateWithFlags(&c->ev_d1[q], hipEventDisableTiming));
@@ -2550,6 +2651,8 @@
   B.d1pk = c->d1pk[1]; B.d1pi = c->d1pi[1]; B.evd1 = c->ev_d1[1]; B.evs = c->ev_s[1];
   A.wseed = c->wseed[0]; A.evm = c->ev_wm[0];
   B.wseed = c->wseed[1]; B.evm = c->ev_wm[1];
+  A.order = c->nn_order[0]; B.order = c->nn_order[1];
+  int* cur_order = c->nn_order[2];
   float* cur_wseed = c->wseed[2];
   hipEvent_t cur_evm = c->ev_wm[2];
   const bool early = c->nn_delta_early != 0;
@@ -2604,6 +2707,10 @@
     HIPC(c, hipStreamWaitEvent(s, c->ev_tree, 0));
     HIPC(c, hipMemcpyAsync(sl.d, sl.h, sizeof(clrrt_sample) * n, hipMemcpyHostToDevice, s));
     HIPC(c, hipEventRecord(sl.evs, s));
+    if (c->nn_lane_order) {
+      KTimer kt(c, 0, s);
+      HIPC(c, launch_nn_order(s, sl.d, n, sl.order));
+    }
     sl.d1_count = 0;
     sl.d1_chunks = 0;
     c->nn_super_bounds += (int64_t)n * walk_super_count(c->n_nodes);
@@ -2668,6 +2775,8 @@
     }
     const int64_t gA_all = A.n > 0 ? A.g : gA;
     draw_to(gb + gA_all + gB);
+    const bool prologue = c->def.active && c->roll_persistent && c->rows_deferred && c->dp.n_steps_max > 0;
+    if (prologue && (rc = round_prologue(c, nb, c->stream)) != CLRRT_OK) break;
     if (have_cur) {
       KTimer kt(c, 4);
       HIPC(c, hipStreamWaitEvent(c->stream, cur_ev, 0));
@@ -2708,9 +2817,9 @@
     };
     int L = nb, nn = 0, n_app = 0;
     if ((rc = eval_samples(c, nb, false, &L, true, (nA > 0 || nB > 0) ? std::function<int()>(ahead) : nullptr,
-                           nullptr)) != CLRRT_OK)
+                           nullptr, prologue, true)) != CLRRT_OK)
       break;
-    if ((rc = compact_and_copy(c, L, &nn, true)) != CLRRT_OK) break;
+    if ((rc = compact_and_copy(c, L, &nn, true, true, true)) != CLRRT_OK) break;
     const double ms_commit = std::chrono::duration<double, std::milli>(std::chrono::steady_clock::now() - t0).count();
     if ((rc = commit_round(c, nn, ms_commit, &n_app)) != CLRRT_OK) break;
     if ((A.n > 0 || (split_delta && B.n > 0)))
@@ -2728,7 +2837,7 @@
         const int max_chunks = (int)std::max<int64_t>(1, c->partial_cap / ((int64_t)A.n * NN_K));
         HIPC(c, launch_nn_delta_partial(s, A.d, A.n, c->nn, (int)first2, (int)cnt2, c->dp, su2.fr, c->pk, c->pi,
                                         max_chunks, A.ckey, A.ncand, early ? A.wseed : c->nn_seed, early,
-                                        c->nn_lane_order ? c->nn_order : nullptr, &nch2));
+                                        c->nn_lane_order ? A.order : nullptr, &nch2));
       }
       if (early) HIPC(c, hipStreamWaitEvent(s, A.evw, 0));
       if (A.d1_count > 0) HIPC(c, hipStreamWaitEvent(s, A.evd1, 0));
@@ -2753,7 +2862,7 @@
         const int max_chunks = (int)std::max<int64_t>(1, c->partial_cap / ((int64_t)A.n * NN_K));
         HIPC(c, launch_nn_delta_partial(s, A.d, A.n, c->nn, (int)first, (int)cnt, c->dp, su2.fr, c->pk, c->pi,
                                         max_chunks, nullptr, nullptr, A.wseed, true,
-                                        c->nn_lane_order ? c->nn_order : nullptr, &nch));
+                                        c->nn_lane_order ? A.order : nullptr, &nch));
       }
       HIPC(c, hipStreamWaitEvent(s, A.evw, 0));
       {
@@ -2791,7 +2900,7 @@
         const int max_chunks = (int)std::max<int64_t>(1, c->partial_cap / ((int64_t)B.n * NN_K));
         HIPC(c, launch_nn_delta_partial(s2, B.d, B.n, c->nn, (int)B.tree_n, (int)cnt1, c->dp, su1.fr, B.d1pk, B.d1pi,
                                         max_chunks, B.ckey, B.ncand, early ? B.wseed : c->nn_seed2, early,
-                                        c->nn_lane_order ? c->nn_order : nullptr, &B.d1_chunks));
+                                        c->nn_lane_order ? B.order : nullptr, &B.d1_chunks));
       }
       HIPC(c, hipEventRecord(B.evd1, s2));
     }
@@ -2813,14 +2922,14 @@
       old.d = c->d_samples; old.h = c->h_samples; old.cand = c->cand; old.ckey = c->ckey; old.ncand = c->ncand;
       old.ctie = c->ctie; old.ev = cur_ev; old.evw = cur_evw; old.stream = cur_stream;
       old.d1pk = cur_d1pk; old.d1pi = cur_d1pi; old.evd1 = cur_evd1; old.evs = cur_evs;
-      old.wseed = cur_wseed; old.evm = cur_evm;
+      old.wseed = cur_wseed; old.evm = cur_evm; old.order = cur_order;
       have_cur = A.n > 0;
       c->d_samples = A.d; c->h_samples = A.h; c->cand = A.cand; c->ckey = A.ckey; c->ncand = A.ncand; c->ctie = A.ctie;
       cur_ev = A.ev;
       cur_evw = A.evw;
       cur_stream = A.stream;
       cur_d1pk = A.d1pk; cur_d1pi = A.d1pi; cur_evd1 = A.evd1; cur_evs = A.evs;
-      cur_wseed = A.wseed; cur_evm = A.evm;
+      cur_wseed = A.wseed; cur_evm = A.evm; cur_order = A.order;
       A = B;
       B = old;
       B.n = 0;
@@ -2934,14 +3043,14 @@
     int L = nb, nn = 0, n_app = 0;
     auto build = [&]() -> int { return pre_roll_build(c, su); };
     if ((rc = eval_samples(c, nb, exact, &L, have_next, nb2 > 0 ? std::function<int()>(prefetch) : nullptr,
-                           nb2 > 0 ? std::function<int()>(build) : nullptr)) != CLRRT_OK)
+                           nb2 > 0 ? std::function<int()>(build) : nullptr, false, !exact)) != CLRRT_OK)
       break;
     if (!exact) {
       int64_t want = gb + (int64_t)cur;
       if (n_iters > 0) want = std::min<int64_t>(want, n_iters - st.iterations);
       draw_to(want);
     }
-    if ((rc = compact_and_copy(c, L, &nn, true)) != CLRRT_OK) break;
+    if ((rc = compact_and_copy(c, L, &nn, true, !exact, !exact)) != CLRRT_OK) break;
     const int64_t first_new = c->n_nodes;
     const double ms_commit = std::chrono::duration<double, std::milli>(std::chrono::steady_clock::now() - t0).count();
     if ((rc = commit_round(c, nn, ms_commit, &n_app)) != CLRRT_OK) break;
diff --git a/cl-rrt_amd/csrc/clrrt_internal.hpp b/cl-rrt_amd/csrc/clrrt_internal.hpp
--- a/cl-rrt_amd/csrc/clrrt_internal.hpp
+++ b/cl-rrt_amd/csrc/clrrt_internal.hpp
@@ -106,6 +106,13 @@
   int job_stride;
 };
 
+struct RingStore {
+  int* cand = nullptr;
+  int* ncand = nullptr;
+  clrrt_sample* samp = nullptr;
+  const int* ncand_src = nullptr;
+};
+
 struct SelArgs {
   DevParams p;
   const clrrt_node* __restrict__ tree;
@@ -123,6 +130,11 @@
   int* gv;
   uint8_t* pend;
   int* new_pend;
+  uint64_t* packed;
+  int64_t* totals;
+  uint64_t* bsum;
+  int* bpend;
+  unsigned* ticket;
 };
 
 struct NnFrame {
@@ -195,8 +207,9 @@
                            float* ckey, int* ncand, int* ctie, float* seed);
 hipError_t launch_nn_delta_partial(hipStream_t st, const clrrt_sample* S, int B, const NnRec* nodes, int first,
                                    int count, const DevParams& p, const NnFrame& fr, float* pk, int* pi, int max_chunks,
-                                   const float* ckey, const int* ncand, float* gcap, bool seeded, int* order,
+                                   const float* ckey, const int* ncand, float* gcap, bool seeded, const int* order,
                                    int* nchunks_out);
+hipError_t launch_nn_order(hipStream_t st, const clrrt_sample* S, int B, int* order);
 hipError_t launch_nn_delta_merge(hipStream_t st, int B, int nchunks, const DevParams& p, const float* pk, const int* pi,
                                  int id0, int* cand, float* ckey, int* ncand, int* ctie);
 hipError_t launch_nn(hipStream_t st, const clrrt_sample* S, int B, const NnRec* nodes, int N,
@@ -210,7 +223,7 @@
                                  const DevParams& p, int* cand, float* ckey, int* ncand, int* ctie);
 int nn_exact_small_max();
 hipError_t launch_rollout_persistent(hipStream_t st, const RollArgs& a, int B, int* qnext, int* best, int blocks,
-                                     bool prefilled = false);
+                                     bool prefilled = false, const RingStore* ring = nullptr);
 struct FillInts {
   int* p[8];
   int n[8];
@@ -241,12 +254,48 @@
 hipError_t launch_conflict(hipStream_t st, const DevParams& p, int B, const clrrt_sample* S,
                            const clrrt_node* reg, const clrrt_node* gbn, const SampleOut* so, const int* ctie,
                            int* first);
+struct CommitRec;
 struct CompactBufs {
   uint64_t* packed;
   uint64_t* scanned;
   void* tmp;
   size_t tmp_bytes;
-};
+  uint64_t* bsum = nullptr;
+  int* bpend = nullptr;
+  double* bbox_part = nullptr;
+  unsigned* ticket = nullptr;
+  CommitRec* rec = nullptr;
+};
+struct CommitRec {
+  int64_t totals[8];
+  double bbox[4];
+  int cnt[3];
+  int carry_ovf;
+  unsigned long long watchdog;
+};
+int commit_blocks(int views);
+struct CommitArgs {
+  int V;
+  const SampleOut* so;
+  const clrrt_node* reg;
+  const clrrt_node* gbn;
+  int64_t row_base;
+  int rank;
+  clrrt_node* out;
+  Job* jobs;
+  int64_t* totals;
+  int tag_slot, tag_R, tag_B;
+  const int* gv;
+  const uint8_t* pend;
+  int* dl_out;
+  int* d_cnt;
+  const unsigned long long* carry_ovf;
+  const unsigned long long* watchdog;
+  double* d_bbox;
+};
+hipError_t launch_commit_scatter(hipStream_t st, const CommitArgs& a, const CompactBufs& cb);
+hipError_t launch_append_replay(hipStream_t st, const clrrt_node* recs, int n, int64_t base, clrrt_node* tree, NnRec* nn,
+                                const Job* jobs, const int* cand, const clrrt_sample* S, const RollRes* res, void* out);
 size_t compact_scan_bytes(int n);
 size_t defer_select_bytes(int n);
 hipError_t launch_defer_select(hipStream_t st, const int* gv, const uint8_t* pend, int n, int* out, int* n_out,
diff --git a/cl-rrt_amd/csrc/clrrt_kernels.hip b/cl-rrt_amd/csrc/clrrt_kernels.hip
--- a/cl-rrt_amd/csrc/clrrt_kernels.hip
+++ b/cl-rrt_amd/csrc/clrrt_kernels.hip
@@ -1244,21 +1244,65 @@
   return (along > 0.f && across >= 0.57735f * along) ? 1 : 0;
 }
 
-__global__ void __launch_bounds__(256) k_roll_order(const int* __restrict__ pflag, const int* __restrict__ ppos,
+__global__ void __launch_bounds__(256) k_roll_order(const int* __restrict__ pflag, const int* __restrict__ bcnt,
                                                     int n, int* __restrict__ perm) {
-  const int q = blockIdx.x * blockDim.x + threadIdx.x;
+  __shared__ int s_w[4], s_before[4], s_total[4];
+  const int q = blockIdx.x * 256 + threadIdx.x;
+  const int lane = threadIdx.x & 63, w = threadIdx.x >> 6;
+  int before = 0, total = 0;
+  for (int i = threadIdx.x; i < (int)gridDim.x; i += 256) {
+    const int v = bcnt[i];
+    total += v;
+    before += i < (int)blockIdx.x ? v : 0;
+  }
+#pragma unroll
+  for (int o = 32; o > 0; o >>= 1) {
+    before += __shfl_xor(before, o, 64);
+    total += __shfl_xor(total, o, 64);
+  }
+  const int f = q < n ? pflag[q] : 0;
+  const unsigned long long m = __ballot(f != 0);
+  if (lane == 0) { s_w[w] = __popcll(m); s_before[w] = before; s_total[w] = total; }
+  __syncthreads();
   if (q >= n) return;
-  const int nf = ppos[n - 1] + pflag[n - 1];
-  const int pos = pflag[q] ? ppos[q] : nf + (q - ppos[q]);
+  int ppos = s_before[0] + s_before[1] + s_before[2] + s_before[3];
+  const int nf = s_total[0] + s_total[1] + s_total[2] + s_total[3];
+  for (int i = 0; i < w; i++) ppos += s_w[i];
+  ppos += __popcll(m & ((1ull << lane) - 1ull));
+  const int pos = f ? ppos : nf + (q - ppos);
   perm[pos] = q;
 }
 
-__global__ void __launch_bounds__(256) k_roll_flag(RollArgs a) {
-  const int j = blockIdx.x * blockDim.x + threadIdx.x;
-  if (j >= a.njobs) return;
-  const int id = a.cand[j];
-  a.pflag[(j % CAND_K) * a.B + j / CAND_K] =
-      id < 0 ? 0 : roll_likely_long(a.tree[id].state, a.samples[j / CAND_K].x, a.samples[j / CAND_K].y);
+__device__ __forceinline__ void ring_store(const RingStore& r, const clrrt_sample* __restrict__ S, int j, int id) {
+  r.cand[j] = id;
+  if (j % CAND_K == 0) {
+    r.ncand[j / CAND_K] = r.ncand_src[j / CAND_K];
+    r.samp[j / CAND_K] = S[j / CAND_K];
+  }
+}
+
+__global__ void __launch_bounds__(256) k_roll_flag(RollArgs a, RingStore r, int* __restrict__ bcnt) {
+  __shared__ int s_w[4];
+  const int q = blockIdx.x * 256 + threadIdx.x;
+  int f = 0;
+  if (q < a.njobs) {
+    const int k = q / a.B, s = q - k * a.B;
+    const int j = s * CAND_K + k;
+    const int id = a.cand[j];
+    f = id < 0 ? 0 : roll_likely_long(a.tree[id].state, a.samples[s].x, a.samples[s].y);
+    a.pflag[q] = f;
+    if (r.cand) ring_store(r, a.samples, j, id);
+  }
+  const unsigned long long m = __ballot(f != 0);
+  if ((threadIdx.x & 63) == 0) s_w[threadIdx.x >> 6] = __popcll(m);
+  __syncthreads();
+  if (threadIdx.x == 0) bcnt[blockIdx.x] = s_w[0] + s_w[1] + s_w[2] + s_w[3];
+}
+
+__global__ void __launch_bounds__(256) k_ring_store(RingStore r, const clrrt_sample* __restrict__ S,
+                                                    const int* __restrict__ cand, int njobs) {
+  const int j = blockIdx.x * 256 + threadIdx.x;
+  if (j < njobs) ring_store(r, S, j, cand[j]);
 }
 
 #ifndef REFILL_MIN
@@ -1641,9 +1685,7 @@
 }
 
 
-__global__ void k_select(SelArgs a) {
-  const int v = blockIdx.x * blockDim.x + threadIdx.x;
-  if (v >= a.B) return;
+__device__ __forceinline__ int select_view(const SelArgs& a, int v, uint64_t& pk, unsigned long long* cnt) {
   const int g = v < a.nd ? a.view[v] : a.sbase + (v - a.nd);
   const int64_t g0 = (int64_t)g * CAND_K;
   const int nc = a.ncand[g];
@@ -1678,13 +1720,14 @@
     if (a.gv) a.gv[v] = g;
     if (a.pend) a.pend[v] = 1;
     if (a.new_pend && v >= a.nd) atomicAdd(a.new_pend, 1);
-    return;
+    return 1;
   }
   if (a.gv) a.gv[v] = g;
   if (a.pend) a.pend[v] = 0;
   o.thr = !a.ckey ? __builtin_inff()
           : o.k >= 0 ? a.ckey[g0 + o.k] : (nc == a.p.sort_limit ? a.ckey[g0 + nc - 1] : __builtin_inff());
   o.gb_ok = 0;
+  uint64_t nn = 0, nr = 0;
   if (o.k >= 0) {
     const int pid = a.cand[g0 + o.k];
     const clrrt_node& par = a.tree[pid];
@@ -1692,6 +1735,7 @@
     fill_node(n, a.res[g0 + o.k], pid, par.costE, par.costS);
     a.regnodes[v] = n;
     o.nrows_reg = n.nrows;
+    nn++; nr += (uint64_t)n.nrows; cnt[5] += n.goal;
     const RollRes& gr = a.res_gb[g0 + o.k];
     if (gr.outcome >= 0) {
       o.rollouts++;
@@ -1705,10 +1749,47 @@
         a.gbnodes[v] = gn;
         o.gb_ok = 1;
         o.nrows_gb = gn.nrows;
+        nn++; nr += (uint64_t)gn.nrows; cnt[5] += gn.goal;
       }
     }
   }
   a.so[v] = o;
+  cnt[0] = o.steps; cnt[1] = o.f_col; cnt[2] = o.f_acc; cnt[3] = o.f_it; cnt[4] = o.rollouts;
+  pk = (nr << 24) | nn;
+  return 0;
+}
+
+template <bool COUNT>
+__global__ void __launch_bounds__(CLRRT_SEL_BLK) k_select(SelArgs a) {
+  const int v = blockIdx.x * blockDim.x + threadIdx.x;
+  uint64_t pk = 0;
+  unsigned long long cnt[6] = {0, 0, 0, 0, 0, 0};
+  int pend = 0;
+  if (v < a.B) pend = select_view(a, v, pk, cnt);
+  if (!COUNT) return;
+  if (v < a.B) a.packed[v] = pk;
+  __shared__ unsigned long long s_sum[CLRRT_SEL_BLK / 64][8];
+  unsigned long long r[8] = {cnt[0], cnt[1], cnt[2], cnt[3], cnt[4], cnt[5], pk, (unsigned long long)pend};
+#pragma unroll
+  for (int c = 0; c < 8; c++) {
+#pragma unroll
+    for (int o = 32; o > 0; o >>= 1) r[c] += __shfl_xor(r[c], o, 64);
+    if ((threadIdx.x & 63) == 0) s_sum[threadIdx.x >> 6][c] = r[c];
+  }
+  __syncthreads();
+  if (threadIdx.x < 8) {
+    unsigned long long t = 0;
+#pragma unroll
+    for (int w = 0; w < CLRRT_SEL_BLK / 64; w++) t += s_sum[w][threadIdx.x];
+    if (threadIdx.x < 6) {
+      if (t) atomicAdd((unsigned long long*)&a.totals[2 + threadIdx.x], t);
+    } else if (threadIdx.x == 6) {
+      a.bsum[blockIdx.x] = t;
+    } else {
+      a.bpend[blockIdx.x] = (int)t;
+      if (blockIdx.x == 0) *a.ticket = 0u;
+    }
+  }
 }
 
 __global__ void k_conflict(DevParams p, int B, const clrrt_sample* __restrict__ S,
@@ -1895,6 +1976,154 @@
   }
 }
 
+static_assert(CLRRT_SEL_BLK == 256, "k_commit_scatter runs k_select's blocks");
+__global__ void __launch_bounds__(256) k_commit_scatter(CommitArgs a, const uint64_t* __restrict__ packed,
+                                                        const uint64_t* __restrict__ bsum,
+                                                        const int* __restrict__ bpend, double* bbox_part,
+                                                        unsigned* ticket, CommitRec* rec) {
+  __shared__ unsigned long long s_before[4], s_total[4], s_wpk[4];
+  __shared__ int s_pbefore[4], s_ptotal[4], s_wpd[4];
+  __shared__ double s_bb[4][4];
+  __shared__ int s_last;
+  const int tid = threadIdx.x, lane = tid & 63, w = tid >> 6;
+  const int s = blockIdx.x * 256 + tid;
+  const int nblk = (a.V + 255) / 256;
+  unsigned long long before = 0, total = 0;
+  int pbefore = 0, ptotal = 0;
+  for (int i = tid; i < nblk; i += 256) {
+    const unsigned long long b = bsum[i];
+    const int p = bpend[i];
+    total += b;
+    ptotal += p;
+    if (i < (int)blockIdx.x) { before += b; pbefore += p; }
+  }
+#pragma unroll
+  for (int o = 32; o > 0; o >>= 1) {
+    before += __shfl_xor(before, o, 64);
+    total += __shfl_xor(total, o, 64);
+    pbefore += __shfl_xor(pbefore, o, 64);
+    ptotal += __shfl_xor(ptotal, o, 64);
+  }
+  const bool act = s < a.V;
+  const unsigned long long pk = act ? packed[s] : 0ull;
+  const int pd = act && a.pend ? (int)a.pend[s] : 0;
+  unsigned long long incl = pk;
+  int pincl = pd;
+#pragma unroll
+  for (int o = 1; o < 64; o <<= 1) {
+    const unsigned long long t = __shfl_up(incl, o, 64);
+    const int tp = __shfl_up(pincl, o, 64);
+    if (lane >= o) { incl += t; pincl += tp; }
+  }
+  if (lane == 0) { s_before[w] = before; s_total[w] = total; s_pbefore[w] = pbefore; s_ptotal[w] = ptotal; }
+  if (lane == 63) { s_wpk[w] = incl; s_wpd[w] = pincl; }
+  __syncthreads();
+  unsigned long long off = s_before[0] + s_before[1] + s_before[2] + s_before[3] + (incl - pk);
+  int poff = s_pbefore[0] + s_pbefore[1] + s_pbefore[2] + s_pbefore[3] + (pincl - pd);
+  for (int i = 0; i < w; i++) { off += s_wpk[i]; poff += s_wpd[i]; }
+  total = s_total[0] + s_total[1] + s_total[2] + s_total[3];
+  ptotal = s_ptotal[0] + s_ptotal[1] + s_ptotal[2] + s_ptotal[3];
+  double bb[4] = {HUGE_VAL, HUGE_VAL, -HUGE_VAL, -HUGE_VAL};
+  if (act) {
+    int64_t node_off = (int64_t)(off & 0xffffffu), row_off = (int64_t)(off >> 24);
+    const SampleOut& o = a.so[s];
+    const int tag = a.tag_R > 0 ? ((a.tag_slot - o.g / a.tag_B + a.tag_R) % a.tag_R) << 8 : 0;
+    if (o.k >= 0) {
+      clrrt_node n = a.reg[s];
+      const double x = n.state[0], y = n.state[1];
+      if (isfinite(x) && isfinite(y)) { bb[0] = fmin(bb[0], x); bb[1] = fmin(bb[1], y); bb[2] = fmax(bb[2], x); bb[3] = fmax(bb[3], y); }
+      n.goal |= tag;
+      n.owner = a.rank;
+      n.row_offset = a.row_base + row_off;
+      a.out[node_off] = n;
+      Job jb;
+      jb.parent = o.g * CAND_K + o.k; jb.from_reg = 0; jb.gb = 0; jb.pad = 0;
+      jb.sx = 0; jb.sy = 0;
+      jb.row_off = a.row_base + row_off;
+      a.jobs[node_off] = jb;
+      node_off++;
+      row_off += o.nrows_reg;
+    }
+    if (o.gb_ok) {
+      clrrt_node n = a.gbn[s];
+      const double x = n.state[0], y = n.state[1];
+      if (isfinite(x) && isfinite(y)) { bb[0] = fmin(bb[0], x); bb[1] = fmin(bb[1], y); bb[2] = fmax(bb[2], x); bb[3] = fmax(bb[3], y); }
+      n.goal |= tag;
+      n.owner = a.rank;
+      n.row_offset = a.row_base + row_off;
+      a.out[node_off] = n;
+      Job jb;
+      jb.parent = o.g * CAND_K + o.k; jb.from_reg = 0; jb.gb = 1; jb.pad = 0;
+      jb.sx = 0; jb.sy = 0;
+      jb.row_off = a.row_base + row_off;
+      a.jobs[node_off] = jb;
+    }
+    if (pd) a.dl_out[poff] = a.gv[s];
+  }
+#pragma unroll
+  for (int o = 32; o > 0; o >>= 1) {
+    bb[0] = fmin(bb[0], __shfl_xor(bb[0], o, 64)); bb[1] = fmin(bb[1], __shfl_xor(bb[1], o, 64));
+    bb[2] = fmax(bb[2], __shfl_xor(bb[2], o, 64)); bb[3] = fmax(bb[3], __shfl_xor(bb[3], o, 64));
+  }
+  if (lane == 0) { s_bb[w][0] = bb[0]; s_bb[w][1] = bb[1]; s_bb[w][2] = bb[2]; s_bb[w][3] = bb[3]; }
+  __syncthreads();
+  if (tid == 0) {
+    double* mine = bbox_part + 4 * (size_t)blockIdx.x;
+    mine[0] = fmin(fmin(s_bb[0][0], s_bb[1][0]), fmin(s_bb[2][0], s_bb[3][0]));
+    mine[1] = fmin(fmin(s_bb[0][1], s_bb[1][1]), fmin(s_bb[2][1], s_bb[3][1]));
+    mine[2] = fmax(fmax(s_bb[0][2], s_bb[1][2]), fmax(s_bb[2][2], s_bb[3][2]));
+    mine[3] = fmax(fmax(s_bb[0][3], s_bb[1][3]), fmax(s_bb[2][3], s_bb[3][3]));
+    __builtin_amdgcn_fence(__ATOMIC_RELEASE, "agent");
+    asm volatile("s_waitcnt vmcnt(0)" ::: "memory");
+    const unsigned t = __hip_atomic_fetch_add(ticket, 1u, __ATOMIC_RELAXED, __HIP_MEMORY_SCOPE_AGENT);
+    const int last = t == gridDim.x - 1;
+    if (last) {
+      __builtin_amdgcn_fence(__ATOMIC_ACQUIRE, "agent");
+      asm volatile("s_waitcnt vmcnt(0)" ::: "memory");
+    }
+    s_last = last;
+  }
+  __syncthreads();
+  if (!s_last) return;
+  bb[0] = bb[1] = HUGE_VAL;
+  bb[2] = bb[3] = -HUGE_VAL;
+  for (int i = tid; i < (int)gridDim.x; i += 256) {
+    const unsigned long long* p = (const unsigned long long*)(bbox_part + 4 * (size_t)i);
+    bb[0] = fmin(bb[0], __longlong_as_double((long long)__hip_atomic_load(p + 0, __ATOMIC_RELAXED, __HIP_MEMORY_SCOPE_AGENT)));
+    bb[1] = fmin(bb[1], __longlong_as_double((long long)__hip_atomic_load(p + 1, __ATOMIC_RELAXED, __HIP_MEMORY_SCOPE_AGENT)));
+    bb[2] = fmax(bb[2], __longlong_as_double((long long)__hip_atomic_load(p + 2, __ATOMIC_RELAXED, __HIP_MEMORY_SCOPE_AGENT)));
+    bb[3] = fmax(bb[3], __longlong_as_double((long long)__hip_atomic_load(p + 3, __ATOMIC_RELAXED, __HIP_MEMORY_SCOPE_AGENT)));
+  }
+#pragma unroll
+  for (int o = 32; o > 0; o >>= 1) {
+    bb[0] = fmin(bb[0], __shfl_xor(bb[0], o, 64)); bb[1] = fmin(bb[1], __shfl_xor(bb[1], o, 64));
+    bb[2] = fmax(bb[2], __shfl_xor(bb[2], o, 64)); bb[3] = fmax(bb[3], __shfl_xor(bb[3], o, 64));
+  }
+  if (lane == 0) { s_bb[w][0] = bb[0]; s_bb[w][1] = bb[1]; s_bb[w][2] = bb[2]; s_bb[w][3] = bb[3]; }
+  __syncthreads();
+  if (tid != 0) return;
+  bb[0] = fmin(fmin(s_bb[0][0], s_bb[1][0]), fmin(s_bb[2][0], s_bb[3][0]));
+  bb[1] = fmin(fmin(s_bb[0][1], s_bb[1][1]), fmin(s_bb[2][1], s_bb[3][1]));
+  bb[2] = fmax(fmax(s_bb[0][2], s_bb[1][2]), fmax(s_bb[2][2], s_bb[3][2]));
+  bb[3] = fmax(fmax(s_bb[0][3], s_bb[1][3]), fmax(s_bb[2][3], s_bb[3][3]));
+  const int64_t nn = (int64_t)(total & 0xffffffu), nr = (int64_t)(total >> 24);
+  a.totals[0] = nn;
+  a.totals[1] = nr;
+  rec->totals[0] = nn;
+  rec->totals[1] = nr;
+  for (int q = 2; q < 8; q++) rec->totals[q] = a.totals[q];
+  for (int q = 0; q < 4; q++) { a.d_bbox[q] = bb[q]; rec->bbox[q] = bb[q]; }
+  if (a.d_cnt) {
+    a.d_cnt[0] = ptotal;
+    rec->cnt[0] = ptotal; rec->cnt[1] = a.d_cnt[1]; rec->cnt[2] = a.d_cnt[2];
+  } else {
+    rec->cnt[0] = rec->cnt[1] = rec->cnt[2] = 0;
+  }
+  rec->carry_ovf = a.carry_ovf ? (int)(unsigned)*a.carry_ovf : 0;
+  rec->watchdog = *a.watchdog;
+  *ticket = 0u;
+}
+
 __global__ void __launch_bounds__(256) k_copy_rows(const Job* __restrict__ jobs, const clrrt_node* __restrict__ recs,
                                                    const double* __restrict__ slots, int slot_rows, int slot_jobs,
                                                    double* __restrict__ arena) {
@@ -2000,6 +2229,42 @@
   r.id = (int32_t)id;
   r.ca = cosf((float)d.ang_par); r.sa = sinf((float)d.ang_par);
   return r;
+}
+
+__global__ void __launch_bounds__(256) k_append_replay(const clrrt_node* __restrict__ in, int n, int64_t base,
+                                                       clrrt_node* tree, NnRec* __restrict__ nn,
+                                                       const Job* __restrict__ jobs, const int* __restrict__ cand,
+                                                       const clrrt_sample* __restrict__ S,
+                                                       const RollRes* __restrict__ res, Replay* __restrict__ out) {
+  const int i = blockIdx.x * blockDim.x + threadIdx.x;
+  if (i >= n) return;
+  clrrt_node d = in[i];
+  {
+    const Job jb = jobs[i];
+    Replay o;
+    o.row_off = jb.row_off;
+    o.nrows = d.nrows;
+    o.pad = 0;
+    o.src.gb = jb.gb;
+    o.src.pad = 0;
+    if (jb.gb) {
+      const RollRes& g = res[jb.parent];
+#pragma unroll
+      for (int q = 0; q < 10; q++) o.src.st[q] = g.st[q];
+      o.src.bx = g.bx; o.src.by = g.by; o.src.vb = g.vback;
+      o.src.sx = o.src.sy = 0.0;
+    } else {
+      const clrrt_node& p = tree[cand[jb.parent]];
+#pragma unroll
+      for (int q = 0; q < 10; q++) o.src.st[q] = p.state[q];
+      o.src.bx = p.ref_back[0]; o.src.by = p.ref_back[1]; o.src.vb = p.ref_vback;
+      o.src.sx = S[jb.parent / CAND_K].x; o.src.sy = S[jb.parent / CAND_K].y;
+    }
+    out[i] = o;
+  }
+  if (d.parent == CLRRT_PARENT_PREV) d.parent = (int32_t)(base + i - 1);
+  tree[base + i] = d;
+  nn[base + i] = nn_record(d, base + i);
 }
 
 __device__ void init_root(const double* st, clrrt_node* tree, NnRec* nn, double* arena, int owner) {
@@ -2536,16 +2801,11 @@
 
 hipError_t launch_nn_delta_partial(hipStream_t st, const clrrt_sample* S, int B, const NnRec* nodes, int first,
                                    int count, const DevParams& p, const NnFrame& fr, float* pk, int* pi, int max_chunks,
-                                   const float* ckey, const int* ncand, float* gcap, bool seeded, int* order,
+                                   const float* ckey, const int* ncand, float* gcap, bool seeded, const int* order,
                                    int* nchunks_out) {
   *nchunks_out = 0;
   if (count <= 0 || B <= 0) return hipSuccess;
-  const int* sord = nullptr;
-  if (order) {
-    hipLaunchKernelGGL(k_nn_order, dim3(1), dim3(1024), 0, st, S, B, order);
-    LAUNCH_CHECK();
-    sord = order;
-  }
+  const int* sord = order;
   const int groups = (B + CLRRT_PATH_BLK - 1) / CLRRT_PATH_BLK;
   int nchunks = (count + 255) / 256;
   const int want = max(1, 2048 / max(1, groups));
@@ -2562,6 +2822,12 @@
                      nchunks, p, fr, pk, pi, gcap, nullptr, sord);
   LAUNCH_CHECK();
   *nchunks_out = nchunks;
+  return hipSuccess;
+}
+hipError_t launch_nn_order(hipStream_t st, const clrrt_sample* S, int B, int* order) {
+  if (B <= 0) return hipSuccess;
+  hipLaunchKernelGGL(k_nn_order, dim3(1), dim3(1024), 0, st, S, B, order);
+  LAUNCH_CHECK();
   return hipSuccess;
 }
 hipError_t launch_nn_delta_merge(hipStream_t st, int B, int nchunks, const DevParams& p, const float* pk, const int* pi,
@@ -2633,19 +2899,13 @@
   return hipSuccess;
 }
 
-size_t roll_order_scratch_bytes(int n) {
-  size_t bytes = 0;
-  hipcub::DeviceScan::ExclusiveSum(nullptr, bytes, (const int*)nullptr, (int*)nullptr, n);
-  return bytes;
-}
-static hipError_t roll_order(hipStream_t st, const RollArgs& a) {
-  if (!a.perm || !a.pflag) return hipSuccess;
-  int* ppos = a.pflag + a.njobs;
-  void* tmp = (void*)(((uintptr_t)(a.pflag + 2 * (size_t)a.njobs) + 255) & ~(uintptr_t)255);
-  size_t bytes = roll_order_scratch_bytes(a.njobs);
-  hipError_t e = hipcub::DeviceScan::ExclusiveSum(tmp, bytes, a.pflag, ppos, a.njobs, st);
-  if (e != hipSuccess) return e;
-  hipLaunchKernelGGL(k_roll_order, dim3((a.njobs + 63) / 64), dim3(64), 0, st, a.pflag, ppos, a.njobs, a.perm);
+size_t roll_order_scratch_bytes(int n) { return sizeof(int) * (size_t)((n + 255) / 256); }
+static hipError_t roll_flag_order(hipStream_t st, const RollArgs& a, const RingStore& ring) {
+  int* bcnt = a.pflag + a.njobs;
+  const int nblk = (a.njobs + 255) / 256;
+  hipLaunchKernelGGL(k_roll_flag, dim3(nblk), dim3(256), 0, st, a, ring, bcnt);
+  LAUNCH_CHECK();
+  hipLaunchKernelGGL(k_roll_order, dim3(nblk), dim3(256), 0, st, a.pflag, bcnt, a.njobs, a.perm);
   return hipGetLastError();
 }
 
@@ -2665,7 +2925,7 @@
 }
 
 hipError_t launch_rollout_persistent(hipStream_t st, const RollArgs& a0, int B, int* qnext, int* best, int blocks,
-                                     bool prefilled) {
+                                     bool prefilled, const RingStore* ring) {
   hipError_t e;
   if (!prefilled && a0.ncarry_out && (e = hipMemsetAsync(a0.ncarry_out, 0, sizeof(int), st)) != hipSuccess) return e;
   if (a0.njobs <= 0 && a0.nrep <= 0 && a0.ncarry <= 0) return hipSuccess;
@@ -2695,12 +2955,15 @@
   }
   a.lanes_per_wave = lpw;
   const int nb = blocks < (nqueue + 4 * lpw - 1) / (4 * lpw) ? blocks : (nqueue + 4 * lpw - 1) / (4 * lpw);
-  if (a.njobs > 0 && a.perm && a.pflag) {
-    hipLaunchKernelGGL(k_roll_flag, dim3((a.njobs + 63) / 64), dim3(64), 0, st, a);
-    LAUNCH_CHECK();
-    if ((e = roll_order(st, a)) != hipSuccess) return e;
+  const RingStore rs = ring && a.njobs > 0 ? *ring : RingStore();
+  if (a.njobs > 0 && a.njobs == B * CAND_K && a.perm && a.pflag) {
+    if ((e = roll_flag_order(st, a, rs)) != hipSuccess) return e;
   } else {
     a.perm = nullptr;
+    if (rs.cand) {
+      hipLaunchKernelGGL(k_ring_store, dim3((a.njobs + 255) / 256), dim3(256), 0, st, rs, a.samples, a.cand, a.njobs);
+      LAUNCH_CHECK();
+    }
   }
   if (carry) {
     if (a.p.need_gap)
@@ -2728,7 +2991,31 @@
 }
 
 hipError_t launch_select(hipStream_t st, const SelArgs& a) {
-  hipLaunchKernelGGL(k_select, dim3((a.B + CLRRT_SEL_BLK - 1) / CLRRT_SEL_BLK), dim3(CLRRT_SEL_BLK), 0, st, a);
+  if (a.B <= 0) return hipSuccess;
+  const dim3 grid((a.B + CLRRT_SEL_BLK - 1) / CLRRT_SEL_BLK);
+  if (a.packed)
+    hipLaunchKernelGGL(k_select<true>, grid, dim3(CLRRT_SEL_BLK), 0, st, a);
+  else
+    hipLaunchKernelGGL(k_select<false>, grid, dim3(CLRRT_SEL_BLK), 0, st, a);
+  LAUNCH_CHECK();
+  return hipSuccess;
+}
+
+int commit_blocks(int views) { return (views + CLRRT_SEL_BLK - 1) / CLRRT_SEL_BLK + 1; }
+
+hipError_t launch_commit_scatter(hipStream_t st, const CommitArgs& a, const CompactBufs& cb) {
+  const int nblk = a.V > 0 ? (a.V + 255) / 256 : 1;
+  hipLaunchKernelGGL(k_commit_scatter, dim3(nblk), dim3(256), 0, st, a, cb.packed, cb.bsum, cb.bpend, cb.bbox_part,
+                     cb.ticket, cb.rec);
+  LAUNCH_CHECK();
+  return hipSuccess;
+}
+
+hipError_t launch_append_replay(hipStream_t st, const clrrt_node* recs, int n, int64_t base, clrrt_node* tree, NnRec* nn,
+                                const Job* jobs, const int* cand, const clrrt_sample* S, const RollRes* res, void* out) {
+  if (n <= 0) return hipSuccess;
+  hipLaunchKernelGGL(k_append_replay, dim3((n + 255) / 256), dim3(256), 0, st, recs, n, base, tree, nn, jobs, cand, S,
+                     res, (Replay*)out);
   LAUNCH_CHECK();
   return hipSuccess;
 }
```
